# rishabhmisra/Scalable-Bayesian-Matrix-Factorization

Measured on AMD Instinct MI355X. Metric: ratings/sec per Gibbs sweep, ML-20M K=100, higher is better.
Workload: dtype f64

## Files before the change

### scalable-bayesian-matrix-factorization_amd/csrc/ctx.h

```cpp
#pragma once
#include <hip/hip_runtime.h>

#include <algorithm>
#include <array>
#include <chrono>
#include <cmath>
#include <cstdarg>
#include <cstdio>
#include <cstdlib>
#include <cstring>
#include <memory>
#include <numeric>
#include <string>
#include <thread>
#include <vector>

#include "../../include/sbmf.h"
#include "comm.h"
#include "common.h"
#include <rccl/rccl.h>
#include "kernels.h"
#include "rng.h"
#include "fmc.h"
#include "fmm.h"
#include "fmg.h"
#include "fmq.h"
#include "foldin.h"
#include "lists.h"
#include "recommend.h"
#include "samples.h"
#include "samples_foldin.h"
#include "vbo.h"

struct sbmf_ctx;

namespace sbmf {

static const int NBIN = GK_NUM + 1;

struct Side {
    uint32_t R = 0;
    std::vector<uint32_t> ptr;
    std::vector<uint32_t> part;
    std::vector<uint32_t> perm;
    std::vector<double> r;
    uint32_t r0 = 0, r1 = 0;
    std::vector<uint64_t> bounds;
    struct StreamSet {
        std::vector<SplitTask> stasks;
        std::vector<SplitRow> xrows;
        uint32_t nxchunk = 0;
        uint32_t sgrid = 0;
        uint32_t cmax = 0;
        uint32_t tune = 0;
    };
    struct Stage {
        uint32_t r0 = 0, r1 = 0;
        std::vector<uint32_t> bin_rows[NBIN];
        StreamSet ss[2];
        std::vector<std::array<uint32_t, 3>> gsub[GK_NUM];
        DBuf d_bins[NBIN], d_stasks[2], d_xrows[2];
        std::vector<size_t> soff, scnt, roff, rcnt;
        size_t rbeg = 0, rend = 0;
    };
    std::vector<std::unique_ptr<Stage>> stg;
    std::vector<std::vector<uint64_t>> sbounds;
    std::vector<ResidTask> rtasks;
    std::vector<uint32_t> rtptr;
    std::vector<uint32_t> perm2, unpack;
    size_t nsend = 0, nrecv = 0;
};

static const int KIND_STREAM = GK_NUM;

}

using namespace sbmf;

struct Hyper {
    double tau = 1.0, b0 = 0.0, mu_b0 = 0.0, sig_b0 = 0.0;
    std::vector<double> sig_u, mu_u, sig_v, mu_v;
};

struct ScoreList {
    const char* what;
    const char* reg;
    uint32_t n = 0, J = 0, Jp = 0;
    uint32_t count = 0;
    int clamp = 0;
    bool latest = false;
    DBuf d_ids, d_S1, d_S2;
    Span sel;
    void alloc(uint32_t n_, uint32_t J_, int clamp_, hipStream_t st);
    void drop();
    template <typename T>
    void accumulate(sbmf_ctx* c, const T* rows, const double* bu, const double* bv, double b0, hipStream_t se);
    void scores(sbmf_ctx* c, const char* fn, uint32_t row, double* mean, double* stdev);
    void recommend(sbmf_ctx* c, const uint32_t* csr_ptr, const uint32_t* csr_items, uint32_t topn, uint32_t flags,
                   double risk, uint32_t* items, double* mean, double* stdev);
};

struct SampleStore {
    uint32_t cap = 0, every = 1, head = 0, count = 0, seen = 0;
    size_t bytes = 0;
    DBuf d_U, d_V, d_bu, d_bv;
    std::vector<double> b0;
    std::vector<uint32_t> sweep;
    std::vector<double> hyper;
    bool has_hyper = false;
    Span cev, scv, sel;
    Span gdr, gsc, gse;
    uint64_t budget = 0;
    bool unfused = false, fused_draw = false;
    uint32_t slot(uint32_t s) const { return (head + s) % cap; }
    void alloc(sbmf_ctx* c, uint32_t cap_, uint32_t every_);
    void drop();
    template <typename T>
    void keep(sbmf_ctx* c, const Hyper& hy, hipStream_t se);
};

struct sbmf_ctx {
    sbmf_ctx() { sbmf::audit().contexts++; }
    sbmf_config cfg{};
    std::string err;
    bool spent = false, dead = false;
    std::vector<uint32_t> tu, ti, su, si;
    std::vector<double> tr, sr;
    uint32_t I = 0, J = 0, I_req = 0, J_req = 0;
    bool prepared = false;
    double init_sd = 1.0, lo = 1.0, hi = 5.0;
    int sd_is_var = 1;
    uint32_t K = 0, Kp = 0;
    Side users, items;
    uint64_t t0 = 0, t1 = 0;
    std::vector<uint64_t> tbounds, tbblocks;
    std::vector<uint64_t> tperm;
    Hyper hyp[2];
    int reported = 0;
    Hyper& hyper_of(uint32_t sw) { return hyp[sw & 1]; }
    bool bias = false;
    std::vector<uint32_t> empty_u, empty_v;
    std::vector<std::array<double, 3>> shadow_u, shadow_v;
    uint32_t sweep = 0, collected = 0;
    GlibcRand grand{1};
    int nranks = 1, rank = 0;
    Comm own_comm;
    Comm* comm = &own_comm;
    hipStream_t st = nullptr;
    hipEvent_t ev[10] = {};
    std::vector<hipEvent_t> kevs;
    hipEvent_t& kev(uint32_t stage, int side, int kind, int e) {
        return kevs[(((size_t)stage * 2 + side) * SBMF_NKIND + kind) * 2 + e];
    }
    std::vector<int8_t> kprev;
    int8_t& kpv(uint32_t stage, int side, int kind) { return kprev[((size_t)stage * 2 + side) * SBMF_NKIND + kind]; }
    std::vector<hipEvent_t> kbegin;
    hipEvent_t& kbg(uint32_t stage, int side, int kind) { return kbegin[((size_t)stage * 2 + side) * SBMF_NKIND + kind]; }
    uint32_t nstages = 1;
    hipStream_t stc = nullptr;
    std::vector<hipEvent_t> sev;
    bool virt = false;
    std::vector<hipEvent_t> tsev;
    hipEvent_t cev[2] = {};
    hipStream_t sto = nullptr;
    hipStream_t sto2 = nullptr;
    hipEvent_t oev[4] = {};
    DBuf d_uptr, d_upart, d_uperm, d_ur, d_vptr, d_vpart, d_vperm, d_vr;
    DBuf d_U, d_V, d_Eu, d_Ev, d_zU, d_zV, d_hyper;
    DBuf d_rowsq_u, d_rowtr_u, d_rowsq_v, d_rowtr_v;
    DBuf d_colpart, d_res, d_scratch;
    size_t scratch_half = 0;

    bool kprof = false;
    int kprof_set = 0;
    DBuf d_kprof;
    DBuf d_rtasks, d_rtptr, d_rtsq;
    DBuf d_xslabs, d_xcnt, d_xchunk_sq, d_xchunk_tr, d_xnewown;
    static constexpr size_t kColdSlot = 256;
    DBuf d_gcold;
    std::vector<unsigned char> h_gcold;
    bool time_kinds = true;
    size_t xset_nx = 1;
    DBuf d_tu, d_ti, d_tr, d_tsum, d_tpart;
    DBuf d_uperm2, d_vperm2, d_uunpack, d_vunpack, d_xrecv;
    DBuf d_bu, d_bv, d_mbu, d_mbv, d_sbu, d_sbv;
    DBuf d_var3u, d_var3v, d_epart;
    std::vector<double> h_res;
    double* h_pre = nullptr;
    void* h_io = nullptr;
    double* h_out() { return static_cast<double*>(h_io); }
    void* h_hyper() { return static_cast<char*>(h_io) + 128; }
    hipEvent_t hev = nullptr;
    struct PreDraw {
        bool valid = false;
        bool staged = false;
        uint32_t sweep = 0;
        double d0 = 0;
        Hyper h;
    } pre;
    bool hyper_ahead = false;
    double* h_pinned = nullptr;
    size_t h_pinned_bytes = 0, h_pre_bytes = 0, h_io_bytes = 0;
    sbmf_timing timing{};
    uint32_t launches = 0;
    ScoreList watch{"watch list", "sbmf_watch_users"};
    hipEvent_t wev[2] = {};
    ScoreList guests{"fold-in list", "sbmf_foldin_users"};
    uint32_t fdrawn = 0;
    GuestCSR fcsr;
    DBuf d_fG, d_fhyp;
    double* h_fhyp = nullptr;
    size_t h_fhyp_bytes = 0;
    hipEvent_t fev[3] = {};
    ScoreList fmq{"query list", "sbmf_fm_query_cases"};
    FMQueryList fmqd;
    SampleStore samples;
    VBLearner* vb = nullptr;
    FMChain* fm = nullptr;
    FMGroups fmgroups;
    std::vector<FMRelation> fmrels;
    struct HostCases {
        std::vector<uint64_t> ptr;
        std::vector<uint32_t> attr;
        std::vector<float> x, y;
        uint32_t num_attr = 0;
        bool set = false;
        sbmf_cases view() {
            sbmf_cases c{};
            c.n = y.size();
            c.nnz = attr.size();
            c.num_attr = num_attr;
            c.ptr = ptr.data();
            c.attr = attr.data();
            c.x = x.data();
            c.target = y.data();
            return c;
        }
    } ctr, cte;
    ~sbmf_ctx();
};

#define API_BEGIN try {
#define API_END(ctx) } catch (...) { return sbmf::api_error(ctx); } return SBMF_OK;

namespace sbmf {

int api_error(sbmf_ctx* ctx);
void samples_ready(sbmf_ctx* c, const char* fn);
size_t slot_bytes(const sbmf_ctx* c);
void partition_bounds(const uint32_t* ptr, uint32_t R, int nranks, uint64_t* bounds);
template <typename T>
void prepare_T(sbmf_ctx* c);
template <typename T>
void run_half(sbmf_ctx* c, const Hyper& hy, bool users, uint32_t stage, hipEvent_t start = nullptr);
template <typename T>
void run_sweeps_T(sbmf_ctx* c, uint32_t nsweeps, sbmf_sweep_cb cb, void* user);

enum { RES_ESQ = 0, RES_TRSQ = 1, RES_TEST_AVG = 2, RES_TEST_THIS = 3, RES_ES = 4, RES_ESQ2 = 5, RES_TIMEOUT = 7, RES_COL = 8 };

static size_t tsize(const sbmf_ctx* c) { return c->cfg.precision == SBMF_F32 ? 4 : 8; }

static bool avg_collected(const sbmf_config& cf) {
    return cf.average == 1 || (cf.average == 0 && cf.quirks == SBMF_QUIRKS_NONE);
}

template <typename T>
static std::vector<T> to_T(const std::vector<double>& v) {
    return std::vector<T>(v.begin(), v.end());
}

template <typename T>
static void upload_table(sbmf_ctx* c, DBuf& d, const double* src, uint32_t R) {
    std::vector<T> h((size_t)R * c->Kp, T(0));
    for (uint32_t r = 0; r < R; ++r)
        for (uint32_t k = 0; k < c->K; ++k) h[(size_t)r * c->Kp + k] = (T)src[(size_t)r * c->K + k];
    HIPCHK(hipMemcpy(d.p, h.data(), h.size() * sizeof(T), hipMemcpyHostToDevice));
}
template <typename T>
static void download_table(sbmf_ctx* c, const DBuf& d, double* dst, uint32_t R) {
    std::vector<T> h((size_t)R * c->Kp);
    HIPCHK(hipMemcpy(h.data(), d.p, h.size() * sizeof(T), hipMemcpyDeviceToHost));
    for (uint32_t r = 0; r < R; ++r)
        for (uint32_t k = 0; k < c->K; ++k) dst[(size_t)r * c->K + k] = (double)h[(size_t)r * c->Kp + k];
}
static void upload_table(sbmf_ctx* c, DBuf& d, const double* src, uint32_t R) {
    c->cfg.precision == SBMF_F32 ? upload_table<float>(c, d, src, R) : upload_table<double>(c, d, src, R);
}
static void download_table(sbmf_ctx* c, const DBuf& d, double* dst, uint32_t R) {
    c->cfg.precision == SBMF_F32 ? download_table<float>(c, d, dst, R) : download_table<double>(c, d, dst, R);
}

static void ensure_pinned(sbmf_ctx* c, size_t bytes) {
    if (c->h_pinned_bytes >= bytes) return;
    pinned_free(c->h_pinned, c->h_pinned_bytes);
    c->h_pinned_bytes = 0;
    pinned_alloc((void**)&c->h_pinned, bytes);
    c->h_pinned_bytes = bytes;
}

}
```

### scalable-bayesian-matrix-factorization_amd/csrc/kernels.h

```cpp
#pragma once
#include <hip/hip_runtime.h>

#include <cstdint>

namespace sbmf {

template <typename T>
struct HalfArgs {
    const uint32_t* ptr;
    const uint32_t* part;
    const uint32_t* perm;
    const T* E_this;
    T* E_other;
    const T* r_this;
    T* own;
    const T* partner;
    const T* sig;
    const T* mu;
    uint32_t zrow;
    const T* zbuf;
    T tau;
    uint32_t K, Kp;
    int sd_is_var;
    uint64_t seed;
    uint32_t sweep, tag;
    double* row_sq;
    double* row_tr;
    T lo, hi;
    int e_from_dot;
    uint32_t tune;
    unsigned long long* prof;
    uint64_t lim_partner;
    uint64_t lim_other;
    uint64_t lim_this;
    uint32_t lim_rows;
};

enum GblockKind { GK_W4 = 0, GK_W16 = 1, GK_B2 = 2, GK_B4 = 3, GK_B8 = 4, GK_NUM = 5 };
inline uint32_t gk_maxdeg(int kind, bool f64, bool wide = false) {
    static const uint32_t waves4[GK_NUM] = {1, 4, 8, 16, 32};
    const uint32_t per_wave = f64 ? 32 : 64;
    if (wide && f64 && (kind == GK_W16 || kind == GK_B2)) return 64;
    return kind == GK_W4 ? per_wave / 4 : per_wave * waves4[kind] / 4;
}

template <typename T>
hipError_t launch_gblock_nw(int nw, const uint32_t* rows, uint32_t nrows, const HalfArgs<T>& a, hipStream_t st);
template <typename T>
hipError_t launch_gblock(int kind, const uint32_t* rows, uint32_t nrows, const HalfArgs<T>& a, hipStream_t st);

template <typename T>
struct GresCold;
template <typename T>
hipError_t launch_grow(int nw, const uint32_t* rows, uint32_t nrows, const HalfArgs<T>& a, const GresCold<T>* d_cold,
                       hipStream_t st);
uint32_t grow_maxdeg(int nw, bool f64);

struct SplitTask {
    uint32_t row;
    uint32_t beg;
    uint32_t len;
    uint32_t nch;
    uint32_t chunk;
    uint32_t slab0;
    uint32_t xrow;
    uint32_t xown;
    uint32_t xstr;
    uint32_t pad[3];
};
constexpr uint32_t SLAB_DOUBLES = 16 * 16 + 16;
struct SplitRow {
    uint32_t row, slab0, nch, pad;
};
struct SplitSync {
    double* slabs;
    uint32_t* qhead;
    uint32_t nblk;
    double* chunk_sq;
    double* chunk_tr;
    void* newown;
    uint32_t* timeout;
    uint32_t cmax;
    unsigned long long* prof;
    uint64_t lim_slab;
    uint32_t lim_chunk;
};
template <typename T>
struct GresCold {
    const uint32_t* ptr;
    const uint32_t* part;
    const uint32_t* perm;
    const T* E_this;
    T* E_other;
    const T* r_this;
    T* own;
    const T* zbuf;
    const T* sig;
    double* row_sq;
    double* row_tr;
    double* chunk_sq;
    double* chunk_tr;
    T* newown;
    uint32_t* timeout;
    T lo, hi;
    uint32_t zrow;
    int e_from_dot;
    unsigned long long* prof;
    uint64_t lim_partner, lim_other, lim_this, lim_slab;
    uint32_t lim_rows, lim_chunk;
};
template <typename T>
GresCold<T> gres_cold(const HalfArgs<T>& a, const SplitSync* sy);

template <typename T>
uint32_t gstream_cmax(uint32_t tune);
int gstream_wg_target(uint32_t tune);
template <typename T>
int gstream_blocks_per_cu(uint32_t cmax, uint32_t tune);
template <typename T>
hipError_t launch_gstream(const SplitTask* tasks, uint32_t ntask, uint32_t grid, const SplitRow* srows, uint32_t nsrow,
                          const HalfArgs<T>& a, const SplitSync& sy, const GresCold<T>* d_cold, hipStream_t st);

constexpr uint32_t RESID_CHUNK = 1024;
struct ResidTask {
    uint32_t row, beg, len, pad;
};
template <typename T>
hipError_t launch_resid(const ResidTask* tasks, uint32_t ntask, const uint32_t* tptr, uint32_t r0, uint32_t r1,
                        const uint32_t* part, const uint32_t* perm, const T* r, const T* own, const T* partner,
                        uint32_t K, uint32_t Kp, T* E_other, double* task_sq, double* row_sq, const double* b_own,
                        const double* b_part, double b0, hipStream_t st);

template <typename T>
hipError_t launch_colstats(const T* tabA, uint32_t rA, const T* muA, double* outA, const T* tabB, uint32_t rB,
                           const T* muB, double* outB, uint32_t K, uint32_t Kp, hipStream_t st);

template <typename T>
hipError_t launch_test(const uint32_t* tu, const uint32_t* ti, const double* tr, uint64_t t0, uint64_t t1,
                       const T* U, const T* V, uint32_t K, uint32_t Kp, T lo, T hi, int collect, double div,
                       double* sum, double* part, const double* bu, const double* bv, double b0, hipStream_t st);

struct BiasArgs {
    double alpha;
    double d0;
    double ag, bg, sg, mg;
    uint64_t seed;
    uint32_t sweep, tag;
    int sd_is_var;
};
template <typename T>
hipError_t launch_bias_rows(const uint32_t* ptr, uint32_t r0, uint32_t r1, T* E, double* b, double* mu_b,
                            double* sig_b, const double* var3, const BiasArgs& p, hipStream_t st);
template <typename T>
hipError_t launch_esum2(const T* E, uint64_t n, double* part, double* out2, hipStream_t st);

template <typename T>
hipError_t launch_rowsum2(const uint32_t* ptr, uint32_t r0, uint32_t r1, const T* E, double* out, hipStream_t st);

template <typename T>
hipError_t launch_unpack(const T* recv, const uint32_t* idx, uint64_t n, T* E, hipStream_t st);

hipError_t launch_sum(const double* in, uint64_t n, double* out, double* scratch, hipStream_t st);
hipError_t launch_sum_cols(const double* in, uint32_t nchunk, uint32_t width, double* out, hipStream_t st);
hipError_t launch_sum_cols2(const double* in, uint32_t nchunk, double* out, const double* in2, uint32_t nchunk2,
                            double* out2, uint32_t width, hipStream_t st);

template <typename T>
hipError_t launch_philox_fill(T* z, uint32_t K, uint32_t r0, uint32_t r1, uint64_t seed, uint32_t sweep, uint32_t tag,
                              hipStream_t st);
template <typename T>
hipError_t launch_philox_fill2(T* zu, uint32_t u0, uint32_t u1, uint32_t tagu, T* zv, uint32_t v0, uint32_t v1,
                               uint32_t tagv, uint32_t K, uint64_t seed, uint32_t sweep, hipStream_t st);
template <typename T>
hipError_t launch_init_philox(T* tab, uint32_t K, uint32_t Kp, uint32_t r0, uint32_t r1, double sd, uint64_t seed,
                              uint32_t tag, hipStream_t st);

}
```

### scalable-bayesian-matrix-factorization_amd/csrc/kernels.hip

```cpp
#include <hip/hip_runtime.h>

#include <cstdlib>

#include "kernels.h"
#include "rng.h"

#ifndef SBMF_KERNELS_INSTR_H_
#define CHK(i, lim) (i)
#define SBMF_GBLOCK_PHASES(on) auto stamp = [](int) {}
#define SBMF_GRES_PHASES(nch, prof_) \
    auto stamp = [](int) {};         \
    auto stamp_first = [](int) {}
#define SBMF_XSENT_CHECK(bad) ((void)0)
#endif

namespace sbmf {
namespace {

template <int CTRL, int ROWM>
__device__ __forceinline__ int dpp_i(int v) {
    if constexpr (ROWM == 0xf && (CTRL <= 0xff || (CTRL >= 0x121 && CTRL <= 0x12f) || CTRL == 0x140 || CTRL == 0x141))
        return __builtin_amdgcn_mov_dpp(v, CTRL, ROWM, 0xf, false);
    else
        return __builtin_amdgcn_update_dpp(0, v, CTRL, ROWM, 0xf, false);
// ... 225 lines not shown
    __shared__ uint32_t pmS[NWAVE][V * 4];
    __shared__ T eS[NWAVE][V * 4];
    {
        const uint32_t k0 = NW > 1 ? threadIdx.x : lane, kst = NW > 1 ? 64 * NW : 64;
        for (uint32_t k = k0; k < Kp; k += kst) zS[ws][k] = k < K ? a.zbuf[(size_t)CHK(row, a.lim_rows) * K + k] : T(0);
    }
    T e[V];
    T* const eR = &eS[wv][rr];
    const uint32_t* const pjR = &pjS[wv][rr];
    constexpr int SG = V < 8 ? V : V >= 16 ? 4 : 8;
#pragma unroll
    for (int g0 = 0; g0 < V; g0 += SG) {
        uint32_t pjv[SG], pmv[SG];
        T ev[SG];
#pragma unroll
        for (int u = 0; u < SG; ++u) {
            const uint32_t q = (uint32_t)((wr * V + g0 + u) * 4 + rr);
            const uint32_t qi = (uint32_t)CHK(q < n ? beg + q : 0u, a.lim_this);
            pjv[u] = a.part[qi];
            pmv[u] = a.perm[qi];
            ev[u] = a.e_from_dot ? T(0) : a.E_this[qi];
        }
#pragma unroll
        for (int u = 0; u < SG; ++u) {
            const int v = g0 + u;
            const uint32_t q = (uint32_t)((wr * V + v) * 4 + rr);
            const uint32_t pj = q < n ? pjv[u] : a.zrow;
            if (ci == 0) {
                pjS[wv][4 * v + rr] = pj * Kp;
                pmS[wv][4 * v + rr] = q < n ? pmv[u] : 0u;
                eR[4 * v] = q < n ? ev[u] : T(0);
            }
        }
    }
    asm volatile("" ::: "memory");
    const T* __restrict__ pbase = a.partner + ci;
#define PROW(v) (pbase + pjR[4 * (v)])
    auto gat = [&](int v, uint32_t k0) -> T { return pbase[CHK(pjR[4 * v] + k0 + ci, a.lim_partner) - ci]; };
    if (a.e_from_dot) {
        T dot[V];
#pragma unroll
        for (int v = 0; v < V; ++v) dot[v] = T(0);
        for (uint32_t k0 = 0; k0 < K; k0 += GB) {
            const T o = a.own[(size_t)row * Kp + k0 + ci];
#pragma unroll
            for (int v = 0; v < V; ++v) dot[v] += PROW(v)[k0] * o;
        }
#pragma unroll
        for (int v = 0; v < V; ++v) {
            const T d = row16_sum(dot[v]);
            const uint32_t q = (uint32_t)((wr * V + v) * 4 + rr);
            const T e0 = q < n ? a.r_this[beg + q] - d : T(0);
            if (ci == 0) eR[4 * v] = e0;
        }
    }
    asm volatile("" ::: "memory");
    const T tau = a.tau;
    const T* __restrict__ orow = a.own + (size_t)CHK(row, a.lim_rows) * Kp + ci;
    stamp(0);
    __shared__ T Rs[NWAVE * V * 4];
    const bool want_r = a.row_tr != nullptr;
    if (want_r) {
#pragma unroll
        for (int g0 = 0; g0 < V; g0 += SG) {
            T rv[SG];
#pragma unroll
            for (int u = 0; u < SG; ++u) {
                const uint32_t q = (uint32_t)((wr * V + g0 + u) * 4 + rr);
                rv[u] = a.r_this[q < n ? beg + q : 0u];
            }
            if (ci == 0) {
#pragma unroll
                for (int u = 0; u < SG; ++u) {
                    const uint32_t q = (uint32_t)((wr * V + g0 + u) * 4 + rr);
                    Rs[(wv * V + g0 + u) * 4 + rr] = q < n ? rv[u] : T(0);
                }
            }
        }
    }
    T s[V], sn[V];
#pragma unroll
    for (int v = 0; v < V; ++v) s[v] = gat(v, 0);
    T oldc = orow[0], sgc = a.sig[ci], muc = a.mu[ci];
    for (uint32_t b0 = 0; b0 < K; b0 += GB) {
        const uint32_t kk = b0 + ci;
        const bool kin = kk < K;
        const uint32_t kn = b0 + GB;
        const T oldn = orow[kn];
        const T sgn = a.sig[kn + ci];
        const T mun = a.mu[kn + ci];
#pragma unroll
        for (int v = 0; v < V; ++v) sn[v] = gat(v, kn);
        acc_t g = {T(0), T(0), T(0), T(0)};
        T cc = T(0);
#pragma unroll
        for (int v = 0; v < V; ++v) {
            g = MfmaT<T>::mfma(s[v], g);
            cc += s[v] * eR[4 * v];
        }
        cc += shfl_xor_t(cc, 16);
        cc += shfl_xor_t(cc, 32);
        stamp(1);
        if constexpr (NW > 1) lds_barrier();
        stamp(2);
#pragma unroll
        for (int j = 0; j < 4; ++j) {
            const int r = MfmaT<T>::row(lane, j);
            Ls[NW > 1 ? wr : ws][r][ci] = ci < r ? g[j] : T(0);
            if (r == ci) Ps[NW > 1 ? wr : ws][ci] = g[j];
        }
        if (lane < GB) Cs[NW > 1 ? wr : ws][lane] = cc;
        if constexpr (NW > 1) {
            lds_barrier();
            for (int x = threadIdx.x; x < GB * GB; x += 64 * NW) {
                const int r0 = x >> 4, c0 = x & 15;
                if (c0 < r0) {
                    T sum = Ls[0][r0][c0];
#pragma unroll
                    for (int w = 1; w < NW; ++w) sum += Ls[w][r0][c0];
                    Ls[0][r0][c0] = sum;
                }
                if (x < GB) {
                    T cs = Cs[0][x], ps = Ps[0][x];
#pragma unroll
                    for (int w = 1; w < NW; ++w) {
                        cs += Cs[w][x];
                        ps += Ps[w][x];
                    }
                    Cs[0][x] = cs;
                    Ps[0][x] = ps;
                }
            }
            lds_barrier();
            stamp(3);
        } else {
            __builtin_amdgcn_s_waitcnt(0xc07f);
            __builtin_amdgcn_wave_barrier();
        }
        T dlt = T(0);
        if (NW == 1 || wr == 0) {
            const T P = Ps[ws][ci];
            const T old = oldc, sg = sgc, mu = muc;
            const T z = zS[ws][kk];
            const T var = kin ? T(1) / (sg + tau * P) : T(0);
            const T sd = tsqrt_if(var, !a.sd_is_var);
            const T A = var * sg * mu + sd * z;
            const T Bq = var * tau;
            dlt = gblock_solve_lds(&Ls[ws][ci][0], Bq, A - old + Bq * (Cs[ws][ci] + P * old));
            const T nwv = old + dlt;
            if constexpr (NW > 1) {
                if (wr == 0 && lane < GB && kin) newS[kk] = nwv;
                if (lane < GB) Dsh[lane] = dlt;
            } else {
                if (lane < GB && kin) a.own[(size_t)row * Kp + kk] = nwv;
            }
        }
        if constexpr (NW > 1) {
            lds_barrier();
            dlt = Dsh[ci];
        }
        stamp(4);
        {
#pragma unroll
            for (int v = 0; v < V; ++v) s[v] = s[v] * dlt;
            const int vb = row16_scatter(s, ci);
            constexpr int RV = V >= 16 ? V / 16 : 1;
#pragma unroll
            for (int j = 0; j < RV; ++j) eR[4 * (vb + j)] = eR[4 * (vb + j)] - s[j];
            asm volatile("" ::: "memory");
        }
        stamp(5);
#pragma unroll
        for (int v = 0; v < V; ++v) s[v] = sn[v];
        oldc = oldn;
        sgc = sgn;
        muc = mun;
    }

    if constexpr (NW > 1) {
        lds_barrier();
        for (uint32_t k = threadIdx.x; k < K; k += 64 * NW) a.own[(size_t)row * Kp + k] = newS[k];
    }
    T sq = T(0), trs = T(0);
#pragma unroll
    for (int v = 0; v < V; ++v) e[v] = eR[4 * v];
#pragma unroll
    for (int v = 0; v < V; ++v) {
        const uint32_t q = (uint32_t)((wr * V + v) * 4 + rr);
        if (q < n && ci == 0) {
            a.E_other[CHK(pmS[wv][4 * v + rr], a.lim_other)] = e[v];
            sq += e[v] * e[v];
            if (want_r) {
                const T r = Rs[(wv * V + v) * 4 + rr];
                T pr = r - e[v];
                pr = (pr < a.hi) ? pr : a.hi;
                pr = (a.lo < pr) ? pr : a.lo;
                trs += (pr - r) * (pr - r);
            }
        }
    }
    if (a.row_sq || a.row_tr) {
        double dsq = wave_sum((double)sq);
        double dtr = wave_sum((double)trs);
        if constexpr (NW > 1) {
            __shared__ double red2[NW][2];
            if (lane == 0) {
                red2[wr][0] = dsq;
                red2[wr][1] = dtr;
            }
            lds_barrier();
            dsq = 0.0;
            dtr = 0.0;
            for (int w = 0; w < NW; ++w) {
                dsq += red2[w][0];
                dtr += red2[w][1];
            }
        }
        if (wr == 0 && lane == 0) {
            if (a.row_sq) a.row_sq[row] = dsq;
            if (a.row_tr) a.row_tr[row] = dtr;
        }
    }
    stamp(6);
#undef PROW
}


__device__ __forceinline__ void st_sc1(double* p, double v) {
    __hip_atomic_store(p, v, __ATOMIC_RELAXED, __HIP_MEMORY_SCOPE_AGENT);
}
__device__ __forceinline__ void st_sc1(uint64_t* p, uint64_t v) {
    __hip_atomic_store(p, v, __ATOMIC_RELAXED, __HIP_MEMORY_SCOPE_AGENT);
}
__device__ __forceinline__ uint64_t ld_sc1(const uint64_t* p) {
    return __hip_atomic_load(p, __ATOMIC_RELAXED, __HIP_MEMORY_SCOPE_AGENT);
}
constexpr uint64_t XSENT = ~0ull;
__device__ __forceinline__ uint64_t xsent_here() {
    uint32_t w = ~0u;
    asm volatile("" : "+v"(w));
    return ((uint64_t)w << 32) | w;
}
__device__ __forceinline__ uint64_t xword(double v) { return (uint64_t)__double_as_longlong(v); }
__device__ __forceinline__ double xdbl(uint64_t w) { return __longlong_as_double((long long)w); }
#ifndef SBMF_XDELAY
#define SBMF_XDELAY 0
#endif
#ifndef SBMF_XBACKOFF
#define SBMF_XBACKOFF 1
#endif
struct GresSums {
    double sq, tr;
};
template <int VC>
struct GresOrder {
    static constexpr int VP = VC <= 8 ? 8 : VC <= 16 ? 16 : VC <= 32 ? 32 : VC <= 64 ? 64 : 128;
    static constexpr int RV = VP >= 16 ? VP / 16 : 1;
    struct Arr {
        int a[VC];
    };
    static constexpr Arr make() {
        Arr o{};
        int n = 0;
        const int lo[4] = {VP / 2, VP / 4, VP / 8, VP / 16};
        const int hi[4] = {VC, VP / 2, VP / 4, VP / 8};
        for (int l = 0; l < 4; ++l) {
            if (l == 3 && VP < 16) break;
            for (int j = lo[l]; j < hi[l] && j < VC; ++j) o.a[n++] = j;
        }
        for (int j = 0; j < RV && j < VC; ++j) o.a[n++] = j;
        return o;
    }
    static constexpr Arr arr = make();
    static constexpr const int* v = arr.a;
};
template <typename T>
struct GresW {
    static constexpr int VW = sizeof(T) == 8 ? 32 : 64;
};
template <typename T>
struct GresHot {
    const T* partner;
    const GresCold<T>* cold;
    T* own;
    const T* sig;
    double* slabs;
    uint32_t* qhead;
    T tau;
    uint32_t K, Kp;
    int sd_is_var;
};
template <typename T>
using ColdP = const __attribute__((address_space(4))) GresCold<T>*;
template <typename T>
__device__ __forceinline__ ColdP<T> cold_here(const GresCold<T>* p) {
    ColdP<T> q = (ColdP<T>)(uintptr_t)p;
    asm volatile("" : "+s"(q));
    return q;
}
template <typename U>
__device__ __forceinline__ __attribute__((address_space(1))) U* glob(U* p) {
    return (__attribute__((address_space(1))) U*)(uintptr_t)p;
}
template <typename T, int NW, int SIDE, bool LIST, int KL = 256>
__device__ __forceinline__ void gres_run(const SplitTask* __restrict__ tasks, const uint32_t* __restrict__ lrows,
                                         uint32_t ntask, const GresHot<T>& a) {
    typedef typename MfmaT<T>::acc_t acc_t;
    constexpr bool ONE = NW == 1;
    constexpr bool DIRECT = LIST;
    constexpr bool SMG = LIST && KL > 128;
    constexpr int VW = GresW<T>::VW;
    constexpr uint32_t CAP = 4 * NW * VW;
    constexpr int SL = GB * GB + GB;
    static_assert(SL == (int)SLAB_DOUBLES, "the host's exchange offsets (SplitTask::xrow, xstr) use SLAB_DOUBLES");
    const int lane = threadIdx.x & 63;
    const int wr = threadIdx.x >> 6;
    const int ci = lane & 15;
    const int rr = lane >> 4;
    const uint32_t K = a.K, Kp = a.Kp;
    const uint32_t nblk = (K + GB - 1) / GB;
    const T tau = a.tau;
#ifdef SBMF_KPROF_BUILD
    unsigned long long* const kprof_ = cold_here(a.cold)->prof;
#endif
    __shared__ uint32_t pjL[CAP];
    __shared__ uint32_t pmL[CAP];
    __shared__ T eL[CAP];
    constexpr int PW = GB * GLD + GB;
    __shared__ T Pw[NW][ONE ? 1 : PW];
    __shared__ T Rr[PW + GB + (ONE ? 64 : 0)];
    __shared__ T newS[DIRECT ? 1 : 256];
    __shared__ double red2[NW][2];
    constexpr int SLP = GB * (GB + 1) / 2 + GB;
    constexpr bool XCH = NW >= 3;
// ... 218 lines not shown
                    if (SBMF_XDELAY > 0) __builtin_amdgcn_s_sleep(SBMF_XDELAY);
                    lds_barrier();
                    if (xpart < XP) {
                        const uint32_t c0 = xpart * nch / XP, c1 = (xpart + 1) * nch / XP;
                        const uint32_t p0 = xrow + tb + xb;
                        auto slab = [&](uint32_t c_, uint32_t u_) {
                            uint32_t pc = p0 + c_ * xstr;
                            asm volatile("" : "+v"(pc));
                            return reinterpret_cast<const uint64_t*>(sb + (size_t)(u_ * xstr) + pc);
                        };
                        uint32_t spins = 0;
                        auto miss = [&](uint32_t m) -> bool {
                            if (!__builtin_amdgcn_ballot_w64(m == 0xffffffffu)) return false;
                            if (++spins > (1u << 22)) {
                                uint32_t one = 1u;
                                asm volatile("" : "+v"(one));
                                __hip_atomic_store(glob(cold_here(a.cold)->timeout), one, __ATOMIC_RELAXED, __HIP_MEMORY_SCOPE_AGENT);
                                spins = 1u << 22;
                                return false;
                            }
                            __builtin_amdgcn_s_sleep(SBMF_XBACKOFF);
                            return true;
                        };
                        double sum = 0.0;
                        uint32_t c = c0;
                        while (c + 8 <= c1) {
                            uint64_t v[8];
                            uint32_t m = 0u;
#pragma unroll
                            for (int u = 0; u < 8; ++u) v[u] = ld_sc1(slab(c, u));
#pragma unroll
                            for (int u = 0; u < 8; ++u) m = max(m, (uint32_t)v[u] & (uint32_t)(v[u] >> 32));
                            if (miss(m)) continue;
                            stamp_first(8);
#pragma unroll
                            for (int u = 0; u < 8; ++u) sum += xdbl(v[u]);
                            c += 8;
                        }
                        while (c < c1) {
                            const uint64_t v = ld_sc1(slab(c, 0));
                            if (miss((uint32_t)v & (uint32_t)(v >> 32))) continue;
                            stamp_first(8);
                            sum += xdbl(v);
                            ++c;
                        }
                        xsum[xpart][xe] = sum;
                    }
                    lds_barrier();
                    if (xin && t > 0)
                        st_sc1(reinterpret_cast<uint64_t*>(sb + (xown + tb + xb) - (uint32_t)(SL * sizeof(double))), xsent_here());
                    if (xin) {
                        double sum = xsum[0][xe];
#pragma unroll
                        for (int q = 1; q < XP; ++q) sum += xsum[q][xe];
                        val = (T)sum;
                    }
                }
                if (xin) Rr[xd] = val;
                lds_barrier();
                }
                stamp(4);
                T dlt;
                {
                    const uint32_t kk = t * GB + ci;
                    const bool kin = kk < K;
                    T sg, mu;
                    if constexpr (SMG) {
                        const T* sgp = a.sig + t * GB;
                        asm volatile("" : "+s"(sgp));
                        sg = sgp[ci];
                        mu = sgp[Kp + ci];
                    } else {
                        sg = sgL[kk];
                        mu = muL[kk];
                    }
                    const T old = oL[kk], z = zL[kk];
                    const T P = Rr[PW + ci];
                    const T Cc = Rr[GB * GLD + ci];
                    const T var = kin ? T(1) / (sg + tau * P) : T(0);
                    const T sd = tsqrt_if(var, !a.sd_is_var);
                    const T A = var * sg * mu + sd * z;
                    const T Bq = var * tau;
                    dlt = gblock_solve_lds(&Rr[ci * GLD], Bq, A - old + Bq * (Cc + P * old));
                    if (lane < GB && wr == 0) {
                        if constexpr (DIRECT) {
                            T* orow = a.own + ((size_t)CHK(row_d, cold_here(a.cold)->lim_rows) * Kp + t * GB);
                            asm volatile("" : "+s"(orow));
                            if (kin) orow[ci] = old + dlt;
                        } else {
                            if (kin) newS[kk] = old + dlt;
                        }
                    }
                }
                Dl = dlt;
                stamp(5);
                return Dl;
            };
            {
                T s[VC];
#pragma unroll
                for (int j = 0; j < VC; ++j) s[j] = gat(j, 0);
                for (uint32_t t = 0; t < nblk; ++t) {
                    asm volatile("" ::: "memory");
                    if (t > 0) {
                        apply(s, Dl, [&](int j) { s[j] = gat(j, t); });
                    }
                    stamp(1);
                    acc_t g = {T(0), T(0), T(0), T(0)};
                    T cc = T(0);
                    accumulate(s, g, cc);
                    stamp(2);
                    Dl = finish_block(g, cc, t, [] {}, std::integral_constant<int, 0>{});
                }
                apply(s, Dl, [](int) {});
            }
            __syncthreads();
            double sq = 0.0, trs = 0.0;
            {
                const ColdP<T> ce = cold_here(a.cold);
                const auto Eo = glob(ce->E_other);
                const bool tr = ce->row_tr != nullptr;
                const auto rt = glob(ce->r_this);
                const T lo = ce->lo, hi = ce->hi;
                const uint32_t beg = tr ? task_here().beg : 0u;
                for (uint32_t x = threadIdx.x; x < n; x += 64 * NW) {
                    const T e = eL[x];
                    Eo[CHK(pmL[x], ce->lim_other)] = e;
                    sq += (double)(e * e);
                    if (tr) {
                        const T r = rt[beg + x];
                        T pr = r - e;
                        pr = (pr < hi) ? pr : hi;
                        pr = (lo < pr) ? pr : lo;
                        trs += (double)((pr - r) * (pr - r));
                    }
                }
            }
            return GresSums{sq, trs};
        };
        GresSums sums;
        if (vpw <= (uint32_t)VW / 4)
            sums = body(std::integral_constant<int, VW / 4>{});
        else if (vpw <= (uint32_t)VW / 2)
            sums = body(std::integral_constant<int, VW / 2>{});
        else if (vpw <= (uint32_t)(3 * VW / 4))
            sums = body(std::integral_constant<int, 3 * VW / 4>{});
        else
            sums = body(std::integral_constant<int, VW>{});
        const ColdP<T> cz = cold_here(a.cold);
        const SplitTask tk = task_here();
        const uint32_t row = tk.row;
        if (!DIRECT && tk.chunk == 0) {
            const auto dst = nch > 1 ? glob(cz->newown) + (size_t)CHK(tk.slab0, cz->lim_chunk) * Kp
                                     : glob(cz->own) + (size_t)CHK(row, cz->lim_rows) * Kp;
            for (uint32_t k = threadIdx.x; k < K; k += 64 * NW) dst[k] = newS[k];
        }
        double dsq = wave_sum(sums.sq);
        double dtr = wave_sum(sums.tr);
        if (lane == 0) {
            red2[wr][0] = dsq;
            red2[wr][1] = dtr;
        }
        __syncthreads();
        if (threadIdx.x == 0) {
            dsq = 0.0;
            dtr = 0.0;
            for (int w = 0; w < NW; ++w) {
                dsq += red2[w][0];
                dtr += red2[w][1];
            }
            if (nch > 1) {
                cz->chunk_sq[CHK(tk.slab0 + tk.chunk, cz->lim_chunk)] = dsq;
                cz->chunk_tr[CHK(tk.slab0 + tk.chunk, cz->lim_chunk)] = dtr;
            } else {
                if (cz->row_sq) cz->row_sq[row] = dsq;
                if (cz->row_tr) cz->row_tr[row] = dtr;
            }
        }
        __syncthreads();
        stamp(6);
    }
}
template <typename T, int NW, int SIDE>
__global__ __launch_bounds__(64 * NW, 4) void k_gres(
    const SplitTask* __restrict__ tasks, uint32_t ntask, GresHot<T> a) {
    gres_run<T, NW, SIDE, false>(tasks, nullptr, ntask, a);
}
template <typename T, int NW, int SIDE, int KL>
__global__ __launch_bounds__(64 * NW, 4) void k_grow(
    const uint32_t* __restrict__ rows, uint32_t nrows, GresHot<T> a) {
    gres_run<T, NW, SIDE, true, KL>(nullptr, rows, nrows, a);
}

template <typename T>
__global__ __launch_bounds__(64) void k_split_finish(const SplitRow* __restrict__ srows, uint32_t nrows, HalfArgs<T> a,
                                                     SplitSync sy) {
    if (blockIdx.x == 0 && threadIdx.x == 0) *sy.qhead = 0u;
    if (blockIdx.x >= nrows) return;
    const SplitRow sr = srows[blockIdx.x];
    const uint32_t K = a.K, Kp = a.Kp;
    {
        constexpr uint32_t SLP = GB * (GB + 1) / 2 + GB;
        uint64_t* const last = reinterpret_cast<uint64_t*>(sy.slabs) + ((size_t)sr.slab0 * sy.nblk + (sy.nblk - 1)) * SLAB_DOUBLES;
        for (uint32_t i = threadIdx.x; i < sr.nch * SLP; i += 64)
            last[CHK((size_t)(i / SLP) * sy.nblk * SLAB_DOUBLES + i % SLP,
                     sy.lim_slab - ((size_t)sr.slab0 * sy.nblk + (sy.nblk - 1)) * SLAB_DOUBLES)] = XSENT;
    }
    for (uint32_t k = threadIdx.x; k < K; k += 64) a.own[(size_t)sr.row * Kp + k] = static_cast<const T*>(sy.newown)[(size_t)sr.slab0 * Kp + k];
    if (threadIdx.x == 0) {
        double s = 0.0, t = 0.0;
        for (uint32_t c = 0; c < sr.nch; ++c) {
            s += sy.chunk_sq[sr.slab0 + c];
            t += sy.chunk_tr[sr.slab0 + c];
        }
        if (a.row_sq) a.row_sq[sr.row] = s;
        if (a.row_tr) a.row_tr[sr.row] = t;
    }
}


template <typename T>
__global__ __launch_bounds__(256) void k_resid(const ResidTask* __restrict__ tasks, uint32_t ntask,
                                                const uint32_t* __restrict__ part, const uint32_t* __restrict__ perm,
                                                const T* __restrict__ r, const T* __restrict__ own,
                                                const T* __restrict__ partner, uint32_t K, uint32_t Kp,
                                                T* __restrict__ E_other, double* __restrict__ task_sq,
                                                const double* __restrict__ b_own, const double* __restrict__ b_part,
                                                double b0) {
    const uint32_t ti = blockIdx.x * 4 + (threadIdx.x >> 6);
    const int lane = threadIdx.x & 63;
    if (ti >= ntask) return;
    const ResidTask tk = tasks[ti];
    const int ci = lane & 15, rr = lane >> 4;
    const T* o = own + (size_t)tk.row * Kp;
    T ov[16];
#pragma unroll
    for (int b = 0; b < 16; ++b) ov[b] = 16 * b < (int)Kp ? o[16 * b + ci] : T(0);
    double sq = 0.0;
    const uint32_t end = tk.beg + tk.len;
    for (uint32_t i0 = tk.beg; i0 < end; i0 += 4) {
        const uint32_t idx = i0 + rr;
        const bool ok = idx < end;
        const T* src = partner + (size_t)part[ok ? idx : tk.beg] * Kp;
        T d = T(0);
#pragma unroll
        for (int b = 0; b < 16; ++b)
            if (16 * b < (int)Kp) d += ov[b] * src[16 * b + ci];
        d = row16_sum(d);
        if (ok && ci == 0) {
            const T e = b_own ? r[idx] - ((T)((b0 + b_part[part[idx]]) + b_own[tk.row]) + d) : r[idx] - d;
            E_other[perm[idx]] = e;
            sq += (double)(e * e);
        }
    }
    sq = wave_sum(sq);
    if (lane == 0) task_sq[ti] = sq;
}

__global__ __launch_bounds__(256) void k_resid_rows(const uint32_t* __restrict__ tptr, uint32_t r0, uint32_t r1,
                                                     const double* __restrict__ task_sq, double* __restrict__ row_sq) {
    const uint32_t row = r0 + blockIdx.x * 256 + threadIdx.x;
    if (row >= r1) return;
    double s = 0.0;
    for (uint32_t t = tptr[row - r0]; t < tptr[row - r0 + 1]; ++t) s += task_sq[t];
    row_sq[row] = s;
}

template <typename T, int CPL>
__global__ __launch_bounds__(256) void k_colstats(const T* __restrict__ tabA, uint32_t rA, const T* __restrict__ muA,
                                                   double* __restrict__ outA, uint32_t nA, const T* __restrict__ tabB,
                                                   uint32_t rB, const T* __restrict__ muB, double* __restrict__ outB,
                                                   uint32_t K, uint32_t Kp) {
    constexpr int RW = 64;
    constexpr int RB = CPL <= 2 ? 16 : 8;
    const bool first = blockIdx.x < nA;
    const T* __restrict__ tab = first ? tabA : tabB;
    const T* __restrict__ mu = first ? muA : muB;
    double* __restrict__ out = first ? outA : outB;
    const uint32_t R = first ? rA : rB;
    const uint32_t c = first ? blockIdx.x : blockIdx.x - nA;
    const int lane = threadIdx.x & 63, w = threadIdx.x >> 6;
    double m[CPL], s1[CPL], s2[CPL];
#pragma unroll
    for (int j = 0; j < CPL; ++j) {
        const uint32_t k = lane + 64 * j;
        m[j] = k < K ? (double)mu[k] : 0.0;
        s1[j] = 0.0;
        s2[j] = 0.0;
    }
    const uint32_t rb = c * 256 + w * RW;
    for (int b0 = 0; b0 < RW; b0 += RB) {
        double x[RB][CPL];
#pragma unroll
        for (int i = 0; i < RB; ++i) {
            const uint32_t r = rb + b0 + i;
            const T* row = tab + (size_t)(r < R ? r : 0) * Kp + lane;
#pragma unroll
            for (int j = 0; j < CPL; ++j) x[i][j] = lane + 64 * j < Kp ? (double)row[64 * j] : 0.0;
        }
#pragma unroll
        for (int i = 0; i < RB; ++i) {
            if (rb + b0 + i < R) {
#pragma unroll
                for (int j = 0; j < CPL; ++j) {
                    s2[j] += (x[i][j] - m[j]) * (x[i][j] - m[j]);
                    s1[j] += x[i][j];
                }
            }
        }
    }
    __shared__ double red[4][2][64 * CPL];
#pragma unroll
    for (int j = 0; j < CPL; ++j) {
        red[w][0][lane + 64 * j] = s2[j];
        red[w][1][lane + 64 * j] = s1[j];
    }
    __syncthreads();
    for (uint32_t k = threadIdx.x; k < K; k += 256) {
        out[(size_t)c * 2 * K + k] = ((red[0][0][k] + red[1][0][k]) + red[2][0][k]) + red[3][0][k];
        out[(size_t)c * 2 * K + K + k] = ((red[0][1][k] + red[1][1][k]) + red[2][1][k]) + red[3][1][k];
    }
}

template <typename T, int PR, int CB, bool REUSE>
__global__ __launch_bounds__(256) void k_test(const uint32_t* __restrict__ tu, const uint32_t* __restrict__ ti,
                                               const double* __restrict__ tr, uint64_t t0, uint64_t t1,
                                               const T* __restrict__ U, const T* __restrict__ V, uint32_t K,
                                               uint32_t Kp, T lo, T hi, int collect, double div,
                                               double* __restrict__ sum, double* __restrict__ part,
                                               const double* __restrict__ bu, const double* __restrict__ bv,
                                               double b0) {
    const int lane = threadIdx.x & 63, w = threadIdx.x >> 6;
    const int ci = lane & 15, rr = lane >> 4;
    const uint64_t gbase = t0 + (uint64_t)blockIdx.x * 256 + (uint64_t)w * 64 + (uint64_t)rr * 16;
    const uint32_t nb = Kp / 16;
    const uint64_t mt = gbase + ci;
    const bool mok = mt < t1;
    const uint64_t mtc = mok ? mt : t0;
    const uint32_t myu = tu[mtc], myi = ti[mtc];
    const double myr = tr[mtc], mys = sum[mtc];
    double myb = 0.0;
    if (bu) myb = (b0 + bu[myu]) + bv[myi];
    double a2 = 0.0, t2 = 0.0;
    T uc[REUSE ? CB : 1];
    uint32_t ucur = 0xffffffffu;
    for (int it = 0; it < 16; it += PR) {
        uint32_t uu[PR], ii[PR];
#pragma unroll
        for (int j = 0; j < PR; ++j) {
            const int src = (lane & 48) + it + j;
            uu[j] = (uint32_t)__shfl((int)myu, src);
            ii[j] = (uint32_t)__shfl((int)myi, src);
        }
        T p[PR];
#pragma unroll
        for (int j = 0; j < PR; ++j) p[j] = T(0);
        if constexpr (REUSE) {
            T ub[PR][CB], vb[PR][CB];
#pragma unroll
            for (int j = 0; j < PR; ++j) {
#pragma unroll
// ... 195 lines not shown
    for (; q < end; q += 64) E[q] = (E[q] + d0) + db;
    if (lane == 0) {
        b[row] = bn;
        mu_b[row] = mu;
        sig_b[row] = sig;
    }
}

template <typename T>
__global__ __launch_bounds__(256) void k_esum2(const T* __restrict__ E, uint64_t n, double* __restrict__ part) {
    const uint64_t b0 = (uint64_t)blockIdx.x * 1024;
    double s = 0.0, s2 = 0.0;
#pragma unroll
    for (int q = 0; q < 4; ++q) {
        const uint64_t i = b0 + threadIdx.x * 4 + q;
        if (i < n) {
            const double e = (double)E[i];
            s += e;
            s2 += e * e;
        }
    }
    s = wave_sum(s);
    s2 = wave_sum(s2);
    __shared__ double red[4][2];
    if ((threadIdx.x & 63) == 0) {
        red[threadIdx.x >> 6][0] = s;
        red[threadIdx.x >> 6][1] = s2;
    }
    __syncthreads();
    if (threadIdx.x == 0) {
        part[2 * blockIdx.x] = ((red[0][0] + red[1][0]) + red[2][0]) + red[3][0];
        part[2 * blockIdx.x + 1] = ((red[0][1] + red[1][1]) + red[2][1]) + red[3][1];
    }
}

template <typename T>
__global__ __launch_bounds__(256) void k_rowsum2(const uint32_t* __restrict__ ptr, uint32_t r0, uint32_t r1,
                                                 const T* __restrict__ E, double* __restrict__ out) {
    const uint32_t r = r0 + blockIdx.x * 4 + (threadIdx.x >> 6);
    if (r >= r1) return;
    const int lane = threadIdx.x & 63;
    double s = 0.0, s2 = 0.0;
    const uint32_t end = ptr[r + 1];
    uint32_t q = ptr[r] + lane;
    for (; q + 7 * 64 < end; q += 8 * 64) {
        T ev[8];
#pragma unroll
        for (int u = 0; u < 8; ++u) ev[u] = E[q + u * 64];
#pragma unroll
        for (int u = 0; u < 8; ++u) {
            const double e = (double)ev[u];
            s += e;
            s2 += e * e;
        }
    }
    for (; q < end; q += 64) {
        const double e = (double)E[q];
        s += e;
        s2 += e * e;
    }
    s = wave_sum(s);
    s2 = wave_sum(s2);
    if (lane == 0) {
        out[2 * (size_t)r] = s;
        out[2 * (size_t)r + 1] = s2;
    }
}

template <typename T>
__global__ __launch_bounds__(256) void k_unpack(const T* __restrict__ recv, const uint32_t* __restrict__ idx,
                                                 uint64_t n, T* __restrict__ E) {
    const uint64_t j = (uint64_t)blockIdx.x * 256 + threadIdx.x;
    if (j < n) E[idx[j]] = recv[j];
}

}

template <typename T>
hipError_t launch_gblock(int kind, const uint32_t* rows, uint32_t nrows, const HalfArgs<T>& a, hipStream_t st) {
    if (nrows == 0) return hipSuccess;
    if (a.K > 256) return hipErrorInvalidValue;
    constexpr int V = sizeof(T) == 8 ? 8 : 16;
    switch (kind) {
        case GK_W4:
            k_gblock<T, V / 4, 1, 4><<<(nrows + 3) / 4, 256, 0, st>>>(rows, nrows, a);
            break;
        case GK_W16:
            if (sizeof(T) == 8 && !(a.tune & 8u))
                k_gblock<T, 16, 1, 2><<<(nrows + 1) / 2, 128, 0, st>>>(rows, nrows, a);
            else
                k_gblock<T, V, 1, 4><<<(nrows + 3) / 4, 256, 0, st>>>(rows, nrows, a);
            break;
        case GK_B2:
            k_gblock<T, V, 2, 1><<<nrows, 128, 0, st>>>(rows, nrows, a);
            break;
        case GK_B4:
            k_gblock<T, V, 4, 1><<<nrows, 256, 0, st>>>(rows, nrows, a);
            break;
        case GK_B8:
            k_gblock<T, V, 8, 1><<<nrows, 512, 0, st>>>(rows, nrows, a);
            break;
        default:
            return hipErrorInvalidValue;
    }
    return hipGetLastError();
}

static int gres_nw(uint32_t tune) { return (tune & 128u) ? 4 : (tune & 0x20000u) ? 16 : 8; }
int gstream_wg_target(uint32_t tune) { return 16 / gres_nw(tune); }

template <typename T>
hipError_t launch_gblock_nw(int nw, const uint32_t* rows, uint32_t nrows, const HalfArgs<T>& a, hipStream_t st) {
    if (nrows == 0) return hipSuccess;
    constexpr int V = sizeof(T) == 8 ? 8 : 16;
    const bool wide = sizeof(T) == 8 && nw >= 5;
#define SBMF_GB_NW(V_, NW_)                                                                      \
    case NW_:                                                                                    \
        k_gblock<T, V_, NW_, 1><<<nrows, 64 * NW_, 0, st>>>(rows, nrows, a);                     \
        break;
    if (wide) {
        switch ((nw + 1) / 2) {
            SBMF_GB_NW(16, 3)
            SBMF_GB_NW(16, 4)
            default:
                return hipErrorInvalidValue;
        }
        return hipGetLastError();
    }
    switch (nw) {
        SBMF_GB_NW(V, 2)
        SBMF_GB_NW(V, 3)
        SBMF_GB_NW(V, 4)
        SBMF_GB_NW(V, 5)
        SBMF_GB_NW(V, 6)
        SBMF_GB_NW(V, 7)
        SBMF_GB_NW(V, 8)
        default:
            return hipErrorInvalidValue;
    }
#undef SBMF_GB_NW
    return hipGetLastError();
}

template <typename T>
GresCold<T> gres_cold(const HalfArgs<T>& a, const SplitSync* sy) {
    GresCold<T> c{};
    c.ptr = a.ptr;
    c.part = a.part;
    c.perm = a.perm;
    c.E_this = a.E_this;
    c.E_other = a.E_other;
    c.r_this = a.r_this;
    c.own = a.own;
    c.zbuf = a.zbuf;
    c.sig = a.sig;
    c.row_sq = a.row_sq;
    c.row_tr = a.row_tr;
    c.lo = a.lo;
    c.hi = a.hi;
    c.zrow = a.zrow;
    c.e_from_dot = a.e_from_dot;
    c.lim_partner = a.lim_partner;
    c.lim_other = a.lim_other;
    c.lim_this = a.lim_this;
    c.lim_rows = a.lim_rows;
    if (sy) {
        c.chunk_sq = sy->chunk_sq;
        c.chunk_tr = sy->chunk_tr;
        c.newown = static_cast<T*>(sy->newown);
        c.timeout = sy->timeout;
        c.prof = sy->prof;
        c.lim_slab = sy->lim_slab;
        c.lim_chunk = sy->lim_chunk;
    }
    return c;
}
template <typename T>
static GresHot<T> gres_hot(const HalfArgs<T>& a, const SplitSync* sy, const GresCold<T>* d_cold) {
    GresHot<T> h{};
    h.partner = a.partner;
    h.cold = d_cold;
    if (!sy) {
        h.own = a.own;
        h.sig = a.sig;
    }
    h.tau = a.tau;
    h.K = a.K;
    h.Kp = a.Kp;
    h.sd_is_var = a.sd_is_var;
    if (sy) {
        h.slabs = sy->slabs;
        h.qhead = sy->qhead;
    }
    return h;
}

template <typename T>
hipError_t launch_grow(int nw, const uint32_t* rows, uint32_t nrows, const HalfArgs<T>& ha, const GresCold<T>* d_cold,
                       hipStream_t st) {
    if (nrows == 0) return hipSuccess;
    if (ha.K > 256 || !d_cold || ha.mu != ha.sig + ha.Kp) return hipErrorInvalidValue;
    const bool side = ha.tag == TAG_ITEMS;
    const GresHot<T> a = gres_hot<T>(ha, nullptr, d_cold);
    auto go = [&](auto kl) {
        constexpr int KL = decltype(kl)::value;
        if (nw == 1) {
            if (side)
                k_grow<T, 1, 1, KL><<<nrows, 64, 0, st>>>(rows, nrows, a);
            else
                k_grow<T, 1, 0, KL><<<nrows, 64, 0, st>>>(rows, nrows, a);
        } else if (nw == 2) {
            if (side)
                k_grow<T, 2, 1, KL><<<nrows, 128, 0, st>>>(rows, nrows, a);
            else
                k_grow<T, 2, 0, KL><<<nrows, 128, 0, st>>>(rows, nrows, a);
        } else {
            return hipErrorInvalidValue;
        }
        return hipGetLastError();
    };
    return ha.Kp <= 128 && !(ha.tune & 0x1000u) ? go(std::integral_constant<int, 128>{})
                                               : go(std::integral_constant<int, 256>{});
}
uint32_t grow_maxdeg(int nw, bool f64) { return 4u * (uint32_t)nw * (f64 ? GresW<double>::VW : GresW<float>::VW); }

template <typename T>
static const void* gstream_fn(uint32_t tune, uint32_t side = 0) {
    if (gres_nw(tune) == 4) return side ? (const void*)k_gres<T, 4, 1> : (const void*)k_gres<T, 4, 0>;
    if (gres_nw(tune) == 16) return side ? (const void*)k_gres<T, 16, 1> : (const void*)k_gres<T, 16, 0>;
    return side ? (const void*)k_gres<T, 8, 1> : (const void*)k_gres<T, 8, 0>;
}

template <typename T>
uint32_t gstream_cmax(uint32_t tune) {
    return 4 * gres_nw(tune) * GresW<T>::VW;
}

template <typename T>
int gstream_blocks_per_cu(uint32_t cmax, uint32_t tune) {
    (void)cmax;
    int n = 0;
    if (hipOccupancyMaxActiveBlocksPerMultiprocessor(&n, gstream_fn<T>(tune), 64 * gres_nw(tune), 0) != hipSuccess)
        return 1;
    return n;
}

template <typename T>
hipError_t launch_gstream(const SplitTask* tasks, uint32_t ntask, uint32_t grid, const SplitRow* srows, uint32_t nsrow,
                          const HalfArgs<T>& a, const SplitSync& sy, const GresCold<T>* d_cold, hipStream_t st) {
    if (ntask == 0) return hipSuccess;
    if (a.K > 256 || sy.cmax == 0 || grid == 0 || !d_cold || a.mu != a.sig + a.Kp) return hipErrorInvalidValue;
    hipError_t err;
    const SplitTask* tp = tasks;
    GresHot<T> hp = gres_hot<T>(a, &sy, d_cold);
    void* args[] = {(void*)&tp, (void*)&ntask, (void*)&hp};
    const void* fn = gstream_fn<T>(a.tune, a.tag == TAG_ITEMS ? 1u : 0u);
    const dim3 g(std::min(grid, ntask)), b(64 * gres_nw(a.tune));
    if (a.tune & 0x1000000u)
        err = hipLaunchCooperativeKernel(fn, g, b, args, 0, st);
    else
        err = hipLaunchKernel(fn, g, b, args, 0, st);
    if (err != hipSuccess) return err;
    {
        k_split_finish<T><<<std::max(nsrow, 1u), 64, 0, st>>>(srows, nsrow, a, sy);
        return hipGetLastError();
    }
    return hipSuccess;
}

template <typename T>
hipError_t launch_resid(const ResidTask* tasks, uint32_t ntask, const uint32_t* tptr, uint32_t r0, uint32_t r1,
                        const uint32_t* part, const uint32_t* perm, const T* r, const T* own, const T* partner,
                        uint32_t K, uint32_t Kp, T* E_other, double* task_sq, double* row_sq, const double* b_own,
                        const double* b_part, double b0, hipStream_t st) {
    if (r1 <= r0) return hipSuccess;
    if (Kp > 256) return hipErrorInvalidValue;
    if (ntask) k_resid<T><<<(ntask + 3) / 4, 256, 0, st>>>(tasks, ntask, part, perm, r, own, partner, K, Kp, E_other,
                                                          task_sq, b_own, b_part, b0);
    k_resid_rows<<<(r1 - r0 + 255) / 256, 256, 0, st>>>(tptr, r0, r1, task_sq, row_sq);
    return hipGetLastError();
}

template <typename T>
hipError_t launch_colstats(const T* tabA, uint32_t rA, const T* muA, double* outA, const T* tabB, uint32_t rB,
                           const T* muB, double* outB, uint32_t K, uint32_t Kp, hipStream_t st) {
    const uint32_t nA = (rA + 255) / 256, nB = (rB + 255) / 256;
    if (nA + nB == 0) return hipSuccess;
    if (K > 256 || Kp > 256) return hipErrorInvalidValue;
    if (Kp <= 64)
        k_colstats<T, 1><<<nA + nB, 256, 0, st>>>(tabA, rA, muA, outA, nA, tabB, rB, muB, outB, K, Kp);
    else if (Kp <= 128)
        k_colstats<T, 2><<<nA + nB, 256, 0, st>>>(tabA, rA, muA, outA, nA, tabB, rB, muB, outB, K, Kp);
    else
        k_colstats<T, 4><<<nA + nB, 256, 0, st>>>(tabA, rA, muA, outA, nA, tabB, rB, muB, outB, K, Kp);
    return hipGetLastError();
}

template <typename T>
hipError_t launch_test(const uint32_t* tu, const uint32_t* ti, const double* tr, uint64_t t0, uint64_t t1, const T* U,
                       const T* V, uint32_t K, uint32_t Kp, T lo, T hi, int collect, double div, double* sum,
                       double* part, const double* bu, const double* bv, double b0, hipStream_t st) {
    if (t1 <= t0) return hipSuccess;
    const uint64_t nb = (t1 - t0 + 255) / 256;
    if (Kp <= 128)
        k_test<T, 2, 8, true><<<(uint32_t)nb, 256, 0, st>>>(tu, ti, tr, t0, t1, U, V, K, Kp, lo, hi, collect, div, sum,
                                                            part, bu, bv, b0);
    else
        k_test<T, 2, 8, false><<<(uint32_t)nb, 256, 0, st>>>(tu, ti, tr, t0, t1, U, V, K, Kp, lo, hi, collect, div, sum,
                                                             part, bu, bv, b0);
    return hipGetLastError();
}

hipError_t launch_sum(const double* in, uint64_t n, double* out, double* scratch, hipStream_t st) {
    if (n == 0) return hipMemsetAsync(out, 0, sizeof(double), st);
    const double* cur = in;
    double* buf[2] = {scratch, scratch + (n + 1023) / 1024 + 1};
    int which = 0;
    while (n > 1) {
        const uint64_t nb = (n + 1023) / 1024;
        double* dst = (nb == 1) ? out : buf[which];
        k_sum_blocks<<<(uint32_t)nb, 256, 0, st>>>(cur, n, dst);
        hipError_t err = hipGetLastError();
        if (err != hipSuccess) return err;
        cur = dst;
        n = nb;
        which ^= 1;
        if (nb == 1) return hipSuccess;
    }
    return hipMemcpyAsync(out, cur, sizeof(double), hipMemcpyDeviceToDevice, st);
}

hipError_t launch_sum_cols(const double* in, uint32_t nchunk, uint32_t width, double* out, hipStream_t st) {
    k_sum_cols<<<width, 256, 0, st>>>(in, nchunk, width, out, nullptr, 0, nullptr);
    return hipGetLastError();
}
hipError_t launch_sum_cols2(const double* in, uint32_t nchunk, double* out, const double* in2, uint32_t nchunk2,
// ... 101 lines not shown
```

### scalable-bayesian-matrix-factorization_amd/csrc/lists.cpp

```cpp
#include "ctx.h"

namespace sbmf {

static void one_real_rank(const sbmf_ctx* c, const char* what, const char* fn) {
    if (c->virt) fail(SBMF_E_STATE, "%s: a virtual rank's numbers are not a chain; no %s there", fn, what);
    if (c->nranks > 1 || c->comm->active() || c->comm != &c->own_comm)
        fail(SBMF_E_STATE, "%s: the %s runs on one rank; this context joined a communicator", fn, what);
}
static void is_prepared(const sbmf_ctx* c, const char* fn) {
    if (!c->prepared) fail(SBMF_E_STATE, "%s: not prepared (sbmf_prepare)", fn);
}
void list_scope(const sbmf_ctx* c, const char* what, const char* fn, bool unbiased_only) {
    if (c->cfg.method != SBMF_METHOD_MCMC)
        fail(SBMF_E_STATE, "%s: the %s is offered by the SBPMF sampler (SBMF_METHOD_MCMC) only; this "
                           "context runs the %s learner", fn, what,
             c->cfg.method == SBMF_METHOD_VB ? "online VB" : c->cfg.method == SBMF_METHOD_ALS ? "ALS" : "libFM MCMC");
    if (unbiased_only && c->bias)
        fail(SBMF_E_STATE, "%s: the %s covers the unbiased quirk sets (final, sbpmf2, none); a guest of "
                           "the biased sampler (bias2 / bias22) would need a bias draw of its own", fn, what);
    one_real_rank(c, what, fn);
    is_prepared(c, fn);
}
void list_sync(sbmf_ctx* c) {
    HIPCHK(hipSetDevice(c->cfg.device));
    HIPCHK(hipStreamSynchronize(c->sto));
    HIPCHK(hipStreamSynchronize(c->st));
}

void TopnScratch::alloc(uint32_t rows, uint32_t topn, uint32_t J, bool exclude) {
    const size_t slots = (size_t)rows * topn;
    d_it.alloc(slots * sizeof(uint32_t));
    d_ms.alloc(2 * slots * sizeof(double));
    if (exclude) d_mask.alloc((size_t)rows * watch_jw(J) * sizeof(uint32_t));
}
void select_topn(TopnScratch& t, const uint32_t* d_ids, uint32_t m, const double* S1, const double* S2, uint32_t J,
                 uint32_t count, const uint32_t* csr_ptr, const uint32_t* csr_items, uint32_t topn, double risk, Span& span,
                 hipStream_t st, uint32_t* items, double* mean, double* stdev) {
    const uint32_t Jw = watch_jw(J);
    const size_t slots = (size_t)m * topn;
    uint32_t* mask = csr_ptr ? t.d_mask.as<uint32_t>() : nullptr;
    double* ms = t.d_ms.as<double>();
    span.begin(st);
    if (mask) {
        HIPCHK(hipMemsetAsync(mask, 0, (size_t)m * Jw * sizeof(uint32_t), st));
        HIPCHK(launch_watch_mask(d_ids, m, csr_ptr, csr_items, mask, Jw, st));
    }
    HIPCHK(launch_watch_select(m, S1, S2, J, (double)count, risk, mask, topn, t.d_it.as<uint32_t>(), ms, ms + slots, st));
    span.end(st);
    HIPCHK(hipStreamSynchronize(st));
    HIPCHK(hipMemcpy(items, t.d_it.p, slots * sizeof(uint32_t), hipMemcpyDeviceToHost));
    HIPCHK(hipMemcpy(mean, ms, slots * sizeof(double), hipMemcpyDeviceToHost));
    if (stdev) HIPCHK(hipMemcpy(stdev, ms + slots, slots * sizeof(double), hipMemcpyDeviceToHost));
}
void row_moments(const double* S1, const double* S2, uint32_t J, uint32_t count, hipStream_t st, double* mean, double* stdev) {
    DBuf tmp;
    tmp.alloc((size_t)2 * J * sizeof(double));
    double* d = tmp.as<double>();
    HIPCHK(launch_watch_moments(S1, S2, J, (double)count, d, d + J, st));
    HIPCHK(hipStreamSynchronize(st));
    HIPCHK(hipMemcpy(mean, d, (size_t)J * sizeof(double), hipMemcpyDeviceToHost));
    if (stdev) HIPCHK(hipMemcpy(stdev, d + J, (size_t)J * sizeof(double), hipMemcpyDeviceToHost));
}

void GuestCSR::check(const char* fn, uint32_t n, const uint32_t* ptr, const uint32_t* items, const double* ratings, uint32_t J) {
    if (n && !ptr) fail(SBMF_E_ARG, "%s: null ptr with n > 0", fn);
    if (n >= 0xfffffffeu) fail(SBMF_E_ARG, "%s: %u guests are too many", fn, n);
    for (uint32_t g = 0; g < n; ++g)
        if (ptr[g + 1] < ptr[g]) fail(SBMF_E_ARG, "%s: ptr decreases at guest %u (%u then %u)", fn, g, ptr[g], ptr[g + 1]);
    const uint32_t p0 = n ? ptr[0] : 0, nnz = n ? ptr[n] - p0 : 0;
    if (nnz && (!items || !ratings)) fail(SBMF_E_ARG, "%s: null items / ratings with ratings listed", fn);
    for (uint32_t q = 0; q < nnz; ++q)
        if (items[p0 + q] >= J)
            fail(SBMF_E_ARG, "%s: items[%u] = %u is not below the %u items", fn, p0 + q, items[p0 + q], J);
}
void GuestCSR::upload(uint32_t n_, const uint32_t* ptr, const uint32_t* items, const double* ratings, uint32_t rows_per_slice,
                      hipStream_t st, uint32_t* ids) {
    n = n_;
    const uint32_t p0 = ptr[0];
    nnz = ptr[n] - p0;
    std::vector<uint32_t> hp(n + 1), ident(n);
    for (uint32_t g = 0; g <= n; ++g) hp[g] = ptr[g] - p0;
    std::iota(ident.begin(), ident.end(), 0u);
    std::vector<uint32_t> order(ident);
    for (uint32_t off = 0; off < n; off += rows_per_slice)
        std::stable_sort(order.begin() + off, order.begin() + std::min(n, off + rows_per_slice),
                         [&](uint32_t x, uint32_t y) { return hp[x + 1] - hp[x] > hp[y + 1] - hp[y]; });
    d_E.alloc((size_t)nnz * sizeof(double));
    d_items.alloc((size_t)nnz * sizeof(uint32_t));
    d_ratings.alloc((size_t)nnz * sizeof(double));
    sbmf::upload(d_ptr, hp, st);
    sbmf::upload(d_order, order, st);
    if (ids) HIPCHK(hipMemcpyAsync(ids, ident.data(), ident.size() * sizeof(uint32_t), hipMemcpyHostToDevice, st));
    else sbmf::upload(d_ids, ident, st);
    if (nnz) {
        HIPCHK(hipMemcpyAsync(d_items.p, items + p0, (size_t)nnz * sizeof(uint32_t), hipMemcpyHostToDevice, st));
        HIPCHK(hipMemcpyAsync(d_ratings.p, ratings + p0, (size_t)nnz * sizeof(double), hipMemcpyHostToDevice, st));
    }
    HIPCHK(hipStreamSynchronize(st));
}
void GuestCSR::drop() {
    for (DBuf* d : {&d_ptr, &d_items, &d_ratings, &d_order, &d_E, &d_ids}) d->release();
    n = nnz = 0;
}

}

void ScoreList::alloc(uint32_t n_, uint32_t J_, int clamp_, hipStream_t st) {
    n = n_;
    J = J_;
    Jp = sbmf::watch_jp(J);
    clamp = clamp_;
    const size_t bytes = (size_t)n * Jp * sizeof(double);
    d_S1.alloc(bytes);
    d_S2.alloc(bytes);
    d_ids.alloc((size_t)n * sizeof(uint32_t));
    sel.create();
    HIPCHK(hipMemsetAsync(d_S1.p, 0, bytes, st));
    HIPCHK(hipMemsetAsync(d_S2.p, 0, bytes, st));
}
void ScoreList::drop() {
    for (sbmf::DBuf* d : {&d_ids, &d_S1, &d_S2}) d->release();
    sel.destroy();
    n = J = Jp = count = 0;
    clamp = 0;
    latest = false;
}
template <typename T>
void ScoreList::accumulate(sbmf_ctx* c, const T* rows, const double* bu, const double* bv, double b0, hipStream_t se) {
    HIPCHK(sbmf::launch_watch_accum<T>(d_ids.as<uint32_t>(), n, rows, c->d_V.as<T>(), c->J, c->Kp, bu, bv, b0, clamp,
                                       c->lo, c->hi, d_S1.as<double>(), d_S2.as<double>(), se));
    count++;
    c->launches++;
}
template void ScoreList::accumulate<float>(sbmf_ctx*, const float*, const double*, const double*, double, hipStream_t);
template void ScoreList::accumulate<double>(sbmf_ctx*, const double*, const double*, const double*, double, hipStream_t);
void ScoreList::scores(sbmf_ctx* c, const char* fn, uint32_t row, double* mean, double* stdev) {
    if (row >= n) sbmf::fail(SBMF_E_ARG, "%s: row %u of a %s of %u", fn, row, what, n);
    sbmf::row_moments(d_S1.as<double>() + (size_t)row * Jp, d_S2.as<double>() + (size_t)row * Jp, J, count, c->st, mean, stdev);
    if (stdev && latest) std::fill(stdev, stdev + J, 0.0);
}
void ScoreList::recommend(sbmf_ctx* c, const uint32_t* csr_ptr, const uint32_t* csr_items, uint32_t topn,
                          uint32_t flags, double risk, uint32_t* items, double* mean, double* stdev) {
    const bool exclude = !(flags & 1u);
    sbmf::TopnScratch t;
    t.alloc(n, topn, J, exclude);
    sbmf::select_topn(t, d_ids.as<uint32_t>(), n, d_S1.as<double>(), d_S2.as<double>(), J, count, exclude ? csr_ptr : nullptr,
                      csr_items, topn, risk, sel, c->st, items, mean, stdev);
    if (stdev && latest)
        for (size_t q = 0, slots = (size_t)n * topn; q < slots; ++q)
            if (items[q] != 0xffffffffu) stdev[q] = 0.0;
}

extern "C" {

static void list_registered(const ScoreList& l, const char* fn) {
    if (!l.n) sbmf::fail(SBMF_E_STATE, "%s: no %s registered (%s)", fn, l.what, l.reg);
}
static void list_ready(sbmf_ctx* c, const ScoreList& l, const char* fn, bool sums = true, const char* note = "") {
    list_registered(l, fn);
    if (sums && !l.count)
        sbmf::fail(SBMF_E_STATE, "%s: no sweep accumulated since the %s was registered%s", fn, l.what, note);
    list_sync(c);
}
static void recommend_args(const char* fn, uint32_t topn, uint32_t flags, double risk) {
    if (topn < 1 || topn > 1024) sbmf::fail(SBMF_E_ARG, "%s: topn %u is not in 1..1024", fn, topn);
    if (flags & ~1u) sbmf::fail(SBMF_E_ARG, "%s: unknown flags 0x%x (bit 0 = keep rated items)", fn, flags & ~1u);
    if (!(risk == risk)) sbmf::fail(SBMF_E_ARG, "%s: risk is NaN", fn);
}

static void watch_drop(sbmf_ctx* c) {
    c->watch.drop();
    for (hipEvent_t& e : c->wev) sbmf::event_destroy(e);
}

int sbmf_watch_users(sbmf_ctx* ctx, uint32_t n, const uint32_t* users, uint32_t flags) {
    API_BEGIN
    if (!ctx) sbmf::fail(SBMF_E_ARG, "null context");
    list_scope(ctx, ctx->watch.what, "sbmf_watch_users", false);
    if (n && !users) sbmf::fail(SBMF_E_ARG, "null user list with n > 0");
// ... 352 lines not shown
```

### scalable-bayesian-matrix-factorization_amd/csrc/prepare.cpp

```cpp
#include "ctx.h"

namespace sbmf {

static void build_exchange(Side& s, const Side& other, int nranks, int rank) {
    const uint64_t N = s.perm.size();
    const size_t P = s.stg.size();
    std::vector<uint64_t> obase(nranks + 1);
    for (int k = 0; k <= nranks; ++k) obase[k] = other.ptr[other.bounds[k]];
    auto owner = [&](uint32_t pos) {
        return (int)(std::upper_bound(obase.begin(), obase.end(), (uint64_t)pos) - obase.begin()) - 1;
    };
    size_t off = 0;
    for (size_t p = 0; p < P; ++p) {
        Side::Stage& g = *s.stg[p];
        g.scnt.assign(nranks, 0);
        for (uint64_t idx = s.ptr[g.r0]; idx < s.ptr[g.r1]; ++idx) {
            const int q = owner(s.perm[idx]);
            if (q != rank) g.scnt[q]++;
        }
        g.soff.assign(nranks, 0);
        for (int k = 0; k < nranks; ++k) {
            g.soff[k] = off;
            off += g.scnt[k];
        }
// ... 96 lines not shown
        const uint32_t d = deg(r);
        if (d > stream_thr) {
            g.bin_rows[KIND_STREAM].push_back(r);
            continue;
        }
        int kind = GK_W4;
        while (d > gk_maxdeg(kind, f64, wide)) ++kind;
        g.bin_rows[kind].push_back(r);
    }
}

static void fill_kernel_bytes(sbmf_ctx* c);
static void build_stream_tasks(const Side& s, Side::StreamSet& S, const std::vector<uint32_t>& rows, uint32_t gres,
                               uint32_t nblk);

template <typename T>
void prepare_T(sbmf_ctx* c) {
    const sbmf_config& cf = c->cfg;
    const uint64_t N = c->tu.size();
    if (N >= 0xffffffffull) fail(SBMF_E_ARG, "more than 2^32-1 ratings are not supported");
    c->K = cf.num_factor;
    c->Kp = (c->K + 15) / 16 * 16;
    if ((uint64_t)(std::max(c->I, c->J) + 2) * c->Kp >= 0xffffffffull)
        fail(SBMF_E_ARG, "factor tables of %u x %u rows at K=%u exceed 2^32 elements", c->I, c->J, c->K);

    std::vector<uint32_t> pos_u, pos_v;
    build_side(N, c->tu.data(), c->ti.data(), c->tr.data(), c->I, c->users, pos_u);
    build_side(N, c->ti.data(), c->tu.data(), c->tr.data(), c->J, c->items, pos_v);
    c->users.perm.resize(N);
    c->items.perm.resize(N);
    for (uint64_t x = 0; x < N; ++x) {
        c->users.perm[pos_u[x]] = pos_v[x];
        c->items.perm[pos_v[x]] = pos_u[x];
    }
    c->nstages = c->nranks > 1 ? 2u : 1u;
    if (const char* e = std::getenv("SBMF_STAGES")) c->nstages = std::max(1, std::min(16, std::atoi(e)));
    partition(c->users, c->nranks, c->rank, c->nstages);
    partition(c->items, c->nranks, c->rank, c->nstages);
    if (c->nranks > 1) {
        build_exchange(c->users, c->items, c->nranks, c->rank);
        build_exchange(c->items, c->users, c->nranks, c->rank);
    }
    const bool f64 = sizeof(T) == 8;
    const bool wide = !(cf.tune & 8u);
    const uint32_t gkmax = gk_maxdeg(GK_NUM - 1, f64, wide);
    const uint32_t sthr = std::min<uint32_t>(cf.stream_threshold ? cf.stream_threshold : gkmax, gkmax);
    for (Side* sd : {&c->users, &c->items})
        for (auto& g : sd->stg) build_bins(*sd, *g, sthr, f64, wide);
    for (Side* sd : {&c->users, &c->items})
        for (auto& gp : sd->stg)
        for (int k = GK_B2; k < GK_NUM; ++k) {
            Side::Stage& g = *gp;
            g.gsub[k].clear();
            const std::vector<uint32_t>& rows = g.bin_rows[k];
            const uint32_t per_wave = f64 ? 32 : 64;
            for (uint32_t i = 0; i < rows.size();) {
                const uint32_t d = sd->ptr[rows[i] + 1] - sd->ptr[rows[i]];
                const uint32_t nw = std::max(2u, (d + per_wave - 1) / per_wave);
                uint32_t j = i;
                while (j < rows.size() &&
                       std::max(2u, (sd->ptr[rows[j] + 1] - sd->ptr[rows[j]] + per_wave - 1) / per_wave) == nw)
                    ++j;
                auto shape = [&](uint32_t w) { return f64 && w >= 5 ? 100 + (w + 1) / 2 : w; };
                if (!g.gsub[k].empty() && shape(g.gsub[k].back()[0]) == shape(nw)) {
                    auto& last = g.gsub[k].back();
                    last[2] += j - i;
                } else {
                    g.gsub[k].push_back({nw, i, j - i});
                }
                i = j;
            }
        }
    const uint32_t nblk = (c->K + 15) / 16;
    {
        int dev_cus = 0;
        HIPCHK(hipDeviceGetAttribute(&dev_cus, hipDeviceAttributeMultiprocessorCount, cf.device));
        for (Side* sd : {&c->users, &c->items}) {
            const bool item16 = sd == &c->items && sizeof(T) == 8 && !(cf.tune & (128u | 0x20000u | 0x8000000u));
            const bool user4 = sd == &c->users && sizeof(T) == 8 && !(cf.tune & (128u | 0x20000u | 0x800000u));
            const bool user2 = user4 && (!(cf.tune & 0x2000u) || (cf.tune & 0x4000u));
            const uint32_t stunes[2] = {user4 ? cf.tune | 128u : cf.tune,
                                        user2 && !(cf.tune & 0x4000u) ? cf.tune : cf.tune | 0x20000u};
            for (auto& gp : sd->stg) {
            std::vector<uint32_t> rows[2];
            for (uint32_t r : gp->bin_rows[KIND_STREAM]) {
                const uint32_t d = sd->ptr[r + 1] - sd->ptr[r];
                rows[(item16 && d > 1024u) || (user2 && d > 512u) ? 1 : 0].push_back(r);
            }
            for (int k = 0; k < 2; ++k) {
                Side::StreamSet& S = gp->ss[k];
                S.tune = stunes[k];
                S.cmax = gstream_cmax<T>(S.tune);
                if (cf.split_chunk) S.cmax = std::min(S.cmax, std::max(cf.split_chunk, 1u));
                const int per_cu =
                    std::max(1, std::min(gstream_wg_target(S.tune), gstream_blocks_per_cu<T>(S.cmax, S.tune)));
                build_stream_tasks(*sd, S, rows[k], (uint32_t)(dev_cus * per_cu), nblk);
            }
            }
        }
    }
    {
        const uint64_t T_ = c->su.size(), nb = (T_ + 255) / 256;
        c->tbounds.assign(c->nranks + 1, 0);
        c->tbblocks.assign(c->nranks + 1, 0);
        for (int k = 0; k <= c->nranks; ++k) {
            c->tbblocks[k] = nb * k / c->nranks;
            c->tbounds[k] = std::min<uint64_t>(T_, c->tbblocks[k] * 256);
        }
        c->t0 = c->tbounds[c->rank];
        c->t1 = c->tbounds[c->rank + 1];
    }

    hipStream_t st = c->st;
    upload(c->d_uptr, c->users.ptr, st);
    upload(c->d_upart, c->users.part, st);
    upload(c->d_uperm, c->users.perm, st);
    upload(c->d_ur, to_T<T>(c->users.r), st);
    upload(c->d_vptr, c->items.ptr, st);
    upload(c->d_vpart, c->items.part, st);
    upload(c->d_vperm, c->items.perm, st);
    upload(c->d_vr, to_T<T>(c->items.r), st);
    for (Side* sd : {&c->users, &c->items})
        for (auto& g : sd->stg)
            for (int k = 0; k < NBIN; ++k) upload(g->d_bins[k], g->bin_rows[k], st);
    {
        Side& s = c->items;
        s.rtasks.clear();
        s.rtptr.assign(1, 0);
        for (uint32_t r = s.r0; r < s.r1; ++r) {
            for (uint32_t b = s.ptr[r]; b < s.ptr[r + 1]; b += RESID_CHUNK)
                s.rtasks.push_back(ResidTask{r, b, std::min<uint32_t>(RESID_CHUNK, s.ptr[r + 1] - b), 0});
            s.rtptr.push_back((uint32_t)s.rtasks.size());
        }
        upload(c->d_rtasks, s.rtasks, st);
        upload(c->d_rtptr, s.rtptr, st);
        c->d_rtsq.alloc(std::max<size_t>(s.rtasks.size(), 1) * sizeof(double));
    }
    size_t nxk[2] = {0, 0};
    for (Side* sd : {&c->users, &c->items})
        for (auto& g : sd->stg)
            for (int k = 0; k < 2; ++k) {
                const Side::StreamSet& S = g->ss[k];
                upload(g->d_stasks[k], S.stasks, st);
                upload(g->d_xrows[k], S.xrows, st);
                nxk[k] = std::max<size_t>(nxk[k], S.nxchunk);
            }
    c->xset_nx = std::max<size_t>(nxk[0], 1);
    {
        const size_t nx = c->xset_nx + std::max<size_t>(nxk[1], 1);
        if ((uint64_t)nx * nblk * SLAB_DOUBLES * sizeof(double) >= 0xffffffffull)
            fail(SBMF_E_ARG, "split-row exchange area of %zu chunks at K=%u exceeds 2^32 bytes", nx, c->K);
        c->d_xslabs.alloc(nx * nblk * SLAB_DOUBLES * sizeof(double));
        HIPCHK(hipMemsetAsync(c->d_xslabs.p, 0xff, c->d_xslabs.bytes, st));
        c->d_gcold.alloc((size_t)c->nstages * 6 * sbmf_ctx::kColdSlot);
        c->h_gcold.assign((size_t)c->nstages * 6 * sbmf_ctx::kColdSlot, 0xff);
        c->d_xcnt.alloc(64 * sizeof(uint32_t));
        HIPCHK(hipMemsetAsync(c->d_xcnt.p, 0, c->d_xcnt.bytes, st));
        c->d_xchunk_sq.alloc(nx * sizeof(double));
        c->d_xchunk_tr.alloc(nx * sizeof(double));
        HIPCHK(hipMemsetAsync(c->d_xchunk_tr.p, 0, c->d_xchunk_tr.bytes, st));
        c->d_xnewown.alloc(nx * c->Kp * sizeof(T));
    }
    c->d_U.alloc((size_t)(c->I + 2) * c->Kp * sizeof(T));
    c->d_V.alloc((size_t)(c->J + 2) * c->Kp * sizeof(T));
    HIPCHK(hipMemsetAsync(c->d_U.p, 0, c->d_U.bytes, st));
    HIPCHK(hipMemsetAsync(c->d_V.p, 0, c->d_V.bytes, st));
    c->d_Eu.alloc(std::max<uint64_t>(N + c->items.nsend, 1) * sizeof(T));
    c->d_Ev.alloc(std::max<uint64_t>(N + c->users.nsend, 1) * sizeof(T));
    if (c->nranks > 1) {
        upload(c->d_uperm2, c->users.perm2, st);
        upload(c->d_vperm2, c->items.perm2, st);
        upload(c->d_uunpack, c->users.unpack, st);
        upload(c->d_vunpack, c->items.unpack, st);
        c->d_xrecv.alloc(std::max<size_t>(std::max(c->users.nrecv, c->items.nrecv), 1) * sizeof(T));
        HIPCHK(hipMemsetAsync(c->d_xrecv.p, 0, c->d_xrecv.bytes, st));
    }
    HIPCHK(hipMemsetAsync(c->d_Eu.p, 0, c->d_Eu.bytes, st));
    HIPCHK(hipMemsetAsync(c->d_Ev.p, 0, c->d_Ev.bytes, st));
    c->d_rowsq_u.alloc((size_t)c->I * sizeof(double));
    c->d_rowtr_u.alloc((size_t)c->I * sizeof(double));
    c->d_rowsq_v.alloc((size_t)c->J * sizeof(double));
    c->d_rowtr_v.alloc((size_t)c->J * sizeof(double));
    HIPCHK(hipMemsetAsync(c->d_rowsq_v.p, 0, c->d_rowsq_v.bytes, st));
    HIPCHK(hipMemsetAsync(c->d_rowtr_v.p, 0, c->d_rowtr_v.bytes, st));
    c->d_hyper.alloc((4 * (size_t)c->Kp + 16) * sizeof(T));
    HIPCHK(hipMemsetAsync(c->d_hyper.p, 0, c->d_hyper.bytes, st));
    const uint32_t nchunk = (c->I + 255) / 256 + (c->J + 255) / 256;
    c->d_colpart.alloc((size_t)nchunk * 2 * c->K * sizeof(double));
    c->h_res.assign(RES_COL + 4 * (size_t)c->K, 0.0);
    c->d_res.alloc(c->h_res.size() * sizeof(double));
    HIPCHK(hipMemsetAsync(c->d_res.p, 0, c->d_res.bytes, st));
    pinned_free(c->h_pre, c->h_pre_bytes);
    c->h_pre_bytes = c->h_res.size() * sizeof(double);
    pinned_alloc((void**)&c->h_pre, c->h_pre_bytes);
    pinned_free(c->h_io, c->h_io_bytes);
    c->h_io_bytes = 128 + 4 * (size_t)c->Kp * sizeof(T);
    pinned_alloc(&c->h_io, c->h_io_bytes);
    c->pre.valid = false;
    c->hyper_ahead = false;
    const uint64_t big = std::max<uint64_t>({(uint64_t)c->I, (uint64_t)c->J, c->su.size() / 128 + 2});
    c->d_scratch.alloc((big / 1024 + 16) * 4 * sizeof(double));
    c->scratch_half = (big / 1024 + 16) * 2;
    const uint64_t T_ = c->su.size();
    {
        std::vector<uint64_t> start((size_t)c->I + 1, 0);
        for (uint64_t x = 0; x < T_; ++x) ++start[c->su[x] + 1];
        for (uint32_t u = 0; u < c->I; ++u) start[u + 1] += start[u];
        c->tperm.resize(T_);
        std::vector<uint32_t> su2(T_), si2(T_);
        std::vector<double> sr2(T_);
        for (uint64_t x = 0; x < T_; ++x) {
            const uint64_t j = start[c->su[x]]++;
            c->tperm[j] = x;
            su2[j] = c->su[x];
            si2[j] = c->si[x];
            sr2[j] = c->sr[x];
        }
        upload(c->d_tu, su2, st);
        upload(c->d_ti, si2, st);
        upload(c->d_tr, sr2, st);
        HIPCHK(hipStreamSynchronize(st));
    }
    c->d_tsum.alloc(std::max<uint64_t>(T_, 1) * sizeof(double));
    HIPCHK(hipMemsetAsync(c->d_tsum.p, 0, c->d_tsum.bytes, st));
    c->d_tpart.alloc(((T_ + 255) / 256 + 1) * 2 * sizeof(double));
    HIPCHK(hipMemsetAsync(c->d_tpart.p, 0, c->d_tpart.bytes, st));
    {
        c->d_zU.alloc((size_t)c->I * c->K * sizeof(T));
        c->d_zV.alloc((size_t)c->J * c->K * sizeof(T));
    }
    {
        const size_t nb = c->bias ? 1 : 0;
        for (DBuf* d : {&c->d_bu, &c->d_mbu, &c->d_sbu}) {
            d->alloc(nb * c->I * sizeof(double));
            HIPCHK(hipMemsetAsync(d->p, 0, d->bytes, st));
        }
        for (DBuf* d : {&c->d_bv, &c->d_mbv, &c->d_sbv}) {
            d->alloc(nb * c->J * sizeof(double));
            HIPCHK(hipMemsetAsync(d->p, 0, d->bytes, st));
        }
        const bool refm = cf.rng_mode == SBMF_RNG_REFERENCE;
        c->d_var3u.alloc((refm ? nb : 0) * 3 * c->I * sizeof(double));
        c->d_var3v.alloc((refm ? nb : 0) * 3 * c->J * sizeof(double));
        c->d_epart.alloc(nb * 2 * ((size_t)c->I + 1) * sizeof(double));
        c->empty_u.clear();
        c->empty_v.clear();
        for (uint32_t i = 0; c->bias && i < c->I; ++i)
            if (c->users.ptr[i + 1] == c->users.ptr[i]) c->empty_u.push_back(i);
        for (uint32_t j = 0; c->bias && j < c->J; ++j)
            if (c->items.ptr[j + 1] == c->items.ptr[j]) c->empty_v.push_back(j);
        c->shadow_u.assign(c->empty_u.size(), {0.0, 0.0, 0.0});
        c->shadow_v.assign(c->empty_v.size(), {0.0, 0.0, 0.0});
    }
    const std::vector<double> z(c->K, 0.0);
    c->hyp[0] = c->hyp[1] = Hyper{1.0, 0.0, 0.0, 0.0, z, z, z, z};
    c->reported = 0;

    if (cf.rng_mode == SBMF_RNG_REFERENCE) {
        c->grand.seed_((unsigned)cf.seed);
        std::vector<double> U((size_t)c->I * c->K), V((size_t)c->J * c->K);
        for (uint32_t i = 0; i < c->I; ++i)
            for (uint32_t k = 0; k < c->K; ++k) U[(size_t)i * c->K + k] = 0.0 + c->init_sd * leva_normal(c->grand);
        for (uint32_t k = 0; k < c->K; ++k)
            for (uint32_t j = 0; j < c->J; ++j) V[(size_t)j * c->K + k] = 0.0 + c->init_sd * leva_normal(c->grand);
        HIPCHK(hipStreamSynchronize(st));
        upload_table<T>(c, c->d_U, U.data(), c->I);
        upload_table<T>(c, c->d_V, V.data(), c->J);
    } else {
        HIPCHK(launch_init_philox<T>(c->d_U.as<T>(), c->K, c->Kp, 0, c->I, c->init_sd, cf.seed, TAG_INIT_U, st));
        HIPCHK(launch_init_philox<T>(c->d_V.as<T>(), c->K, c->Kp, 0, c->J, c->init_sd, cf.seed, TAG_INIT_V, st));
    }
    HIPCHK(hipStreamSynchronize(st));
    c->kprof = std::getenv("SBMF_KPROF") && std::atoi(std::getenv("SBMF_KPROF")) > 0;
    if (c->kprof) {
        if (const char* e = std::getenv("SBMF_KPROF_SET")) c->kprof_set = std::atoi(e) ? 1 : 0;
        c->d_kprof.alloc(128 * sizeof(unsigned long long));
        HIPCHK(hipMemset(c->d_kprof.p, 0, 128 * sizeof(unsigned long long)));
    }
    for (hipEvent_t& e : c->kevs) event_destroy(e);
    for (hipEvent_t& e : c->sev) event_destroy(e);
    c->kevs.assign((size_t)c->nstages * 2 * SBMF_NKIND * 2, nullptr);
    c->kprev.assign((size_t)c->nstages * 2 * SBMF_NKIND, (int8_t)-1);
    c->kbegin.assign((size_t)c->nstages * 2 * SBMF_NKIND, nullptr);
    c->sev.assign((size_t)2 * c->nstages, nullptr);
    for (hipEvent_t& e : c->kevs) event_create(&e);
    for (hipEvent_t& e : c->sev) event_create(&e, hipEventDisableTiming);
    for (hipEvent_t& e : c->tsev) event_destroy(e);
    c->tsev.assign(c->virt ? (size_t)2 * (c->nstages + 1) : 0, nullptr);
    for (hipEvent_t& e : c->tsev) event_create(&e);
    c->sweep = 0;
    c->collected = 0;
    fill_kernel_bytes(c);
    c->prepared = true;
}
template void prepare_T<float>(sbmf_ctx*);
template void prepare_T<double>(sbmf_ctx*);

static void build_stream_tasks(const Side& s, Side::StreamSet& S, const std::vector<uint32_t>& rows, uint32_t gres,
                               uint32_t nblk) {
    const uint32_t cmax = S.cmax;
    S.stasks.clear();
    S.xrows.clear();
    S.nxchunk = 0;
    S.sgrid = 0;
    for (uint32_t r : rows) {
        const uint32_t n = s.ptr[r + 1] - s.ptr[r];
        const uint32_t nch = (n + cmax - 1) / cmax;
        if (nch > gres)
            fail(SBMF_E_ARG, "row %u has %u ratings: more than %u co-resident chunks of %u", r, n, gres, cmax);
        if (nch == 1) {
            S.stasks.push_back(SplitTask{r, s.ptr[r], n, 1, 0, 0, 0, 0, 0, {0, 0, 0}});
        } else {
            const uint32_t slab0 = S.nxchunk;
            const uint32_t per = (n + nch - 1) / nch;
            const uint64_t xstr = (uint64_t)nblk * SLAB_DOUBLES * sizeof(double), xrow = (uint64_t)slab0 * xstr;
            if (xrow + (uint64_t)nch * xstr >= 0xffffffffull)
                fail(SBMF_E_ARG, "split-row exchange area exceeds 2^32 bytes at row %u", r);
            for (uint32_t c = 0; c < nch; ++c) {
                const uint32_t b = c * per, e = std::min(n, b + per);
                S.stasks.push_back(SplitTask{r, s.ptr[r] + b, e - b, nch, c, slab0, (uint32_t)xrow,
                                             (uint32_t)(xrow + c * xstr), (uint32_t)xstr, {0, 0, 0}});
            }
            S.xrows.push_back(SplitRow{r, slab0, nch, 0});
            S.nxchunk += nch;
        }
    }
    S.sgrid = std::min<uint32_t>(gres, (uint32_t)S.stasks.size());
}

static uint64_t alg_bytes(const Side& s, const std::vector<uint32_t>& rows, uint32_t K, uint64_t tsz) {
    uint64_t b = 0;
    for (uint32_t r : rows) b += (uint64_t)(s.ptr[r + 1] - s.ptr[r]) * (tsz * K + 4 + tsz) + 2 * tsz * K;
    return b;
}
static void fill_kernel_bytes(sbmf_ctx* c) {
    const uint64_t tsz = tsize(c);
    for (int sd = 0; sd < 2; ++sd) {
        const Side& s = sd == 0 ? c->users : c->items;
        for (int k = 0; k < SBMF_NKIND; ++k) {
            c->timing.kern_bytes[sd][k] = 0;
            c->timing.kern_rows[sd][k] = 0;
        }
        for (const auto& g : s.stg) {
            for (int k = 0; k < NBIN; ++k) {
                c->timing.kern_bytes[sd][k] += alg_bytes(s, g->bin_rows[k], c->K, tsz);
                c->timing.kern_rows[sd][k] += (uint32_t)g->bin_rows[k].size();
            }
        }
    }
}

}
```

### scalable-bayesian-matrix-factorization_amd/csrc/samples.cpp

```cpp
#include "ctx.h"

namespace sbmf {

void samples_ready(sbmf_ctx* c, const char* fn) {
    list_scope(c, "sample store", fn, false);
    if (!c->samples.cap || !c->samples.count)
        fail(SBMF_E_STATE, "%s: no sample kept yet (sbmf_keep_samples, then a collected sweep; or sbmf_load_samples)", fn);
    list_sync(c);
}
size_t slot_bytes(const sbmf_ctx* c) {
    return ((size_t)c->I + c->J) * c->Kp * tsize(c) + (c->bias ? ((size_t)c->I + c->J) * sizeof(double) : 0);
}

}

namespace {

sbmf::SampleView view_of(sbmf_ctx* c, sbmf::DBuf& d_b0, hipStream_t st) {
    const SampleStore& ss = c->samples;
    sbmf::SampleView v;
    v.U = ss.d_U.p;
    v.V = ss.d_V.p;
    v.su = (size_t)c->I * c->Kp;
    v.sv = (size_t)c->J * c->Kp;
// ... 45 lines not shown

constexpr uint64_t kBudget = 1ull << 30;

void guests_ready(sbmf_ctx* c, const char* fn, uint32_t n, const uint32_t* ptr, const uint32_t* items, const double* ratings,
                  uint32_t scans) {
    list_scope(c, "sample store", fn, false);
    if (c->bias)
        sbmf::fail(SBMF_E_STATE, "%s: guests are folded into a store of the unbiased quirk sets (final, sbpmf2, none); a "
                                 "guest bias would need a draw of its own", fn);
    if (scans < 1 || scans > sbmf::SAMPLES_FOLDIN_SCANS_MAX)
        sbmf::fail(SBMF_E_ARG, "%s: scans %u is not in 1..%u", fn, scans, sbmf::SAMPLES_FOLDIN_SCANS_MAX);
    sbmf::GuestCSR::check(fn, n, ptr, items, ratings, c->J);
    samples_ready(c, fn);
    if (!c->samples.has_hyper)
        sbmf::fail(SBMF_E_STATE, "%s: the stored samples have no hyperparameters (a sample file holds none: "
                                 "sbmf_load_samples_hyper loads its companion file)", fn);
}

struct GuestCall {
    sbmf_ctx* c;
    const char* fn;
    uint32_t n, nnz, scans, rows = 0;
    size_t gs = 0;
    sbmf::GuestCSR csr;
    sbmf::DBuf d_hyp, d_tau, d_sw, d_GS, d_S1, d_S2, d_b0;
    sbmf::SamplesFoldinArgs a;

    GuestCall(sbmf_ctx* c_, const char* fn_, uint32_t n_, const uint32_t* ptr, const uint32_t* items, const double* ratings,
              uint32_t scans_, bool sums)
        : c(c_), fn(fn_), n(n_), nnz(n_ ? ptr[n_] - ptr[0] : 0), scans(scans_) {
        const SampleStore& ss = c->samples;
        const uint32_t K = c->K, Kp = c->Kp, Jp = sbmf::watch_jp(c->J), count = ss.count;
        const size_t ts = sbmf::tsize(c);
        const uint64_t budget = ss.budget ? ss.budget : kBudget;
        const uint64_t per = (sums ? (uint64_t)2 * Jp * sizeof(double) : 0) + (uint64_t)count * Kp * ts;
        rows = (uint32_t)std::min<uint64_t>(n, std::max<uint64_t>(budget / per / 64 * 64, 64));
        gs = ((size_t)rows + 2) * Kp;
        const size_t b_GS = (size_t)count * gs * ts, b_sum = sums ? (size_t)rows * Jp * sizeof(double) : 0;
        const size_t b_tot = b_GS + 2 * b_sum + ((size_t)n + 1 + 3 * (size_t)n + nnz + count) * sizeof(uint32_t) +
                             ((size_t)2 * nnz + (size_t)count * (2 * Kp + 1)) * sizeof(double) +
                             (ss.fused_draw ? 0 : (size_t)rows * Kp * sizeof(double));
        try {
            hipStream_t st = c->st;
            std::vector<double> hyp((size_t)count * 2 * Kp, 0.0), tau(count);
            std::vector<uint32_t> sw(count);
            for (uint32_t s = 0; s < count; ++s) {
                const uint32_t p = ss.slot(s);
                const double* h = ss.hyper.data() + (size_t)p * (4 * K + 1);
                std::copy(h, h + K, hyp.begin() + (size_t)s * 2 * Kp);
                std::copy(h + K, h + 2 * K, hyp.begin() + (size_t)s * 2 * Kp + Kp);
                tau[s] = h[4 * K];
                sw[s] = ss.sweep[p];
            }
            d_GS.alloc(b_GS + (ss.fused_draw ? 0 : (size_t)rows * Kp * sizeof(double)));
            if (sums) {
                d_S1.alloc(b_sum);
                d_S2.alloc(b_sum);
            }
            sbmf::upload(d_hyp, hyp, st);
            sbmf::upload(d_tau, tau, st);
            sbmf::upload(d_sw, sw, st);
            a.sv = view_of(c, d_b0, st);
            csr.upload(n, ptr, items, ratings, rows, st);
        } catch (const sbmf::Error& e) {
            if (e.code == SBMF_E_NOMEM)
                sbmf::fail(SBMF_E_NOMEM, "%s: %u guests with %u ratings at %u samples need %zu bytes of device memory: %s", fn,
                           n, nnz, count, b_tot, e.msg.c_str());
            throw;
        }
        a.GS = d_GS.p;
        a.gs = gs;
        a.ptr = csr.d_ptr.as<uint32_t>();
        a.items = csr.d_items.as<uint32_t>();
        a.ratings = csr.d_ratings.as<double>();
        a.K = K;
        a.Kp = Kp;
        a.hyper = d_hyp.as<double>();
        a.tau = d_tau.as<double>();
        a.sweeps = d_sw.as<uint32_t>();
        a.scans = scans;
        a.sd_is_var = c->sd_is_var;
        a.seed = c->cfg.seed;
        a.E = csr.d_E.as<double>();
    }

    template <typename T>
    void draw_T(uint32_t off, uint32_t m) {
        SampleStore& ss = c->samples;
        hipStream_t st = c->st;
        a.n = m;
        a.g0 = off;
        a.order = csr.d_order.as<uint32_t>() + off;
        HIPCHK(hipMemsetAsync(d_GS.p, 0, d_GS.bytes, st));
        ss.gdr.begin(st);
        if (ss.fused_draw) {
            HIPCHK(sbmf::launch_samples_foldin<T>(a, st));
        } else {
            double* carry = reinterpret_cast<double*>(static_cast<char*>(d_GS.p) + (size_t)ss.count * gs * sizeof(T));
            for (uint32_t s = 0; s < ss.count; ++s)
                for (uint32_t r = 0; r < scans; ++r) HIPCHK(sbmf::launch_samples_foldin_step<T>(a, s, r, carry, st));
        }
        ss.gdr.end(st);
    }
    void draw(uint32_t off, uint32_t m) {
        c->cfg.precision == SBMF_F32 ? draw_T<float>(off, m) : draw_T<double>(off, m);
    }
    void score(uint32_t m, int clamp) {
        SampleStore& ss = c->samples;
        sbmf::SampleView v = a.sv;
        v.U = d_GS.p;
        v.su = gs;
        ss.gsc.begin(c->st);
        score_rows(c, v, csr.d_ids.as<uint32_t>(), m, clamp, d_S1.as<double>(), d_S2.as<double>(), c->st);
        ss.gsc.end(c->st);
    }
};

}

void SampleStore::alloc(sbmf_ctx* c, uint32_t cap_, uint32_t every_) {
    const size_t ts = sbmf::tsize(c), I = c->I, J = c->J, Kp = c->Kp;
    d_U.alloc((size_t)cap_ * I * Kp * ts);
    d_V.alloc((size_t)cap_ * J * Kp * ts);
    if (c->bias) {
        d_bu.alloc((size_t)cap_ * I * sizeof(double));
        d_bv.alloc((size_t)cap_ * J * sizeof(double));
    }
    for (sbmf::Span* s : {&cev, &scv, &sel, &gdr, &gsc, &gse}) s->create();
    b0.assign(cap_, 0.0);
    sweep.assign(cap_, 0);
    hyper.assign((size_t)cap_ * (4 * c->K + 1), 0.0);
    has_hyper = true;
    cap = cap_;
    every = every_;
    bytes = (size_t)cap_ * slot_bytes(c);
}
void SampleStore::drop() {
    for (sbmf::DBuf* d : {&d_U, &d_V, &d_bu, &d_bv}) d->release();
    for (sbmf::Span* s : {&cev, &scv, &sel, &gdr, &gsc, &gse}) s->destroy();
    b0.clear();
    sweep.clear();
    hyper.clear();
    has_hyper = false;
    cap = head = count = seen = 0;
    every = 1;
    bytes = 0;
}
template <typename T>
void SampleStore::keep(sbmf_ctx* c, const Hyper& hy, hipStream_t se) {
    if (seen++ % every) return;
    const uint32_t p = count < cap ? slot(count) : head;
    const size_t I = c->I, J = c->J, Kp = c->Kp;
    cev.begin(se);
    HIPCHK(hipMemcpyAsync(d_U.as<T>() + p * I * Kp, c->d_U.p, I * Kp * sizeof(T), hipMemcpyDeviceToDevice, se));
    HIPCHK(hipMemcpyAsync(d_V.as<T>() + p * J * Kp, c->d_V.p, J * Kp * sizeof(T), hipMemcpyDeviceToDevice, se));
    if (c->bias) {
        HIPCHK(hipMemcpyAsync(d_bu.as<double>() + p * I, c->d_bu.p, I * sizeof(double), hipMemcpyDeviceToDevice, se));
        HIPCHK(hipMemcpyAsync(d_bv.as<double>() + p * J, c->d_bv.p, J * sizeof(double), hipMemcpyDeviceToDevice, se));
    }
    cev.end(se);
    b0[p] = hy.b0;
    sweep[p] = c->sweep;
    const size_t K = c->K;
    double* h = hyper.data() + (size_t)p * (4 * K + 1);
    std::copy(hy.sig_u.begin(), hy.sig_u.begin() + K, h);
    std::copy(hy.mu_u.begin(), hy.mu_u.begin() + K, h + K);
    std::copy(hy.sig_v.begin(), hy.sig_v.begin() + K, h + 2 * K);
    std::copy(hy.mu_v.begin(), hy.mu_v.begin() + K, h + 3 * K);
    h[4 * K] = hy.tau;
    if (count < cap) count++;
    else head = (head + 1) % cap;
    c->launches += c->bias ? 4 : 2;
}
template void SampleStore::keep<float>(sbmf_ctx*, const Hyper&, hipStream_t);
template void SampleStore::keep<double>(sbmf_ctx*, const Hyper&, hipStream_t);

extern "C" {

int sbmf_keep_samples(sbmf_ctx* ctx, uint32_t every, uint32_t cap) {
    API_BEGIN
    if (!ctx) sbmf::fail(SBMF_E_ARG, "null context");
    list_scope(ctx, "sample store", "sbmf_keep_samples", false);
    if (every == 0) sbmf::fail(SBMF_E_ARG, "sbmf_keep_samples: every = 0 (1 keeps every collected sweep)");
    if (cap > 65535) sbmf::fail(SBMF_E_ARG, "sbmf_keep_samples: cap %u is above 65535", cap);
    list_sync(ctx);
    ctx->samples.drop();
    if (cap == 0) return SBMF_OK;
    try {
        ctx->samples.alloc(ctx, cap, every);
    } catch (const sbmf::Error& e) {
        ctx->samples.drop();
        if (e.code == SBMF_E_NOMEM)
            sbmf::fail(SBMF_E_NOMEM, "sbmf_keep_samples: %u samples of %zu bytes need %zu bytes of device memory: %s", cap,
                       slot_bytes(ctx), (size_t)cap * slot_bytes(ctx), e.msg.c_str());
        throw;
    } catch (...) {
        ctx->samples.drop();
        throw;
    }
    API_END(ctx)
}

int sbmf_samples_info(sbmf_ctx* ctx, uint32_t* count, uint32_t* cap, uint32_t* every, uint64_t* bytes) {
    API_BEGIN
    if (!ctx) sbmf::fail(SBMF_E_ARG, "null context");
    list_scope(ctx, "sample store", "sbmf_samples_info", false);
    const SampleStore& ss = ctx->samples;
    if (count) *count = ss.count;
    if (cap) *cap = ss.cap;
    if (every) *every = ss.every;
    if (bytes) *bytes = ss.bytes;
    API_END(ctx)
}

int sbmf_get_sample(sbmf_ctx* ctx, uint32_t s, uint32_t* sweep, double* U, double* V, double* bu, double* bv, double* b0) {
    API_BEGIN
    if (!ctx) sbmf::fail(SBMF_E_ARG, "null context");
    samples_ready(ctx, "sbmf_get_sample");
    const SampleStore& ss = ctx->samples;
    if (s >= ss.count) sbmf::fail(SBMF_E_ARG, "sbmf_get_sample: sample %u of %u kept", s, ss.count);
    const uint32_t p = ss.slot(s);
    const size_t I = ctx->I, J = ctx->J;
    if (sweep) *sweep = ss.sweep[p];
    if (b0) *b0 = ctx->bias ? ss.b0[p] : 0.0;
    const size_t K = ctx->K, Kp = ctx->Kp;
    auto table = [&](auto type, const sbmf::DBuf& d, size_t R, double* out) {
        using T = decltype(type);
        std::vector<T> h(R * Kp);
        HIPCHK(hipMemcpy(h.data(), d.as<T>() + (size_t)p * R * Kp, R * Kp * sizeof(T), hipMemcpyDeviceToHost));
        for (size_t r = 0; r < R; ++r)
            for (size_t k = 0; k < K; ++k) out[r * K + k] = (double)h[r * Kp + k];
    };
    const bool f32 = ctx->cfg.precision == SBMF_F32;
    if (U) f32 ? table(float{}, ss.d_U, I, U) : table(double{}, ss.d_U, I, U);
    if (V) f32 ? table(float{}, ss.d_V, J, V) : table(double{}, ss.d_V, J, V);
    auto biases = [&](const sbmf::DBuf& d, size_t R, double* out) {
        if (ctx->bias)
            HIPCHK(hipMemcpy(out, d.as<double>() + (size_t)p * R, R * sizeof(double), hipMemcpyDeviceToHost));
        else
            std::fill(out, out + R, 0.0);
    };
    if (bu) biases(ss.d_bu, I, bu);
    if (bv) biases(ss.d_bv, J, bv);
    API_END(ctx)
}

int sbmf_samples_recommend(sbmf_ctx* ctx, uint32_t n, const uint32_t* users, uint32_t topn, uint32_t flags, double risk,
                           uint32_t* items, double* mean, double* stdev) {
    API_BEGIN
    const char* fn = "sbmf_samples_recommend";
    if (!ctx) sbmf::fail(SBMF_E_ARG, "null context");
    list_scope(ctx, "sample store", fn, false);
    if (n && (!users || !items || !mean)) sbmf::fail(SBMF_E_ARG, "%s: null argument", fn);
    if (topn < 1 || topn > 1024) sbmf::fail(SBMF_E_ARG, "%s: topn %u is not in 1..1024", fn, topn);
    if (flags & ~3u)
        sbmf::fail(SBMF_E_ARG, "%s: unknown flags 0x%x (bit 0 = keep rated items, bit 1 = clamp)", fn, flags & ~3u);
    if (!(risk == risk)) sbmf::fail(SBMF_E_ARG, "%s: risk is NaN", fn);
    check_users(ctx, fn, n, users);
    samples_ready(ctx, fn);
    if (n == 0) return SBMF_OK;
    SampleStore& ss = ctx->samples;
    hipStream_t st = ctx->st;
    const uint32_t J = ctx->J, Jp = sbmf::watch_jp(J);
    const bool exclude = !(flags & 1u);
    const int clamp = (flags & 2u) ? 1 : 0;
    const uint64_t budget = ss.budget ? ss.budget : kBudget;
    const uint64_t fit = budget / ((uint64_t)2 * Jp * sizeof(double)) / 64 * 64;
    const uint32_t rows = (uint32_t)std::min<uint64_t>(n, std::max<uint64_t>(fit, 64));
    sbmf::DBuf d_b0, d_ids, d_S1, d_S2;
    sbmf::TopnScratch t;
    const sbmf::SampleView v = view_of(ctx, d_b0, st);
    d_ids.alloc((size_t)rows * sizeof(uint32_t));
    d_S1.alloc((size_t)rows * Jp * sizeof(double));
    d_S2.alloc((size_t)rows * Jp * sizeof(double));
    t.alloc(rows, topn, J, exclude);
    for (uint32_t off = 0; off < n; off += rows) {
        const uint32_t m = std::min(rows, n - off);
        const size_t o = (size_t)off * topn;
        HIPCHK(hipMemcpyAsync(d_ids.p, users + off, (size_t)m * sizeof(uint32_t), hipMemcpyHostToDevice, st));
        ss.scv.begin(st);
        score_rows(ctx, v, d_ids.as<uint32_t>(), m, clamp, d_S1.as<double>(), d_S2.as<double>(), st);
        ss.scv.end(st);
        sbmf::select_topn(t, d_ids.as<uint32_t>(), m, d_S1.as<double>(), d_S2.as<double>(), J, ss.count,
                          exclude ? ctx->d_uptr.as<uint32_t>() : nullptr, ctx->d_upart.as<uint32_t>(), topn, risk, ss.sel, st,
                          items + o, mean + o, stdev ? stdev + o : nullptr);
    }
    API_END(ctx)
}

int sbmf_samples_scores(sbmf_ctx* ctx, uint32_t user, uint32_t flags, double* mean, double* stdev) {
    API_BEGIN
    const char* fn = "sbmf_samples_scores";
    if (!ctx || !mean) sbmf::fail(SBMF_E_ARG, "null argument");
    list_scope(ctx, "sample store", fn, false);
    if (flags & ~2u) sbmf::fail(SBMF_E_ARG, "%s: unknown flags 0x%x (bit 1 = clamp)", fn, flags & ~2u);
    check_users(ctx, fn, 1, &user);
    samples_ready(ctx, fn);
    SampleStore& ss = ctx->samples;
    hipStream_t st = ctx->st;
    const uint32_t J = ctx->J, Jp = sbmf::watch_jp(J);
    sbmf::DBuf d_b0, d_id, d_S;
    const sbmf::SampleView v = view_of(ctx, d_b0, st);
    d_id.alloc(sizeof(uint32_t));
    d_S.alloc((size_t)2 * Jp * sizeof(double));
    double* S = d_S.as<double>();
    HIPCHK(hipMemcpyAsync(d_id.p, &user, sizeof(uint32_t), hipMemcpyHostToDevice, st));
    ss.scv.begin(st);
// ... 200 lines not shown
```

### scalable-bayesian-matrix-factorization_amd/csrc/sbmf.cpp

```cpp
#include "ctx.h"

namespace {
thread_local std::string g_err;
}

namespace sbmf {

[[noreturn]] void comm_fail(const char* what, ncclResult_t r) {
    fail(SBMF_E_COMM, "%s failed: %s", what, rccl_error_string((int)r));
}

Audit& audit() {
    static Audit a;
    return a;
}

}

sbmf_ctx::~sbmf_ctx() {
    vbo_destroy(vb);
    delete fm;
    using namespace sbmf;
    pinned_free(h_pinned, h_pinned_bytes);
    pinned_free(h_pre, h_pre_bytes);
    pinned_free(h_io, h_io_bytes);
    for (hipEvent_t& e : ev) event_destroy(e);
    for (hipEvent_t& e : kevs) event_destroy(e);
    for (hipEvent_t& e : sev) event_destroy(e);
    for (hipEvent_t& e : tsev) event_destroy(e);
    for (hipEvent_t& e : cev) event_destroy(e);
    for (hipEvent_t& e : oev) event_destroy(e);
    for (hipEvent_t& e : wev) event_destroy(e);
    for (hipEvent_t& e : fev) event_destroy(e);
    for (ScoreList* l : {&watch, &guests, &fmq}) l->drop();
    fmqd.drop();
    samples.drop();
    pinned_free(h_fhyp, h_fhyp_bytes);
    event_destroy(hev);
    stream_destroy(sto);
    stream_destroy(sto2);
    stream_destroy(stc);
    stream_destroy(st);
    audit().contexts--;
}

namespace sbmf {
template <typename T>
void rccl_selftest(sbmf_ctx* c, uint64_t nbytes, uint32_t reps, double deadline_s, sbmf_rccl_selftest* out) {
    *out = sbmf_rccl_selftest{};
    Comm loop;
    loop.init_loopback();
    const size_t n = (size_t)nbytes, nag = n / 4;
    std::vector<uint8_t> pa(n), pb(n), pc(nag);
    for (size_t x = 0; x < n; ++x) {
        pa[x] = (uint8_t)(x * 2654435761u >> 13);
        pb[x] = (uint8_t)(x * 40503u + 17u);
    }
    for (size_t x = 0; x < nag; ++x) pc[x] = (uint8_t)(x * 97u + 5u);
    DBuf blk, snd, rcv, ags, agr;
    blk.alloc(n);
    snd.alloc(n);
    rcv.alloc(n);
    ags.alloc(nag);
    agr.alloc(nag);
    HIPCHK(hipMemcpy(blk.p, pa.data(), n, hipMemcpyHostToDevice));
    HIPCHK(hipMemcpy(snd.p, pb.data(), n, hipMemcpyHostToDevice));
    HIPCHK(hipMemcpy(ags.p, pc.data(), nag, hipMemcpyHostToDevice));
    HIPCHK(hipDeviceSynchronize());
    struct Events {
        hipEvent_t e[4] = {};
        bool keep = false;
        ~Events() {
            if (!keep)
                for (hipEvent_t& x : e) event_destroy(x);
        }
    } evs;
    hipEvent_t* e = evs.e;
    for (int x = 0; x < 4; ++x) event_create(&e[x]);
    const std::vector<uint64_t> b0{0}, b1{n / 3}, b2{2 * (n / 3)}, b3{n};
    const std::vector<size_t> soff{0}, scnt{n / 2}, roff{n / 2}, rcnt{n / 2};
    const std::vector<size_t> soff2{n / 2}, scnt2{n / 2}, roff2{0}, rcnt2{n / 2};
    HIPCHK(hipEventRecord(e[0], c->st));
    for (uint32_t r = 0; r < reps; ++r) {
        run_half<T>(c, c->hyp[c->reported], false, 0);
        if (r == 0) HIPCHK(hipEventRecord(e[2], c->stc));
        loop.group_begin();
        loop.bcast_blocks(blk.p, 1, b0, b1, c->stc);
        loop.bcast_blocks(blk.p, 1, b1, b2, c->stc);
        loop.bcast_blocks(blk.p, 1, b2, b3, c->stc);
        loop.group_end();
        loop.alltoallv(snd.p, r & 1 ? soff2 : soff, r & 1 ? scnt2 : scnt, rcv.p, r & 1 ? roff2 : roff,
                       r & 1 ? rcnt2 : rcnt, c->stc);
        loop.allgather(ags.p, nag, agr.p, c->stc);
        out->n_calls += 3 + 2 + 1;
    }
    HIPCHK(hipEventRecord(e[1], c->st));
    HIPCHK(hipEventRecord(e[3], c->stc));
    const auto t0 = std::chrono::steady_clock::now();
    for (;;) {
        const hipError_t q = hipEventQuery(e[3]);
        if (q == hipSuccess) break;
        if (q != hipErrorNotReady) fail(SBMF_E_COMM, "RCCL self-test: %s", hipGetErrorString(q));
        if (std::chrono::duration<double>(std::chrono::steady_clock::now() - t0).count() > deadline_s) {
            loop.abort();
            evs.keep = true;
            for (DBuf* b : {&blk, &snd, &rcv, &ags, &agr}) b->leak();
            c->dead = true;
            fail(SBMF_E_COMM, "RCCL self-test: the comm stream did not finish within %.1f s (communicator aborted, "
                              "context unusable)", deadline_s);
        }
        std::this_thread::sleep_for(std::chrono::microseconds(200));
    }
    HIPCHK(hipEventSynchronize(e[1]));
    float f = 0.f;
    HIPCHK(hipEventElapsedTime(&f, e[0], e[1]));
    out->ms_half = f;
    HIPCHK(hipEventElapsedTime(&f, e[2], e[3]));
    out->ms_rccl = f;
    HIPCHK(hipEventElapsedTime(&f, e[0], e[3]));
    out->ms_rccl_end = f;
    std::vector<uint8_t> h(n);
    HIPCHK(hipMemcpy(h.data(), blk.p, n, hipMemcpyDeviceToHost));
    for (size_t x = 0; x < n; ++x) out->bad_bcast += h[x] != pa[x];
    HIPCHK(hipMemcpy(h.data(), rcv.p, n, hipMemcpyDeviceToHost));
    for (size_t x = 0; x < n; ++x) {
        if (x < n / 2 && reps == 1) continue;
        out->bad_p2p += h[x] != pb[x < n / 2 ? x + n / 2 : x - n / 2];
    }
    h.resize(nag);
    HIPCHK(hipMemcpy(h.data(), agr.p, nag, hipMemcpyDeviceToHost));
    for (size_t x = 0; x < nag; ++x) out->bad_allgather += h[x] != pc[x];
    out->overlapped = out->ms_rccl_end < out->ms_half ? 1u : 0u;
}
}

int sbmf::api_error(sbmf_ctx* ctx) {
    int code = SBMF_E_ARG;
    try {
        throw;
    } catch (const sbmf::Error& e) {
        g_err = e.msg;
        code = e.code;
    } catch (const std::bad_alloc&) {
        g_err = "host allocation failed";
        code = SBMF_E_NOMEM;
    } catch (const std::exception& e) {
        g_err = e.what();
    }
    if (ctx) ctx->err = g_err;
    return code;
}

extern "C" {

int sbmf_abi_version(void) { return SBMF_ABI_VERSION; }

namespace {
int g_exit_rc = 1;
bool g_exit_guarded = false;
void exit_guard_handler() {
    std::fflush(nullptr);
    std::_Exit(g_exit_rc);
}
}
int sbmf_exit_guard(int rc) {
    g_exit_rc = rc;
    if (g_exit_guarded) return SBMF_OK;
    if (std::atexit(exit_guard_handler) != 0) {
        g_err = "sbmf_exit_guard: atexit failed";
        return SBMF_E_STATE;
    }
    g_exit_guarded = true;
    return SBMF_OK;
}

int sbmf_config_default(sbmf_config* c) {
    if (!c) return SBMF_E_ARG;
    std::memset(c, 0, sizeof *c);
    c->num_factor = 20;
    c->num_iter = 100;
    c->burnin = 0;
    c->seed = 1;
    c->rng_mode = SBMF_RNG_REFERENCE;
    c->quirks = SBMF_QUIRKS_FINAL;
    c->precision = SBMF_F64;
    c->device = 0;
    c->init_stdev = -1.0;
    c->clamp_lo = -1.0;
    c->clamp_hi = 5.0;
    c->a0 = 1;
    c->b0 = 1;
    c->alpha0 = 1;
    c->beta0 = 1;
    c->nu0 = 1;
    c->mu0 = 0.0;
    c->recompute_every = 1;
    c->eval_train = 0;
    c->eval_test = 1;
    c->libfm_dim = 3;
    return SBMF_OK;
}

const char* sbmf_last_error(const sbmf_ctx* ctx) { return ctx ? ctx->err.c_str() : g_err.c_str(); }
const char* sbmf_last_global_error(void) { return g_err.c_str(); }

int sbmf_create(const sbmf_config* cfg, sbmf_ctx** out) {
    sbmf_ctx* ctx = nullptr;
    API_BEGIN
    if (!cfg || !out) sbmf::fail(SBMF_E_ARG, "null argument");
    *out = nullptr;
    if (cfg->num_factor == 0 || cfg->num_factor > 256) sbmf::fail(SBMF_E_ARG, "num_factor must be in [1,256]");
    if (cfg->rng_mode != SBMF_RNG_REFERENCE && cfg->rng_mode != SBMF_RNG_PHILOX) sbmf::fail(SBMF_E_ARG, "bad rng_mode");
    if (cfg->quirks < 0 || cfg->quirks > 4) sbmf::fail(SBMF_E_ARG, "bad quirks");
    if (cfg->average > 2) sbmf::fail(SBMF_E_ARG, "bad average (0 default, 1 collected sweeps, 2 sweep + 1)");
    if (cfg->precision != SBMF_F64 && cfg->precision != SBMF_F32) sbmf::fail(SBMF_E_ARG, "bad precision");
    if (cfg->method > SBMF_METHOD_ALS) sbmf::fail(SBMF_E_ARG, "bad method");
    if (cfg->method == SBMF_METHOD_VB && cfg->precision != SBMF_F64)
        sbmf::fail(SBMF_E_ARG, "the online VB learner computes in f64 (the reference's double) only");
    if ((cfg->method == SBMF_METHOD_LIBFM_MCMC || cfg->method == SBMF_METHOD_ALS) && cfg->precision != SBMF_F64)
        sbmf::fail(SBMF_E_ARG, "the libFM MCMC / ALS learner computes in f64 (the reference's double) only");
    if (cfg->libfm_dim > 3) sbmf::fail(SBMF_E_ARG, "bad libfm_dim (bit 0 = w0, bit 1 = w)");
    if (cfg->task > SBMF_TASK_CLASSIFICATION) sbmf::fail(SBMF_E_ARG, "bad task (0 regression, 1 classification)");
    if (cfg->task == SBMF_TASK_CLASSIFICATION && cfg->method != SBMF_METHOD_LIBFM_MCMC && cfg->method != SBMF_METHOD_ALS) {
        static const char* const names[] = {"mcmc (the SBPMF sampler)", "vb (online VB)"};
        sbmf::fail(SBMF_E_ARG, "classification (task = SBMF_TASK_CLASSIFICATION) is libFM's MCMC / ALS learner's "
                               "(SBMF_METHOD_LIBFM_MCMC, SBMF_METHOD_ALS); method %s fits real-valued targets only",
                   names[cfg->method]);
    }
    {
        constexpr uint32_t known = (1u << 1) | (1u << 2) | (1u << 3) | (1u << 7) | (1u << 8) | (1u << 9) | (1u << 10) |
                                   (1u << 11) | (1u << 12) | (1u << 13) | (1u << 14) | (1u << 17) |
                                   (1u << 23) | (1u << 24) | (1u << 25) | (1u << 26) | (1u << 27) | (1u << 28) |
                                   (1u << 29) | (1u << 30);
        if (cfg->tune & ~known)
            sbmf::fail(SBMF_E_ARG, "tune bits 0x%x have no meaning in this build (variants removed earlier; see "
                                   "include/sbmf.h and INTEGRATION.md)", cfg->tune & ~known);
    }
    if (cfg->gram_threshold || cfg->row_kernel)
        sbmf::fail(SBMF_E_ARG, "gram_threshold / row_kernel are reserved (must be 0): the per-coordinate and "
                               "full-Gram row kernels were removed (measured slower than the Gram-block kernels)");
    int ndev = 0;
    const hipError_t derr = hipGetDeviceCount(&ndev);
    if (derr != hipSuccess || ndev <= 0)
        sbmf::fail(SBMF_E_DEVICE, "no HIP device available (%s; this library has no CPU fallback)",
                   derr != hipSuccess ? hipGetErrorString(derr) : "0 devices");
    if (cfg->device < 0 || cfg->device >= ndev) sbmf::fail(SBMF_E_DEVICE, "device %d out of range (%d)", cfg->device, ndev);
    hipDeviceProp_t prop;
    HIPCHK(hipGetDeviceProperties(&prop, cfg->device));
    if (std::strncmp(prop.gcnArchName, "gfx950", 6) != 0)
        sbmf::fail(SBMF_E_DEVICE, "device %d is %s; this build targets gfx950 (MI355X)", cfg->device, prop.gcnArchName);
    HIPCHK(hipSetDevice(cfg->device));
    std::unique_ptr<sbmf_ctx> c(new sbmf_ctx());
    c->cfg = *cfg;
    const bool q2 = cfg->quirks == SBMF_QUIRKS_SBPMF2 || cfg->quirks == SBMF_QUIRKS_BIAS2;
    c->bias = cfg->quirks == SBMF_QUIRKS_BIAS2 || cfg->quirks == SBMF_QUIRKS_BIAS22;
    if (c->bias && (cfg->tune & 2u))
        sbmf::fail(SBMF_E_ARG, "tune bit 1 (residuals from r - own.partner) does not carry biases");
    c->init_sd = cfg->init_stdev >= 0 ? cfg->init_stdev : (q2 ? 0.1 : 1.0);
    c->lo = cfg->clamp_lo >= 0 ? cfg->clamp_lo : (q2 ? 0.5 : 1.0);
    c->hi = cfg->clamp_hi;
    c->sd_is_var = cfg->quirks == SBMF_QUIRKS_NONE ? 0 : 1;
    sbmf::stream_create(&c->st);
    sbmf::stream_create(&c->stc);
    for (auto& e : c->ev) sbmf::event_create(&e);
    for (auto& e : c->cev) sbmf::event_create(&e, hipEventDisableTiming);
    sbmf::stream_create(&c->sto);
    sbmf::stream_create(&c->sto2);
    for (auto& e : c->oev) sbmf::event_create(&e, hipEventDisableTiming);
    sbmf::event_create(&c->hev, hipEventDisableTiming);
    *out = c.release();
    API_END(ctx)
}

void sbmf_destroy(sbmf_ctx* ctx) {
    if (!ctx || ctx->dead) return;
    (void)hipSetDevice(ctx->cfg.device);
    (void)hipStreamSynchronize(ctx->st);
    delete ctx;
}

static bool libfm_method(const sbmf_ctx* c) {
    return c->cfg.method == SBMF_METHOD_LIBFM_MCMC || c->cfg.method == SBMF_METHOD_ALS;
}

static void prepare_cases(sbmf_ctx* c, bool triples) {
    if (c->nranks > 1 || c->virt || c->comm != &c->own_comm || c->own_comm.active())
        sbmf::fail(SBMF_E_STATE, "the general libFM learner (cases with any number of features) runs on one rank: "
                                 "this context joined a communicator or is a virtual rank");
    c->K = c->cfg.num_factor;
    c->fm = fmg_create(c->cfg, c->ctr.view(), c->cte.view(), c->st, &c->fmgroups, &c->fmrels);
    if (triples) {
        c->fm->I = c->I;
        c->fm->J = c->J;
    }
    c->prepared = true;
}

static void triples_to_cases(const std::vector<uint32_t>& u, const std::vector<uint32_t>& i, const std::vector<double>& r,
                             uint32_t I, sbmf_ctx::HostCases& out) {
    const size_t n = u.size();
    out.ptr.resize(n + 1);
    out.attr.resize(2 * n);
    out.x.assign(2 * n, 1.0f);
    out.y.resize(n);
    uint32_t mx = 0;
    for (size_t q = 0; q < n; ++q) {
        if ((uint64_t)I + i[q] > 0xfffffffdull) sbmf::fail(SBMF_E_ARG, "attribute id too large");
        out.ptr[q] = 2 * q;
        out.attr[2 * q] = u[q];
        out.attr[2 * q + 1] = I + i[q];
        mx = std::max(mx, I + i[q]);
        out.y[q] = (float)r[q];
    }
    out.ptr[n] = 2 * n;
    out.num_attr = n ? mx + 1 : 0;
    out.set = true;
}

static void prepare_ctx(sbmf_ctx* c) {
    if (c->ctr.set) {
        prepare_cases(c, false);
        return;
    }
    if (c->cte.set) sbmf::fail(SBMF_E_STATE, "sbmf_set_test_cases without sbmf_set_train_cases");
    if (c->tu.empty()) sbmf::fail(SBMF_E_STATE, "no training data (sbmf_set_train)");
    uint32_t umax = 0, imax = 0;
    for (size_t x = 0; x < c->tu.size(); ++x) {
        umax = std::max(umax, c->tu[x]);
        imax = std::max(imax, c->ti[x]);
    }
    for (size_t x = 0; x < c->su.size(); ++x) {
        umax = std::max(umax, c->su[x]);
        imax = std::max(imax, c->si[x]);
    }
    c->I = std::max(c->I_req, umax + 1);
    c->J = std::max(c->J_req, imax + 1);
    c->K = c->cfg.num_factor;
    if (c->cfg.method == SBMF_METHOD_MCMC) {
        c->cfg.precision == SBMF_F32 ? prepare_T<float>(c) : prepare_T<double>(c);
        return;
    }
    sbmf::Comm* comm = c->nranks > 1 ? c->comm : nullptr;
    const char* gen = std::getenv("SBMF_FMM_GENERAL");
    const bool grouped = !c->fmgroups.group.empty() || !c->fmgroups.regw.empty() || !c->fmrels.empty();
    if (libfm_method(c) && ((gen && std::atoi(gen) != 0) || grouped)) {
        triples_to_cases(c->tu, c->ti, c->tr, c->I, c->ctr);
        triples_to_cases(c->su, c->si, c->sr, c->I, c->cte);
        prepare_cases(c, true);
        return;
    }
    if (c->cfg.method == SBMF_METHOD_VB)
        c->vb = vbo_create(c->cfg, c->tu.size(), c->tu.data(), c->ti.data(), c->tr.data(), c->su.size(), c->su.data(),
                           c->si.data(), c->sr.data(), c->I, c->J, c->st, comm);
    else
        c->fm = fmm_create(c->cfg, c->tu.size(), c->tu.data(), c->ti.data(), c->tr.data(), c->su.size(), c->su.data(),
                           c->si.data(), c->sr.data(), c->I, c->J, c->st, comm);
    c->prepared = true;
}

static void set_triples(uint64_t n, const uint32_t* u, const uint32_t* i, const double* r, std::vector<uint32_t>& U,
                        std::vector<uint32_t>& I, std::vector<double>& R) {
    if (n && (!u || !i || !r)) sbmf::fail(SBMF_E_ARG, "null array with n > 0");
    U.assign(u, u + n);
    I.assign(i, i + n);
    R.assign(r, r + n);
}

int sbmf_set_train(sbmf_ctx* ctx, uint64_t n, const uint32_t* user, const uint32_t* item, const double* rating) {
    API_BEGIN
    if (!ctx) sbmf::fail(SBMF_E_ARG, "null context");
    if (ctx->prepared) sbmf::fail(SBMF_E_STATE, "data already prepared");
    if (ctx->ctr.set || ctx->cte.set) sbmf::fail(SBMF_E_STATE, "the context already holds cases (sbmf_set_train_cases)");
    set_triples(n, user, item, rating, ctx->tu, ctx->ti, ctx->tr);
    API_END(ctx)
}

int sbmf_set_test(sbmf_ctx* ctx, uint64_t n, const uint32_t* user, const uint32_t* item, const double* rating) {
    API_BEGIN
    if (!ctx) sbmf::fail(SBMF_E_ARG, "null context");
    if (ctx->prepared) sbmf::fail(SBMF_E_STATE, "data already prepared");
    if (ctx->ctr.set || ctx->cte.set) sbmf::fail(SBMF_E_STATE, "the context already holds cases (sbmf_set_test_cases)");
    set_triples(n, user, item, rating, ctx->su, ctx->si, ctx->sr);
    API_END(ctx)
}

static void set_cases(const sbmf_cases* in, sbmf_ctx::HostCases& out, const char* fn) {
    if (!in) sbmf::fail(SBMF_E_ARG, "%s: null cases", fn);
    if ((in->n && (!in->ptr || !in->target)) || (in->nnz && (!in->attr || !in->x)))
        sbmf::fail(SBMF_E_ARG, "%s: null array", fn);
    if (in->n && (in->ptr[0] != 0 || in->ptr[in->n] != in->nnz))
        sbmf::fail(SBMF_E_ARG, "%s: ptr must run from 0 to nnz", fn);
    sbmf_ctx::HostCases h;
    h.ptr.assign(in->n + 1, 0);
    if (in->n) h.ptr.assign(in->ptr, in->ptr + in->n + 1);
    h.attr.assign(in->attr, in->attr + in->nnz);
    h.x.assign(in->x, in->x + in->nnz);
    h.y.assign(in->target, in->target + in->n);
    h.num_attr = in->num_attr;
    std::vector<std::pair<uint32_t, float>> tmp;
    for (uint64_t c = 0; c < in->n; ++c) {
        const uint64_t b = h.ptr[c], e = h.ptr[c + 1];
        if (e < b || e > in->nnz) sbmf::fail(SBMF_E_ARG, "%s: ptr decreases at case %llu", fn, (unsigned long long)c);
        bool sorted = true;
        for (uint64_t k = b; k < e; ++k) {
            if (h.attr[k] >= in->num_attr)
                sbmf::fail(SBMF_E_ARG, "%s: case %llu holds attribute %u >= num_attr %u", fn, (unsigned long long)c,
                           h.attr[k], in->num_attr);
            if (k > b && h.attr[k - 1] >= h.attr[k]) sorted = false;
        }
        if (sorted) continue;
        tmp.clear();
        for (uint64_t k = b; k < e; ++k) tmp.emplace_back(h.attr[k], h.x[k]);
        std::stable_sort(tmp.begin(), tmp.end(), [](const auto& a, const auto& b2) { return a.first < b2.first; });
        for (uint64_t k = b; k < e; ++k) {
            h.attr[k] = tmp[k - b].first;
            h.x[k] = tmp[k - b].second;
            if (k > b && h.attr[k - 1] == h.attr[k])
                sbmf::fail(SBMF_E_ARG, "%s: case %llu repeats attribute %u (the learner writes one record per case of "
                                       "a row)", fn, (unsigned long long)c, h.attr[k]);
        }
    }
    h.set = true;
// ... 221 lines not shown
    if (!ctx || !out) sbmf::fail(SBMF_E_ARG, "null argument");
    if (!ctx->prepared) sbmf::fail(SBMF_E_STATE, "not prepared");
    if (!ctx->fm || !ctx->fm->nranges)
        sbmf::fail(SBMF_E_STATE, "sbmf_test_fm_group_sums: this context does not run the general libFM learner");
    HIPCHK(hipSetDevice(ctx->cfg.device));
    ctx->fm->group_sums(out);
    API_END(ctx)
}

int sbmf_test_tgauss(int mode, int device, uint64_t seed, uint32_t it, uint64_t n, const double* mean, const int32_t* sign,
                     const uint32_t* index, double* out) {
    sbmf_ctx* ctx = nullptr;
    API_BEGIN
    if (n && (!mean || !sign || !out)) sbmf::fail(SBMF_E_ARG, "null argument");
    if (mode == 1) {
        sbmf::GlibcRand g((unsigned)seed);
        for (uint64_t i = 0; i < n; ++i)
            out[i] = sign[i] >= 0 ? sbmf::ran_left_tgaussian(g, 0.0, mean[i], 1.0)
                                  : sbmf::ran_right_tgaussian(g, 0.0, mean[i], 1.0);
    } else if (mode == 0) {
        if (n >= 0xffffffffull) sbmf::fail(SBMF_E_ARG, "more than 2^32-1 draws");
        int ndev = 0;
        const hipError_t derr = hipGetDeviceCount(&ndev);
        if (derr != hipSuccess || ndev <= 0)
            sbmf::fail(SBMF_E_DEVICE, "no HIP device available (%s; this library has no CPU fallback)",
                       derr != hipSuccess ? hipGetErrorString(derr) : "0 devices");
        if (device < 0 || device >= ndev) sbmf::fail(SBMF_E_DEVICE, "device %d out of range (%d)", device, ndev);
        HIPCHK(hipSetDevice(device));
        std::vector<float> y(n);
        for (uint64_t i = 0; i < n; ++i) y[i] = sign[i] >= 0 ? 1.0f : -1.0f;
        sbmf::DBuf d_mean, d_y, d_out, d_idx;
        if (index && n) {
            d_idx.alloc(n * sizeof(uint32_t));
            HIPCHK(hipMemcpy(d_idx.p, index, n * sizeof(uint32_t), hipMemcpyHostToDevice));
        }
        d_mean.alloc(std::max<uint64_t>(n, 1) * sizeof(double));
        d_y.alloc(std::max<uint64_t>(n, 1) * sizeof(float));
        d_out.alloc(std::max<uint64_t>(n, 1) * sizeof(double));
        if (n) {
            HIPCHK(hipMemcpy(d_mean.p, mean, n * sizeof(double), hipMemcpyHostToDevice));
            HIPCHK(hipMemcpy(d_y.p, y.data(), n * sizeof(float), hipMemcpyHostToDevice));
            HIPCHK(sbmf::fm_tgauss(seed, it, n, d_mean.as<double>(), d_y.as<float>(), d_idx.as<uint32_t>(), d_out.as<double>(),
                                   nullptr));
            HIPCHK(hipDeviceSynchronize());
            HIPCHK(hipMemcpy(out, d_out.p, n * sizeof(double), hipMemcpyDeviceToHost));
        }
    } else {
        sbmf::fail(SBMF_E_ARG, "sbmf_test_tgauss: mode %d (0 device, 1 host)", mode);
    }
    API_END(ctx)
}

int sbmf_fm_ranges(const sbmf_cases* train, uint32_t num_attr, uint32_t* bounds, uint32_t cap, uint32_t* nranges) {
    sbmf_ctx* ctx = nullptr;
    API_BEGIN
    if (!train || !nranges) sbmf::fail(SBMF_E_ARG, "null argument");
    if ((train->n && !train->ptr) || (train->nnz && !train->attr)) sbmf::fail(SBMF_E_ARG, "null array");
    if (train->n && train->ptr[train->n] != train->nnz) sbmf::fail(SBMF_E_ARG, "ptr[n] != nnz");
    for (uint64_t k = 0; k < train->nnz; ++k)
        if (train->attr[k] >= num_attr) sbmf::fail(SBMF_E_ARG, "attribute %u >= num_attr %u", train->attr[k], num_attr);
    std::vector<uint32_t> b;
    sbmf::fm_ranges(*train, num_attr, b);
    *nranges = (uint32_t)b.size() - 1;
    if (bounds) {
        if (cap < b.size()) sbmf::fail(SBMF_E_ARG, "bounds holds %u values, %zu needed", cap, b.size());
        std::copy(b.begin(), b.end(), bounds);
    }
    API_END(ctx)
}

int sbmf_set_dims(sbmf_ctx* ctx, uint32_t num_users, uint32_t num_items) {
    API_BEGIN
    if (!ctx) sbmf::fail(SBMF_E_ARG, "null context");
    if (ctx->prepared) sbmf::fail(SBMF_E_STATE, "data already prepared");
    ctx->I_req = num_users;
    ctx->J_req = num_items;
    API_END(ctx)
}

int sbmf_prepare(sbmf_ctx* ctx) {
    API_BEGIN
    if (!ctx) sbmf::fail(SBMF_E_ARG, "null context");
    HIPCHK(hipSetDevice(ctx->cfg.device));
    if (ctx->prepared) return SBMF_OK;
    for (size_t x = 0; x < ctx->tu.size(); ++x)
        if ((ctx->I_req && ctx->tu[x] >= ctx->I_req) || (ctx->J_req && ctx->ti[x] >= ctx->J_req))
            sbmf::fail(SBMF_E_ARG, "rating %zu has an id beyond sbmf_set_dims", x);
    prepare_ctx(ctx);
    API_END(ctx)
}

int sbmf_run(sbmf_ctx* ctx, uint32_t sweeps, sbmf_sweep_cb cb, void* user) {
    API_BEGIN
    if (!ctx) sbmf::fail(SBMF_E_ARG, "null context");
    if (ctx->spent || ctx->dead)
        sbmf::fail(SBMF_E_STATE, "sbmf_test_rccl_selftest ran extra item halves on this context: its chain is no "
                                 "longer the sampler's; create a new context");
    HIPCHK(hipSetDevice(ctx->cfg.device));
    if (!ctx->prepared) prepare_ctx(ctx);
    if (ctx->vb) {
        vbo_run(ctx->vb, sweeps, cb, user);
        ctx->timing = sbmf_timing{};
        ctx->timing.n_launch = vbo_launches(ctx->vb);
        ctx->timing.ms_vb_factor = vbo_factor_ms(ctx->vb);
        return SBMF_OK;
    }
    if (ctx->fm) {
        ctx->fm->run(sweeps, cb, user);
        ctx->timing = sbmf_timing{};
        ctx->timing.n_launch = ctx->fm->n_launch;
        return SBMF_OK;
    }
    ctx->cfg.precision == SBMF_F32 ? run_sweeps_T<float>(ctx, sweeps, cb, user) : run_sweeps_T<double>(ctx, sweeps, cb, user);
    API_END(ctx)
}

int sbmf_predict(sbmf_ctx* ctx, double* out) {
    API_BEGIN
    if (!ctx || !out) sbmf::fail(SBMF_E_ARG, "null argument");
    if (!ctx->prepared) sbmf::fail(SBMF_E_STATE, "not prepared");
    HIPCHK(hipSetDevice(ctx->cfg.device));
    if (ctx->vb) {
        vbo_predict_out(ctx->vb, out);
        return SBMF_OK;
    }
    if (ctx->fm) {
        ctx->fm->predict_out(out);
        return SBMF_OK;
    }
    const uint64_t T_ = ctx->su.size();
    if (ctx->nranks > 1) ctx->comm->bcast_ranges(ctx->d_tsum.p, sizeof(double), ctx->tbounds, ctx->st);
    HIPCHK(hipStreamSynchronize(ctx->st));
    std::vector<double> h(T_);
    HIPCHK(hipMemcpy(h.data(), ctx->d_tsum.p, T_ * sizeof(double), hipMemcpyDeviceToHost));
    const double div = sbmf::avg_collected(ctx->cfg) ? (double)std::max(1u, ctx->collected) : (double)std::max(1u, ctx->sweep);
    for (uint64_t j = 0; j < T_; ++j) out[ctx->tperm[j]] = h[j] / div;
    API_END(ctx)
}

int sbmf_get_factors(sbmf_ctx* ctx, double* U, double* V) {
    API_BEGIN
    if (!ctx) sbmf::fail(SBMF_E_ARG, "null context");
    if (!ctx->prepared) sbmf::fail(SBMF_E_STATE, "not prepared");
    HIPCHK(hipSetDevice(ctx->cfg.device));
    HIPCHK(hipStreamSynchronize(ctx->st));
    if (ctx->vb) {
        vbo_factors(ctx->vb, U, V);
        return SBMF_OK;
    }
    if (ctx->fm) {
        ctx->fm->factors(U, V);
        return SBMF_OK;
    }
    if (U) sbmf::download_table(ctx, ctx->d_U, U, ctx->I);
    if (V) sbmf::download_table(ctx, ctx->d_V, V, ctx->J);
    API_END(ctx)
}

int sbmf_set_factors(sbmf_ctx* ctx, const double* U, const double* V) {
    API_BEGIN
    if (!ctx) sbmf::fail(SBMF_E_ARG, "null context");
    if (!ctx->prepared) sbmf::fail(SBMF_E_STATE, "not prepared");
    if (ctx->vb || ctx->fm)
        sbmf::fail(SBMF_E_STATE, "sbmf_set_factors is not supported by the VB / libFM learners");
    HIPCHK(hipSetDevice(ctx->cfg.device));
    HIPCHK(hipStreamSynchronize(ctx->st));
    ctx->pre.valid = false;
    if (U) sbmf::upload_table(ctx, ctx->d_U, U, ctx->I);
    if (V) sbmf::upload_table(ctx, ctx->d_V, V, ctx->J);
    API_END(ctx)
}

int sbmf_get_hyper(sbmf_ctx* ctx, double* h, double* tau) {
    API_BEGIN
    if (!ctx) sbmf::fail(SBMF_E_ARG, "null context");
    if (!ctx->prepared) sbmf::fail(SBMF_E_STATE, "not prepared");
    if (ctx->vb) {
        HIPCHK(hipSetDevice(ctx->cfg.device));
        vbo_hyper_out(ctx->vb, h, tau);
        return SBMF_OK;
    }
    if (ctx->fm) {
        ctx->fm->hyper_out(h, tau);
        return SBMF_OK;
    }
    const uint32_t K = ctx->K;
    const Hyper& hy = ctx->hyp[ctx->reported];
    if (h) {
        std::copy(hy.sig_u.begin(), hy.sig_u.end(), h);
        std::copy(hy.mu_u.begin(), hy.mu_u.end(), h + K);
        std::copy(hy.sig_v.begin(), hy.sig_v.end(), h + 2 * K);
        std::copy(hy.mu_v.begin(), hy.mu_v.end(), h + 3 * K);
    }
    if (tau) *tau = hy.tau;
    API_END(ctx)
}

int sbmf_get_biases(sbmf_ctx* ctx, double* bu, double* bv, double* b0) {
    API_BEGIN
    if (!ctx) sbmf::fail(SBMF_E_ARG, "null context");
    if (!ctx->prepared) sbmf::fail(SBMF_E_STATE, "not prepared");
    HIPCHK(hipSetDevice(ctx->cfg.device));
    if (ctx->vb) {
        vbo_biases(ctx->vb, bu, bv, b0);
        return SBMF_OK;
    }
    if (ctx->fm) {
        ctx->fm->biases(bu, bv, b0);
        return SBMF_OK;
    }
    if (!ctx->bias) sbmf::fail(SBMF_E_STATE, "not a biased sampler (quirks bias2 / bias22) or the VB learner");
    HIPCHK(hipStreamSynchronize(ctx->st));
    if (bu) HIPCHK(hipMemcpy(bu, ctx->d_bu.p, (size_t)ctx->I * sizeof(double), hipMemcpyDeviceToHost));
    if (bv) HIPCHK(hipMemcpy(bv, ctx->d_bv.p, (size_t)ctx->J * sizeof(double), hipMemcpyDeviceToHost));
    if (b0) *b0 = ctx->hyp[ctx->reported].b0;
    API_END(ctx)
}

int sbmf_get_dims(sbmf_ctx* ctx, uint32_t* nu, uint32_t* ni, uint64_t* ntr, uint64_t* nte) {
    API_BEGIN
    if (!ctx) sbmf::fail(SBMF_E_ARG, "null context");
    if (nu) *nu = ctx->I;
    if (ni) *ni = ctx->J;
    const bool cases = ctx->ctr.set && ctx->tu.empty();
    if (ntr) *ntr = cases ? ctx->ctr.y.size() : ctx->tu.size();
    if (nte) *nte = cases ? ctx->cte.y.size() : ctx->su.size();
    API_END(ctx)
}

int sbmf_get_timing(sbmf_ctx* ctx, sbmf_timing* t) {
    API_BEGIN
    if (!ctx || !t) sbmf::fail(SBMF_E_ARG, "null argument");
    *t = ctx->timing;
    const uint64_t s = sbmf::tsize(ctx);
    const uint64_t N = ctx->tu.size();
    t->bytes_algorithmic = 2 * N * (s * ctx->K + 4 + s) + ((uint64_t)ctx->I + ctx->J) * 2 * s * ctx->K;
    API_END(ctx)
}

int sbmf_comm_unique_id(uint8_t id[128]) {
    sbmf_ctx* ctx = nullptr;
    API_BEGIN
    if (!id) sbmf::fail(SBMF_E_ARG, "null id");
    sbmf::Comm::unique_id(id);
    API_END(ctx)
}

int sbmf_comm_init(sbmf_ctx* ctx, int nranks, int rank, const uint8_t id[128]) {
    API_BEGIN
    if (!ctx || !id) sbmf::fail(SBMF_E_ARG, "null argument");
    if (ctx->prepared) sbmf::fail(SBMF_E_STATE, "sbmf_comm_init must precede sbmf_prepare");
    if (nranks < 1 || rank < 0 || rank >= nranks) sbmf::fail(SBMF_E_ARG, "bad rank %d / %d", rank, nranks);
    HIPCHK(hipSetDevice(ctx->cfg.device));
    ctx->nranks = nranks;
    ctx->rank = rank;
    if (ctx->comm != &ctx->own_comm) sbmf::fail(SBMF_E_STATE, "context already attached to a communicator");
    if (nranks > 1) ctx->comm->init(nranks, rank, id);
    API_END(ctx)
}

struct sbmf_comm {
    sbmf::Comm c;
    int device = 0, nranks = 1, rank = 0;
};

int sbmf_comm_create(int device, int nranks, int rank, const uint8_t id[128], sbmf_comm** out) {
    sbmf_ctx* ctx = nullptr;
    API_BEGIN
    if (!id || !out) sbmf::fail(SBMF_E_ARG, "null argument");
    *out = nullptr;
    if (nranks < 1 || rank < 0 || rank >= nranks) sbmf::fail(SBMF_E_ARG, "bad rank %d / %d", rank, nranks);
    if (device < 0) sbmf::fail(SBMF_E_ARG, "bad device %d", device);
    std::unique_ptr<sbmf_comm> cm(new sbmf_comm());
    cm->device = device;
    cm->nranks = nranks;
    cm->rank = rank;
    if (nranks > 1) {
        HIPCHK(hipSetDevice(device));
        cm->c.init(nranks, rank, id);
    }
    *out = cm.release();
    API_END(ctx)
}

int sbmf_comm_attach(sbmf_ctx* ctx, sbmf_comm* comm) {
    API_BEGIN
    if (!ctx || !comm) sbmf::fail(SBMF_E_ARG, "null argument");
    if (ctx->prepared) sbmf::fail(SBMF_E_STATE, "sbmf_comm_attach must precede sbmf_prepare");
    if (ctx->own_comm.active() || ctx->virt) sbmf::fail(SBMF_E_STATE, "context already joined a communicator");
    if (comm->nranks > 1 && comm->device != ctx->cfg.device)
        sbmf::fail(SBMF_E_ARG, "communicator on device %d, context on device %d", comm->device, ctx->cfg.device);
    ctx->nranks = comm->nranks;
    ctx->rank = comm->rank;
    ctx->comm = &comm->c;
    API_END(ctx)
}

void sbmf_comm_destroy(sbmf_comm* comm) { delete comm; }

int sbmf_test_virtual_rank(sbmf_ctx* ctx, int nranks, int rank) {
    API_BEGIN
    if (!ctx) sbmf::fail(SBMF_E_ARG, "null context");
    if (ctx->prepared) sbmf::fail(SBMF_E_STATE, "sbmf_test_virtual_rank must precede sbmf_prepare");
    if (nranks < 2 || rank < 0 || rank >= nranks) sbmf::fail(SBMF_E_ARG, "bad rank %d / %d", rank, nranks);
    if (ctx->cfg.method != SBMF_METHOD_MCMC) sbmf::fail(SBMF_E_ARG, "virtual ranks: the SBPMF sampler only");
    if (ctx->comm->active() || ctx->comm != &ctx->own_comm)
        sbmf::fail(SBMF_E_STATE, "context already joined a communicator");
    ctx->nranks = nranks;
    ctx->rank = rank;
    ctx->virt = true;
    API_END(ctx)
}

int sbmf_test_stage_ms(sbmf_ctx* ctx, double* ms, uint32_t cap, uint32_t* nstages) {
    API_BEGIN
    if (!ctx || !nstages) sbmf::fail(SBMF_E_ARG, "null argument");
    if (!ctx->virt || !ctx->prepared) sbmf::fail(SBMF_E_STATE, "stage times need a prepared virtual rank");
    *nstages = ctx->nstages;
    if (ms && cap < 2 * ctx->nstages) sbmf::fail(SBMF_E_ARG, "need %u slots", 2 * ctx->nstages);
    HIPCHK(hipStreamSynchronize(ctx->st));
    for (uint32_t sd = 0; ms && sd < 2; ++sd)
// ... 88 lines not shown
```

### scalable-bayesian-matrix-factorization_amd/csrc/sweep.cpp

```cpp
#include "ctx.h"

namespace sbmf {

struct HostStream {
    double g_tau;
    double g_sb0 = 0, z_mb0 = 0, z_b0 = 0;
    std::vector<double> g_su, z_mu, g_sv, z_mv;
};

template <class G>
static void draw_hyper_variates(G& g, sbmf_ctx* c, HostStream& hs) {
    const sbmf_config& cf = c->cfg;
    const uint64_t N = c->tu.size();
    if (c->bias) {
        hs.g_tau = mt_gamma(g, cf.a0 + (double)N);
        hs.g_sb0 = mt_gamma(g, cf.alpha0 + 1);
        hs.z_mb0 = leva_normal(g);
        hs.z_b0 = leva_normal(g);
    } else {
        hs.g_tau = mt_gamma(g, cf.a0 + 0.5 * (double)N);
    }
    hs.g_su.resize(c->K);
    hs.z_mu.resize(c->K);
    hs.g_sv.resize(c->K);
    hs.z_mv.resize(c->K);
    const double shu = c->bias ? cf.alpha0 + c->I : cf.alpha0 + 0.5 * (c->I + 1);
    const double shv = c->bias ? cf.alpha0 + c->J : cf.alpha0 + 0.5 * (c->J + 1);
    for (uint32_t k = 0; k < c->K; ++k) {
        hs.g_su[k] = mt_gamma(g, shu);
        hs.z_mu[k] = leva_normal(g);
        hs.g_sv[k] = mt_gamma(g, shv);
        hs.z_mv[k] = leva_normal(g);
    }
}

template <typename T>
static void fill_bias_variates(sbmf_ctx* c, const Hyper& hy) {
    const uint32_t K = c->K;
    const sbmf_config& cf = c->cfg;
    auto sdv = [&](double var) { return c->sd_is_var ? var : std::sqrt(var); };
    auto consumes = [](double sd) { return !(sd == 0.0 || std::isnan(sd)); };
    auto hyper_rows = [&](uint32_t R, const std::vector<uint32_t>& empty, std::vector<std::array<double, 3>>& sh,
                          std::vector<double>& v) {
        size_t e = 0;
        for (uint32_t r = 0; r < R; ++r) {
            const double g = mt_gamma(c->grand, cf.alpha0 + 1);
            v[3 * (size_t)r] = g;
            if (e < empty.size() && empty[e] == r) {
                std::array<double, 3>& x = sh[e++];
                x[2] = g / (cf.beta0 + (0.5 * (x[0] - x[1]) * (x[0] - x[1])));
                const double s4 = 1.0 / (cf.nu0 + x[2]);
                const double mean = s4 * ((cf.nu0 * cf.mu0) + x[0] * x[2]);
                const double z = consumes(sdv(s4)) ? leva_normal(c->grand) : 0.0;
                v[3 * (size_t)r + 1] = z;
                x[1] = consumes(sdv(s4)) ? mean + sdv(s4) * z : mean;
            } else {
                v[3 * (size_t)r + 1] = leva_normal(c->grand);
            }
        }
    };
    auto bias_draw = [&](const std::vector<uint32_t>& empty, std::vector<std::array<double, 3>>& sh, uint32_t r,
                         size_t& e) -> double {
        if (e < empty.size() && empty[e] == r) {
            std::array<double, 3>& x = sh[e++];
            const double sb = 1 / (x[2] + (hy.tau * 0.0));
            const double mb = sb * ((x[2] * x[1]) + hy.tau * 0.0);
            if (!consumes(sdv(sb))) {
                x[0] = mb;
                return 0.0;
            }
            const double z = leva_normal(c->grand);
            x[0] = mb + sdv(sb) * z;
            return z;
        }
        return leva_normal(c->grand);
    };
    std::vector<double> vu((size_t)3 * c->I), vv((size_t)3 * c->J);
    hyper_rows(c->I, c->empty_u, c->shadow_u, vu);
    hyper_rows(c->J, c->empty_v, c->shadow_v, vv);
    const size_t nz = ((size_t)c->I + c->J) * K;
    ensure_pinned(c, nz * sizeof(T));
    T* h = reinterpret_cast<T*>(c->h_pinned);
    size_t e = 0;
    for (uint32_t i = 0; i < c->I; ++i) {
        vu[3 * (size_t)i + 2] = bias_draw(c->empty_u, c->shadow_u, i, e);
        for (uint32_t k = 0; k < K; ++k) h[(size_t)i * K + k] = (T)leva_normal(c->grand);
    }
    T* hv = h + (size_t)c->I * K;
    e = 0;
    for (uint32_t j = 0; j < c->J; ++j) {
        vv[3 * (size_t)j + 2] = bias_draw(c->empty_v, c->shadow_v, j, e);
        for (uint32_t k = 0; k < K; ++k) hv[(size_t)j * K + k] = (T)leva_normal(c->grand);
    }
    HIPCHK(hipMemcpy(c->d_zU.p, h, (size_t)c->I * K * sizeof(T), hipMemcpyHostToDevice));
    HIPCHK(hipMemcpy(c->d_zV.p, hv, (size_t)c->J * K * sizeof(T), hipMemcpyHostToDevice));
    HIPCHK(hipMemcpy(c->d_var3u.p, vu.data(), vu.size() * sizeof(double), hipMemcpyHostToDevice));
    HIPCHK(hipMemcpy(c->d_var3v.p, vv.data(), vv.size() * sizeof(double), hipMemcpyHostToDevice));
}

static BiasArgs bias_args(const sbmf_ctx* c, const Hyper& hy, bool users, double d0) {
    BiasArgs p{};
    p.alpha = hy.tau;
    p.d0 = d0;
    p.ag = c->cfg.alpha0;
    p.bg = c->cfg.beta0;
    p.sg = c->cfg.nu0;
    p.mg = c->cfg.mu0;
    p.seed = c->cfg.seed;
    p.sweep = c->sweep;
    p.tag = users ? TAG_BIAS_U : TAG_BIAS_V;
    p.sd_is_var = c->sd_is_var;
    return p;
}

template <typename T>
static void fill_z(sbmf_ctx* c, uint32_t R, DBuf& d) {
    const size_t n = (size_t)R * c->K;
    ensure_pinned(c, n * sizeof(T));
    T* h = reinterpret_cast<T*>(c->h_pinned);
    for (size_t x = 0; x < n; ++x) h[x] = (T)leva_normal(c->grand);
    HIPCHK(hipMemcpy(d.p, h, n * sizeof(T), hipMemcpyHostToDevice));
}

template <typename T>
static HalfArgs<T> half_args(sbmf_ctx* c, const Hyper& hy, bool users) {
    HalfArgs<T> a{};
    const bool md = c->nranks > 1;
    if (users) {
        a.ptr = c->d_uptr.as<uint32_t>();
        a.part = c->d_upart.as<uint32_t>();
        a.perm = (md ? c->d_uperm2 : c->d_uperm).as<uint32_t>();
        a.E_this = c->d_Eu.as<T>();
        a.E_other = c->d_Ev.as<T>();
        a.r_this = c->d_ur.as<T>();
        a.own = c->d_U.as<T>();
        a.partner = c->d_V.as<T>();
        a.sig = c->d_hyper.as<T>();
        a.mu = c->d_hyper.as<T>() + c->Kp;
        a.zrow = c->J;
        a.zbuf = c->d_zU.as<T>();
        a.tag = TAG_USERS;
        a.row_sq = nullptr;
        a.row_tr = nullptr;
    } else {
        a.ptr = c->d_vptr.as<uint32_t>();
        a.part = c->d_vpart.as<uint32_t>();
        a.perm = (md ? c->d_vperm2 : c->d_vperm).as<uint32_t>();
        a.E_this = c->d_Ev.as<T>();
        a.E_other = c->d_Eu.as<T>();
        a.r_this = c->d_vr.as<T>();
        a.own = c->d_V.as<T>();
        a.partner = c->d_U.as<T>();
        a.sig = c->d_hyper.as<T>() + 2 * c->Kp;
        a.mu = c->d_hyper.as<T>() + 3 * c->Kp;
        a.zrow = c->I;
        a.zbuf = c->d_zV.as<T>();
        a.tag = TAG_ITEMS;
        a.row_sq = c->d_rowsq_v.as<double>();
        a.row_tr = c->cfg.eval_train ? c->d_rowtr_v.as<double>() : nullptr;
    }
    a.tune = c->cfg.tune;
    a.prof = c->kprof ? c->d_kprof.as<unsigned long long>() + 16 + 8 * (users ? 0 : 1) : nullptr;
    a.tau = (T)hy.tau;
    a.K = c->K;
    a.Kp = c->Kp;
    a.sd_is_var = c->sd_is_var;
    a.seed = c->cfg.seed;
    a.sweep = c->sweep;
    a.lo = (T)c->lo;
    a.hi = (T)c->hi;
    a.lim_partner = (uint64_t)((users ? c->J : c->I) + 2) * c->Kp;
    a.lim_other = (uint64_t)c->tu.size() + (users ? c->users.nsend : c->items.nsend);
    a.lim_this = c->tu.size();
    a.lim_rows = users ? c->I : c->J;
    a.e_from_dot = (c->cfg.tune & 2u) ? 1 : 0;
    return a;
}

template <typename T>
static const GresCold<T>* cold_block(sbmf_ctx* c, int slot, const GresCold<T>& cold) {
    static_assert(sizeof(GresCold<T>) <= sbmf_ctx::kColdSlot, "cold block slot");
    unsigned char* h = c->h_gcold.data() + (size_t)slot * sbmf_ctx::kColdSlot;
    unsigned char* d = c->d_gcold.as<unsigned char>() + (size_t)slot * sbmf_ctx::kColdSlot;
    if (std::memcmp(h, &cold, sizeof(cold)) != 0) {
        for (hipStream_t s : {c->st, c->sto, c->sto2}) HIPCHK(hipStreamSynchronize(s));
        HIPCHK(hipMemcpy(d, &cold, sizeof(cold), hipMemcpyHostToDevice));
        std::memcpy(h, &cold, sizeof(cold));
        static const bool log = std::getenv("SBMF_COLD_LOG") != nullptr;
        if (log) std::fprintf(stderr, "[sbmf] cold block upload: slot %d, sweep %u\n", slot, c->sweep);
    }
    return reinterpret_cast<const GresCold<T>*>(d);
}

template <typename T>
void run_half(sbmf_ctx* c, const Hyper& hy, bool users, uint32_t stage, hipEvent_t start) {
    Side& s = users ? c->users : c->items;
    Side::Stage& g = *s.stg[stage];
    HalfArgs<T> a = half_args<T>(c, hy, users);
    hipStream_t st = c->st;
    const int sd = users ? 0 : 1;
    int others = 0;
    for (int k = 0; k < NBIN; ++k) others += k != KIND_STREAM && !g.bin_rows[k].empty();
    const bool serial = (c->cfg.tune & 0x20000000u) != 0;
    const bool ovl = !serial && others && !g.bin_rows[KIND_STREAM].empty();
    static const uint64_t kSetsSideMin = [] {
        const char* e = std::getenv("SBMF_SETS_SIDE_MIN");
        return e ? (uint64_t)std::strtoull(e, nullptr, 10) : (uint64_t)4000000;
    }();
    const bool big = (uint64_t)(s.ptr[g.r1] - s.ptr[g.r0]) >= kSetsSideMin;
    const bool sov = ovl && big && !(c->cfg.tune & 0x40000000u) && !g.ss[0].stasks.empty() && !g.ss[1].stasks.empty();
    const bool two = !serial && (others >= 2 || sov) && !(c->cfg.tune & 0x2000000u);
    const bool side = ovl || two;
    bool st_busy = false;
    auto fork = [&] {
        hipEvent_t f = start && !st_busy ? start : c->oev[0];
        if (f == c->oev[0]) HIPCHK(hipEventRecord(c->oev[0], c->st));
        HIPCHK(hipStreamWaitEvent(c->sto, f, 0));
        if (two) HIPCHK(hipStreamWaitEvent(c->sto2, f, 0));
    };
    if (side) fork();
    int last[3] = {-1, -1, -1};
    int nside = 0;
    for (int k = NBIN - 1; k >= 0; --k) {
        if (g.bin_rows[k].empty()) continue;
        st = side && k != KIND_STREAM ? (two && (sov || (nside++ & 1)) ? c->sto2 : c->sto) : c->st;
        const bool timed = c->time_kinds || k == KIND_STREAM;
        int& lk = last[st == c->st ? 0 : st == c->sto ? 1 : 2];
        if (timed) {
            c->kpv(stage, sd, k) = (int8_t)lk;
            if (lk < 0) {
                if (st == c->st && start && !st_busy) {
                    c->kbg(stage, sd, k) = start;
                } else {
                    HIPCHK(hipEventRecord(c->kev(stage, sd, k, 0), st));
                    c->kbg(stage, sd, k) = c->kev(stage, sd, k, 0);
                }
            }
            lk = k;
        } else {
            lk = -1;
        }
        const uint32_t tn = c->cfg.tune;
        const bool g32 = sizeof(T) == 4 && !(tn & 0x800u);
        const int gw = g32 ? (k == GK_W16 || k == GK_B2 || k == GK_B4 ? 1 : k == GK_B8 ? 2 : 0)
                       : sizeof(T) != 8                               ? 0
                       : k == GK_B4 && !(tn & 0x100u)                 ? 1
                       : k == GK_B8 && !(tn & 0x200u)                 ? 2
                       : k == GK_W16 && !(tn & 0x400u) && !(tn & 8u)  ? 1
                                                                      : 0;
        if (gw) {
            HIPCHK(launch_grow<T>(gw, g.d_bins[k].as<uint32_t>(), (uint32_t)g.bin_rows[k].size(), a,
                                  cold_block<T>(c, (2 * (int)stage + sd) * 3 + 2, gres_cold<T>(a, nullptr)), st));
        } else if (k < GK_NUM && k >= GK_B2 && !(c->cfg.tune & 4u)) {
            for (const auto& gs : g.gsub[k])
                HIPCHK(launch_gblock_nw<T>((int)gs[0], g.d_bins[k].as<uint32_t>() + gs[1], gs[2], a, st));
        } else if (k < GK_NUM)
            HIPCHK(launch_gblock<T>(k, g.d_bins[k].as<uint32_t>(), (uint32_t)g.bin_rows[k].size(), a, st));
        else {
            for (int q = 0; q < 2; ++q) {
                const int set = sov ? 1 - q : q;
                const Side::StreamSet& S = g.ss[set];
                if (S.stasks.empty()) continue;
                const hipStream_t ss = sov && set == 0 ? c->sto : st;
                const size_t ox = set ? c->xset_nx : 0;
                SplitSync sy{};
                sy.nblk = (c->K + 15) / 16;
                sy.slabs = c->d_xslabs.as<double>() + ox * sy.nblk * SLAB_DOUBLES;
                sy.qhead = c->d_xcnt.as<uint32_t>() + 32 * set;
                sy.chunk_sq = c->d_xchunk_sq.as<double>() + ox;
                sy.chunk_tr = c->d_xchunk_tr.as<double>() + ox;
                sy.newown = c->d_xnewown.as<T>() + ox * c->Kp;
                sy.timeout = reinterpret_cast<uint32_t*>(c->d_res.as<double>() + RES_TIMEOUT);
                sy.cmax = S.cmax;
                sy.lim_slab = (uint64_t)(c->d_xslabs.bytes / sizeof(double)) - ox * sy.nblk * SLAB_DOUBLES;
                sy.lim_chunk = (uint32_t)(c->d_xchunk_sq.bytes / sizeof(double) - ox);
                sy.prof = c->kprof && set == c->kprof_set ? c->d_kprof.as<unsigned long long>() + 8 * (users ? 0 : 1) : nullptr;
                HalfArgs<T> as = a;
                as.tune = S.tune;
                HIPCHK(launch_gstream<T>(g.d_stasks[set].as<SplitTask>(), (uint32_t)S.stasks.size(), S.sgrid,
                                         g.d_xrows[set].as<SplitRow>(), (uint32_t)S.xrows.size(), as, sy,
                                         cold_block<T>(c, (2 * (int)stage + sd) * 3 + set, gres_cold<T>(as, &sy)), ss));
                if (ss == c->st) st_busy = true;
            }
            if (sov) {
                HIPCHK(hipEventRecord(c->oev[2], c->sto));
                HIPCHK(hipStreamWaitEvent(st, c->oev[2], 0));
            }
        }
        if (st == c->st) st_busy = true;
        if (timed) HIPCHK(hipEventRecord(c->kev(stage, sd, k, 1), st));
        c->launches++;
    }
    if (side) {
        HIPCHK(hipEventRecord(c->oev[1], c->sto));
        HIPCHK(hipStreamWaitEvent(c->st, c->oev[1], 0));
        if (two) {
            HIPCHK(hipEventRecord(c->oev[3], c->sto2));
            HIPCHK(hipStreamWaitEvent(c->st, c->oev[3], 0));
        }
    }
}

template <typename T, class F>
static void exchange_stage(sbmf_ctx* c, bool users, uint32_t p, hipStream_t st, F&& with) {
    if (c->nranks <= 1) return;
    const Side& s = users ? c->users : c->items;
    const Side::Stage& g = *s.stg[p];
    DBuf& E = users ? c->d_Ev : c->d_Eu;
    auto rel = [](const std::vector<size_t>& v, size_t base) {
        std::vector<size_t> b(v);
        for (size_t& x : b) x = (x - base) * sizeof(T);
        return b;
    };
    auto bytes = [](const std::vector<size_t>& v) {
        std::vector<size_t> b(v);
        for (size_t& x : b) x *= sizeof(T);
        return b;
    };
    c->comm->group_begin();
    with(p);
    c->comm->group_end();
    const size_t s0 = g.soff.empty() ? 0 : g.soff[0];
    c->comm->alltoallv(E.as<T>() + c->tu.size() + s0, rel(g.soff, s0), bytes(g.scnt), c->d_xrecv.as<T>() + g.rbeg,
                      rel(g.roff, g.rbeg), bytes(g.rcnt), st);
    HIPCHK(launch_unpack<T>(c->d_xrecv.as<T>() + g.rbeg, (users ? c->d_uunpack : c->d_vunpack).as<uint32_t>() + g.rbeg,
                            g.rend - g.rbeg, E.as<T>(), st));
}
template <typename T>
static void exchange_residuals(sbmf_ctx* c, bool users, hipStream_t st) {
    for (uint32_t p = 0; p < c->nstages; ++p) exchange_stage<T>(c, users, p, st, [](uint32_t) {});
}
static void bcast_stage(sbmf_ctx* c, const Side& s, uint32_t p, void* base, size_t unit_bytes) {
    std::vector<uint64_t> lo(c->nranks), hi(c->nranks);
    for (int k = 0; k < c->nranks; ++k) {
        lo[k] = s.sbounds[k][p];
        hi[k] = s.sbounds[k][p + 1];
    }
    c->comm->bcast_blocks(base, unit_bytes, lo, hi, c->stc);
}
template <typename T, class F>
static void run_half_pipelined(sbmf_ctx* c, const Hyper& hy, bool users, F&& bcasts, hipEvent_t start = nullptr) {
    const int sd = users ? 0 : 1;
    const size_t tb = (size_t)sd * (c->nstages + 1);
    if (c->virt) HIPCHK(hipEventRecord(c->tsev[tb], c->st));
    for (uint32_t p = 0; p < c->nstages; ++p) {
        run_half<T>(c, hy, users, p, p == 0 && !c->virt ? start : nullptr);
        if (c->nranks > 1) HIPCHK(hipEventRecord(c->sev[(size_t)sd * c->nstages + p], c->st));
        if (c->virt) HIPCHK(hipEventRecord(c->tsev[tb + p + 1], c->st));
    }
    HIPCHK(hipEventRecord(c->ev[users ? 2 : 4], c->st));
    if (c->nranks <= 1) return;
    for (uint32_t p = 0; p < c->nstages; ++p) {
        HIPCHK(hipStreamWaitEvent(c->stc, c->sev[(size_t)sd * c->nstages + p], 0));
        exchange_stage<T>(c, users, p, c->stc, bcasts);
    }
    HIPCHK(hipEventRecord(c->cev[sd], c->stc));
    HIPCHK(hipStreamWaitEvent(c->st, c->cev[sd], 0));
}

static void kprof_report(sbmf_ctx* c, uint32_t s_cur) {
    unsigned long long h[128];
    HIPCHK(hipMemcpy(h, c->d_kprof.p, sizeof(h), hipMemcpyDeviceToHost));
    HIPCHK(hipMemset(c->d_kprof.p, 0, sizeof(h)));
    static const char* gn[7] = {"setup", "load+mfma", "barrier", "reduce", "solve+handoff", "e-update",
                                "epilogue"};
    for (int sd = 0; sd < 2; ++sd) {
        double tot = 0;
        for (int k = 0; k < 7; ++k) tot += (double)h[16 + 8 * sd + k];
        if (tot == 0) continue;
        std::fprintf(stderr, "[kprof] sweep %u %s gblock multi-wave rows (wave-0 Gcycles total):", s_cur,
                     sd ? "items" : "users");
        for (int k = 0; k < 7; ++k)
            std::fprintf(stderr, " %s %.3f (%.0f%%)", gn[k], (double)h[16 + 8 * sd + k] / 1e9,
                         100.0 * (double)h[16 + 8 * sd + k] / tot);
        std::fprintf(stderr, "\n");
    }
    static const char* nm[7] = {"stage", "apply+issue", "gather+acc", "wg-wait", "xwave+xchg", "solve", "epilogue"};
    for (int sd = 0; sd < 2; ++sd) {
        const Side& S = sd ? c->items : c->users;
        double tot = 0;
        const unsigned long long x7 = h[96 + 2 * sd], x8 = h[97 + 2 * sd], x4 = h[8 * sd + 4];
        h[8 * sd + 4] += x7 + x8;
        for (int k = 0; k < 7; ++k) tot += (double)h[8 * sd + k];
        if (tot == 0) continue;
        std::fprintf(stderr, "[kprof] sweep %u gres %s (grid %u, %zu tasks, wave-0 Mcycles per WG):", s_cur,
                     sd ? "items" : "users", S.stg[0]->ss[c->kprof_set].sgrid,
                     S.stg[0]->ss[c->kprof_set].stasks.size());
        for (int k = 0; k < 7; ++k)
            std::fprintf(stderr, " %s %.3f (%.0f%%)", nm[k], (double)h[8 * sd + k] / S.stg[0]->ss[c->kprof_set].sgrid / 1e6,
                         100.0 * (double)h[8 * sd + k] / tot);
        std::fprintf(stderr, "\n[kprof]   xwave+xchg = xwave+publish %.3f + to-first-valid %.3f + read+sum %.3f\n",
                     (double)x7 / S.stg[0]->ss[c->kprof_set].sgrid / 1e6, (double)x8 / S.stg[0]->ss[c->kprof_set].sgrid / 1e6,
                     (double)x4 / S.stg[0]->ss[c->kprof_set].sgrid / 1e6);
        static const char* cn[3] = {"whole rows", "2-16 chunks", ">16 chunks"};
        for (int cl = 0; cl < 3; ++cl) {
            unsigned long long* hc = h + 32 + 24 * sd + 8 * cl;
            if (!hc[7]) continue;
            const unsigned long long* hx = h + 100 + 6 * sd + 2 * cl;
            const unsigned long long c4 = hc[4];
            hc[4] += hx[0] + hx[1];
            std::fprintf(stderr, "[kprof]   %s: %llu tasks, kcycles per task:", cn[cl], hc[7]);
            for (int k = 0; k < 7; ++k) std::fprintf(stderr, " %s %.1f", nm[k], (double)hc[k] / hc[7] / 1e3);
            std::fprintf(stderr, " (xwave+publish %.1f, to-first-valid %.1f, read+sum %.1f)\n", (double)hx[0] / hc[7] / 1e3,
                         (double)hx[1] / hc[7] / 1e3, (double)c4 / hc[7] / 1e3);
        }
    }
}

static double draw_hyper(const sbmf_ctx* c, const Hyper& prev, const double* res, const HostStream& hs, Hyper& next) {
    const sbmf_config& cf = c->cfg;
    const uint32_t K = c->K;
    const uint64_t N = c->tu.size();
    const bool q2 = cf.quirks == SBMF_QUIRKS_SBPMF2;
    const double* Su2 = &res[RES_COL];
    const double* Su1 = Su2 + K;
    const double* Sv2 = Su2 + 2 * K;
    const double* Sv1 = Su2 + 3 * K;
    auto sd = [&](double var) { return c->sd_is_var ? var : std::sqrt(var); };
    for (std::vector<double>* v : {&next.sig_u, &next.mu_u, &next.sig_v, &next.mu_v}) v->resize(K);
    double d0 = 0.0;
    if (c->bias) {
        const double es = res[RES_ES], esq = res[RES_ESQ2];
        next.tau = hs.g_tau / (cf.b0 + esq);
        next.sig_b0 = hs.g_sb0 / (cf.beta0 + (0.5 * (prev.b0 - prev.mu_b0) * (prev.b0 - prev.mu_b0)));
        const double s0 = 1.0 / (cf.nu0 + next.sig_b0);
        next.mu_b0 = s0 * ((cf.nu0 * cf.mu0) + prev.b0 * next.sig_b0) + sd(s0) * hs.z_mb0;
        const double sb0 = 1 / (next.sig_b0 + next.tau * (double)N);
        const double mb0 = sb0 * (next.sig_b0 * next.mu_b0 + next.tau * (es + (double)N * prev.b0));
        next.b0 = mb0 + sd(sb0) * hs.z_b0;
        d0 = prev.b0 - next.b0;
        for (uint32_t k = 0; k < K; ++k) {
            next.sig_u[k] = hs.g_su[k] / (cf.beta0 + (0.5) * Su2[k]);
            const double s2 = 1 / (cf.nu0 + next.sig_u[k] * c->I);
            next.mu_u[k] = s2 * (cf.nu0 * cf.mu0 + next.sig_u[k] * Su1[k]) + sd(s2) * hs.z_mu[k];
            next.sig_v[k] = hs.g_sv[k] / (cf.beta0 + (0.5) * Sv2[k]);
            const double s1 = 1 / (cf.nu0 + next.sig_v[k] * c->J);
            next.mu_v[k] = s1 * (cf.nu0 * cf.mu0 + next.sig_v[k] * Sv1[k]) + sd(s1) * hs.z_mv[k];
        }
    } else {
        const double esq = res[RES_ESQ];
        next.tau = hs.g_tau / (cf.b0 + 0.5 * esq);
        for (uint32_t k = 0; k < K; ++k) {
            const double du = prev.mu_u[k] - cf.mu0;
            const double bu = q2 ? cf.beta0 + cf.nu0 * du * du + (0.5) * Su2[k]
                                 : cf.beta0 + 0.5 * cf.nu0 * du * du + (0.5) * Su2[k];
            next.sig_u[k] = hs.g_su[k] / bu;
            const double su_star = (double)1.0 / (cf.nu0 * next.sig_u[k] + next.sig_u[k] * c->I);
            const double mu_star = su_star * (cf.nu0 * cf.mu0 * next.sig_u[k] + next.sig_u[k] * Su1[k]);
            next.mu_u[k] = mu_star + sd(su_star) * hs.z_mu[k];
            const double dv = prev.mu_v[k] - cf.mu0;
            const double bv = q2 ? cf.beta0 + cf.nu0 * dv * dv + (0.5) * Sv2[k]
                                 : cf.beta0 + 0.5 * cf.nu0 * dv * dv + (0.5) * Sv2[k];
            next.sig_v[k] = hs.g_sv[k] / bv;
            const double sv_star = (double)1.0 / (cf.nu0 * next.sig_v[k] + next.sig_v[k] * c->J);
            const double mv_star = (q2 ? su_star : sv_star) * (cf.nu0 * cf.mu0 * next.sig_v[k] + next.sig_v[k] * Sv1[k]);
            next.mu_v[k] = mv_star + sd(sv_star) * hs.z_mv[k];
        }
    }
    return d0;
}

template <typename T>
struct SweepRun {
    sbmf_ctx* const c;
    const sbmf_config& cf = c->cfg;
    const hipStream_t st = c->st;
    const uint32_t K = c->K;
    const uint64_t N = c->tu.size(), T_ = c->su.size();
    const bool ref = cf.rng_mode == SBMF_RNG_REFERENCE;
    const bool q2 = cf.quirks == SBMF_QUIRKS_SBPMF2;
    double* const d_res = c->d_res.as<double>();
    double* const scratch = c->d_scratch.as<double>();
    const bool overlap = !ref && !(cf.tune & 0x4000000u);
    const bool par_eval = overlap && c->nranks == 1 && !(cf.tune & 0x10000000u);
    const hipEvent_t ev3 = c->nranks > 1 ? c->ev[3] : c->ev[2];
    const hipEvent_t ev5 = c->nranks > 1 ? c->ev[5] : c->ev[4];
    hipEvent_t ev1(bool staged) const { return staged ? c->ev[0] : c->ev[1]; }

    void prologue_gpu(uint32_t sw, const Hyper& prev) {
        const bool recompute = sw == 0 || (cf.recompute_every && sw % cf.recompute_every == 0);
        if (recompute) {
            HIPCHK(launch_resid<T>(c->d_rtasks.as<ResidTask>(), (uint32_t)c->items.rtasks.size(),
                                   c->d_rtptr.as<uint32_t>(), c->items.r0, c->items.r1, c->d_vpart.as<uint32_t>(),
                                   (c->nranks > 1 ? c->d_vperm2 : c->d_vperm).as<uint32_t>(), c->d_vr.as<T>(),
                                   c->d_V.as<T>(), c->d_U.as<T>(), K,
                                   c->Kp, c->d_Eu.as<T>(), c->d_rtsq.as<double>(), c->d_rowsq_v.as<double>(),
                                   c->bias ? c->d_bv.as<double>() : nullptr, c->d_bu.as<double>(), prev.b0, st));
            c->launches++;
            if (c->nranks > 1) c->comm->bcast_ranges(c->d_rowsq_v.p, sizeof(double), c->items.bounds, st);
            exchange_residuals<T>(c, false, st);
        }
        HIPCHK(launch_sum(c->d_rowsq_v.as<double>(), c->J, d_res + RES_ESQ, scratch, st));
        if (c->bias) {
            double* rs2 = c->d_epart.as<double>();
            HIPCHK(launch_rowsum2<T>(c->d_uptr.as<uint32_t>(), c->users.r0, c->users.r1, c->d_Eu.as<T>(), rs2, st));
            if (c->nranks > 1) c->comm->bcast_ranges(rs2, 2 * sizeof(double), c->users.bounds, st);
            HIPCHK(launch_sum_cols(rs2, c->I, 2, d_res + RES_ES, st));
        }
        const T* hyp = c->d_hyper.as<T>();
        double* colpart = c->d_colpart.as<double>();
        double* colpart_v = colpart + (size_t)((c->I + 255) / 256) * 2 * K;
        HIPCHK(launch_colstats<T>(c->d_U.as<T>(), c->I, hyp + c->Kp, colpart, c->d_V.as<T>(), c->J, hyp + 3 * c->Kp,
                                  colpart_v, K, c->Kp, st));
        HIPCHK(launch_sum_cols2(colpart, (c->I + 255) / 256, d_res + RES_COL, colpart_v, (c->J + 255) / 256,
                                d_res + RES_COL + 2 * K, 2 * K, st));
        c->launches += 3;
        HIPCHK(hipMemcpyAsync(c->h_pre, d_res, c->h_res.size() * sizeof(double), hipMemcpyDeviceToHost, st));
    }
    void stage_hyper(const Hyper& hy) {
        const size_t Kp = c->Kp;
        T* h = static_cast<T*>(c->h_hyper());
        HIPCHK(hipEventSynchronize(c->hev));
        std::fill(h, h + 4 * Kp, T(0));
        for (uint32_t k = 0; k < K; ++k) {
            h[k] = (T)hy.sig_u[k];
            h[Kp + k] = (T)hy.mu_u[k];
            h[2 * Kp + k] = (T)hy.sig_v[k];
            h[3 * Kp + k] = (T)hy.mu_v[k];
        }
        HIPCHK(hipMemcpyAsync(c->d_hyper.p, h, 4 * Kp * sizeof(T), hipMemcpyHostToDevice, st));
        HIPCHK(hipEventRecord(c->hev, st));
    }
    struct Start {
        bool staged;
        uint32_t n_launch;
    };
    Start start_sweep(bool first) {
        c->time_kinds = first;
        const uint32_t n0 = c->launches;
        HIPCHK(hipEventRecord(c->ev[0], st));
        double d0;
        Hyper& hy = c->hyper_of(c->sweep);
        const Hyper& prev = c->hyper_of(c->sweep - 1);
        const bool staged = c->pre.valid && c->pre.sweep == c->sweep && c->pre.staged;
        if (!staged && c->hyper_ahead) stage_hyper(prev);
        c->hyper_ahead = false;
        if (c->pre.valid && c->pre.sweep == c->sweep) {
            std::swap(hy, c->pre.h);
            d0 = c->pre.d0;
        } else {
            HostStream hs;
            if (ref) {
                draw_hyper_variates(c->grand, c, hs);
            } else {
                PhiloxStream ps(cf.seed, c->sweep, 0);
                draw_hyper_variates(ps, c, hs);
            }
            prologue_gpu(c->sweep, prev);
            HIPCHK(hipStreamSynchronize(st));
            d0 = draw_hyper(c, prev, c->h_pre, hs, hy);
        }
        c->pre.valid = false;
        c->pre.staged = false;
        if (!staged) {
            stage_hyper(hy);
            if (ref && c->bias) {
                fill_bias_variates<T>(c, hy);
            } else if (ref) {
                fill_z<T>(c, c->I, c->d_zU);
                fill_z<T>(c, c->J, c->d_zV);
            }
            HIPCHK(hipStreamSynchronize(st));
            HIPCHK(hipEventRecord(c->ev[1], st));
        }
        if (!ref && !staged)
            HIPCHK(launch_philox_fill<T>(c->d_zU.as<T>(), K, c->users.r0, c->users.r1, cf.seed, c->sweep, TAG_USERS, st));
        if (c->bias)
            HIPCHK(launch_bias_rows<T>(c->d_uptr.as<uint32_t>(), c->users.r0, c->users.r1, c->d_Eu.as<T>(),
                                       c->d_bu.as<double>(), c->d_mbu.as<double>(), c->d_sbu.as<double>(),
                                       ref ? c->d_var3u.as<double>() : nullptr, bias_args(c, hy, true, d0), st));
        run_half_pipelined<T>(c, hy, true, [&](uint32_t p) {
            bcast_stage(c, c->users, p, c->d_U.p, c->Kp * sizeof(T));
            if (c->bias) bcast_stage(c, c->users, p, c->d_bu.p, sizeof(double));
        }, c->nranks == 1 && staged && !c->bias ? ev1(staged) : nullptr);
        if (c->nranks > 1) HIPCHK(hipEventRecord(c->ev[3], st));
        return Start{staged, c->launches - n0};
    }
    void item_half(const Hyper& hy, bool staged) {
        if (!ref && !staged)
            HIPCHK(launch_philox_fill<T>(c->d_zV.as<T>(), K, c->items.r0, c->items.r1, cf.seed, c->sweep, TAG_ITEMS, st));
        if (c->bias)
            HIPCHK(launch_bias_rows<T>(c->d_vptr.as<uint32_t>(), c->items.r0, c->items.r1, c->d_Ev.as<T>(),
                                       c->d_bv.as<double>(), c->d_mbv.as<double>(), c->d_sbv.as<double>(),
                                       ref ? c->d_var3v.as<double>() : nullptr, bias_args(c, hy, false, 0.0), st));
        run_half_pipelined<T>(c, hy, false, [&](uint32_t p) {
            bcast_stage(c, c->items, p, c->d_V.p, c->Kp * sizeof(T));
            if (c->bias) bcast_stage(c, c->items, p, c->d_bv.p, sizeof(double));
            bcast_stage(c, c->items, p, c->d_rowsq_v.p, sizeof(double));
            if (cf.eval_train) bcast_stage(c, c->items, p, c->d_rowtr_v.p, sizeof(double));
        }, c->nranks == 1 && staged && !c->bias ? c->ev[2] : nullptr);
        if (c->nranks > 1) HIPCHK(hipEventRecord(c->ev[5], st));
    }
    void evaluate(hipStream_t se, const Hyper& hy, bool collect, double div) {
        if (cf.eval_test && T_) {
            HIPCHK(launch_test<T>(c->d_tu.as<uint32_t>(), c->d_ti.as<uint32_t>(), c->d_tr.as<double>(), c->t0,
                                  c->t1, c->d_U.as<T>(), c->d_V.as<T>(), K, c->Kp, (T)c->lo, (T)c->hi,
                                  collect ? 1 : 0, div, c->d_tsum.as<double>(), c->d_tpart.as<double>(),
                                  c->bias ? c->d_bu.as<double>() : nullptr, c->d_bv.as<double>(), hy.b0, se));
            if (c->nranks > 1) c->comm->bcast_ranges(c->d_tpart.p, 2 * sizeof(double), c->tbblocks, se);
            const uint32_t nb = (uint32_t)((T_ + 255) / 256);
            HIPCHK(launch_sum_cols(c->d_tpart.as<double>(), nb, 2, d_res + RES_TEST_AVG, se));
        }
        if (cf.eval_train)
            HIPCHK(launch_sum(c->d_rowtr_v.as<double>(), c->J, d_res + RES_TRSQ, scratch + c->scratch_half, se));
        if (c->watch.n && collect) {
            HIPCHK(hipEventRecord(c->wev[0], se));
            c->watch.accumulate<T>(c, c->d_U.as<T>(), c->bias ? c->d_bu.as<double>() : nullptr, c->d_bv.as<double>(),
                                   hy.b0, se);
            HIPCHK(hipEventRecord(c->wev[1], se));
        }
        if (c->samples.cap && collect) c->samples.keep<T>(c, hy, se);
        if (c->guests.n) {
            const size_t Kp = c->Kp;
            double* h = c->h_fhyp;
            HIPCHK(hipEventSynchronize(c->fev[0]));
            std::fill(h, h + 2 * Kp, 0.0);
            std::copy(hy.sig_u.begin(), hy.sig_u.begin() + K, h);
            std::copy(hy.mu_u.begin(), hy.mu_u.begin() + K, h + Kp);
            HIPCHK(hipMemcpyAsync(c->d_fhyp.p, h, 2 * Kp * sizeof(double), hipMemcpyHostToDevice, se));
            HIPCHK(hipEventRecord(c->fev[0], se));
            HIPCHK(launch_foldin<T>(c->guests.n, c->fcsr.d_order.as<uint32_t>(), c->fcsr.d_ptr.as<uint32_t>(),
                                    c->fcsr.d_items.as<uint32_t>(), c->fcsr.d_ratings.as<double>(), c->d_fG.as<T>(),
                                    c->d_V.as<T>(), K, c->Kp, c->d_fhyp.as<double>(), hy.tau, c->sd_is_var, cf.seed,
                                    c->sweep, c->fcsr.d_E.as<double>(), se));
            HIPCHK(hipEventRecord(c->fev[1], se));
            c->fdrawn++;
            c->launches++;
            if (collect) {
                c->guests.accumulate<T>(c, c->d_fG.as<T>(), nullptr, nullptr, 0.0, se);
                HIPCHK(hipEventRecord(c->fev[2], se));
            }
        }
        HIPCHK(hipEventRecord(c->ev[6], se));
    }
    void evaluation(const Hyper& hy, bool collect, double div) {
        if (par_eval) {
            HIPCHK(hipStreamWaitEvent(c->sto, ev5, 0));
            evaluate(c->sto, hy, collect, div);
        }
        if (overlap) {
            prologue_gpu(c->sweep + 1, hy);
            HIPCHK(hipEventRecord(c->ev[7], st));
            HIPCHK(launch_philox_fill2<T>(c->d_zU.as<T>(), c->users.r0, c->users.r1, TAG_USERS, c->d_zV.as<T>(),
                                          c->items.r0, c->items.r1, TAG_ITEMS, K, cf.seed, c->sweep + 1, st));
            HIPCHK(hipEventRecord(c->ev[8], st));
        }
        if (par_eval)
            HIPCHK(hipStreamWaitEvent(st, c->ev[6], 0));
        else
            evaluate(st, hy, collect, div);
        HIPCHK(hipMemcpyAsync(c->h_out(), d_res, 8 * sizeof(double), hipMemcpyDeviceToHost, st));
        HIPCHK(hipEventRecord(c->ev[9], st));
    }
    void draw_ahead(const Hyper& hy) {
        HIPCHK(hipEventSynchronize(c->ev[7]));
        HostStream hs;
        PhiloxStream ps(cf.seed, c->sweep + 1, 0);
        draw_hyper_variates(ps, c, hs);
        c->pre.d0 = draw_hyper(c, hy, c->h_pre, hs, c->pre.h);
        c->pre.sweep = c->sweep + 1;
        c->pre.valid = true;
        stage_hyper(c->pre.h);
        c->pre.staged = true;
        c->hyper_ahead = true;
    }
    void report_times(sbmf_sweep_info& info, bool staged) {
        c->timing.ms_hyper = staged ? 0.0 : ev_ms(c->ev[0], ev1(staged));
        c->timing.ms_user_half = ev_ms(ev1(staged), c->ev[2]);
        c->timing.ms_item_half = ev_ms(ev3, c->ev[4]);
        c->timing.ms_comm = c->nranks > 1 ? ev_ms(c->ev[2], c->ev[3]) + ev_ms(c->ev[4], c->ev[5]) : 0.0;
        for (int sd = 0; sd < 2; ++sd) {
            const Side& sdd = sd == 0 ? c->users : c->items;
            for (int k = 0; k < SBMF_NKIND; ++k) {
                if (!c->time_kinds && k != KIND_STREAM) continue;
                double ms = 0.0;
                for (uint32_t p = 0; p < c->nstages; ++p) {
                    const Side::Stage& g = *sdd.stg[p];
                    const bool ran = k < NBIN && !g.bin_rows[k].empty();
                    const int kp = ran ? c->kpv(p, sd, k) : -1;
                    if (ran) ms += ev_ms(kp >= 0 ? c->kev(p, sd, kp, 1) : c->kbg(p, sd, k), c->kev(p, sd, k, 1));
                }
                c->timing.kern_ms[sd][k] = ms;
            }
        }
        info.ms_sweep = ev_ms(c->ev[0], ev5);
    }
    void report_results(sbmf_sweep_info& info) {
        const double* res8 = c->h_out();
        std::copy(res8, res8 + 8, c->h_res.begin());
        uint32_t split_timeout;
        std::memcpy(&split_timeout, res8 + RES_TIMEOUT, sizeof(split_timeout));
        if (c->kprof) kprof_report(c, info.sweep);
        if (split_timeout)
            fail(SBMF_E_STATE, "sweep %u: split-row hand-off timed out (workgroups not co-resident)", info.sweep);
        info.rmse_avg = (cf.eval_test && T_) ? std::sqrt(c->h_res[RES_TEST_AVG] / T_) : NAN;
        info.rmse_this = (cf.eval_test && T_) ? std::sqrt(c->h_res[RES_TEST_THIS] / T_) : NAN;
        info.rmse_train = cf.eval_train && N ? std::sqrt(c->h_res[RES_TRSQ] / N) : NAN;
        c->timing.ms_hyper += overlap ? ev_ms(ev5, c->ev[8]) : 0.0;
        c->timing.ms_eval = overlap && !par_eval ? ev_ms(c->ev[8], c->ev[6]) : ev_ms(ev5, c->ev[6]);
        info.ms_eval = c->timing.ms_eval;
    }

    void run(uint32_t nsweeps, sbmf_sweep_cb cb, void* user) {
        bool queued = false, stop_after = false;
        Start start{};
        for (uint32_t it = 0; it < nsweeps; ++it) {
            if (!queued) start = start_sweep(it == 0);
            queued = false;
            const Hyper& hy = c->hyper_of(c->sweep);
            const uint32_t n1 = c->launches;
            const bool collect = q2 ? true : (c->sweep >= cf.burnin);
            if (collect) c->collected++;
            const double div = avg_collected(cf) ? (double)std::max(1u, c->collected) : (double)(c->sweep + 1);
            item_half(hy, start.staged);
            evaluation(hy, collect, div);
            if (overlap) draw_ahead(hy);
            if (!overlap) HIPCHK(hipEventSynchronize(c->ev[9]));
            sbmf_sweep_info info{};
            info.acc_train = info.acc_avg = info.acc_this = info.ll_this = NAN;
            info.sweep = c->sweep;
            info.collected = collect ? 1u : 0u;
            info.tau = hy.tau;
            report_times(info, start.staged);
            c->timing.n_launch = start.n_launch + (c->launches - n1);
            c->sweep++;
            if (overlap && cf.pipeline && it + 1 < nsweeps && !c->kprof && !stop_after) {
                start = start_sweep(false);
                queued = true;
            }
            if (overlap) HIPCHK(hipEventSynchronize(c->ev[9]));
            report_results(info);
            c->reported = (int)(info.sweep & 1);
            if (cb && cb(&info, user)) {
                if (!queued) break;
                stop_after = true;
            } else if (stop_after) {
                break;
            }
        }
    }
};

template <typename T>
void run_sweeps_T(sbmf_ctx* c, uint32_t nsweeps, sbmf_sweep_cb cb, void* user) {
    SweepRun<T>{c}.run(nsweeps, cb, user);
}
template void run_sweeps_T<float>(sbmf_ctx*, uint32_t, sbmf_sweep_cb, void*);
template void run_sweeps_T<double>(sbmf_ctx*, uint32_t, sbmf_sweep_cb, void*);
template void run_half<float>(sbmf_ctx*, const Hyper&, bool, uint32_t, hipEvent_t);
template void run_half<double>(sbmf_ctx*, const Hyper&, bool, uint32_t, hipEvent_t);

}
```

Baseline: 2.847 billion.

## Double-buffer U and move sweep-tail evaluation off the critical stream

The user factor table is double-buffered, so the user half writes into a separate output buffer and evaluation can keep reading the previous U while the next sweep proceeds. An optional short-tail mode (enabled only by the SBMF_SHORT_TAIL env var) runs evaluation and next-sweep noise generation on side streams, with event waits at the start of the next sweep instead of serialising on the main stream. This costs twice the U memory, an extra device copy at init and upload, and more complex cross-stream dependencies, including a change to which result entries get copied back. With the default settings only the double buffering runs, and the tail path stays dormant.

```diff
diff --git a/scalable-bayesian-matrix-factorization_amd/csrc/ctx.h b/scalable-bayesian-matrix-factorization_amd/csrc/ctx.h
--- a/scalable-bayesian-matrix-factorization_amd/csrc/ctx.h
+++ b/scalable-bayesian-matrix-factorization_amd/csrc/ctx.h
@@ -165,8 +165,18 @@
     hipStream_t sto = nullptr;
     hipStream_t sto2 = nullptr;
     hipEvent_t oev[4] = {};
+    hipStream_t eval_stream() const { return nranks == 1 ? stc : sto; }
+    hipEvent_t tev[2] = {};
+    bool tail_pending = false;
+    bool short_tail = false;
     DBuf d_uptr, d_upart, d_uperm, d_ur, d_vptr, d_vpart, d_vperm, d_vr;
-    DBuf d_U, d_V, d_Eu, d_Ev, d_zU, d_zV, d_hyper;
+    DBuf d_V, d_Eu, d_Ev, d_zU, d_zV, d_hyper;
+    DBuf d_Ub[2];
+    int u_cur = 0;
+    DBuf& U() { return d_Ub[u_cur]; }
+    const DBuf& U() const { return d_Ub[u_cur]; }
+    DBuf& U_out() { return d_Ub[u_cur ^ 1]; }
+    void flip_U() { u_cur ^= 1; }
     DBuf d_rowsq_u, d_rowtr_u, d_rowsq_v, d_rowtr_v;
     DBuf d_colpart, d_res, d_scratch;
     size_t scratch_half = 0;
@@ -290,6 +300,10 @@
     c->cfg.precision == SBMF_F32 ? download_table<float>(c, d, dst, R) : download_table<double>(c, d, dst, R);
 }
 
+static void mirror_U(sbmf_ctx* c, hipStream_t st) {
+    HIPCHK(hipMemcpyAsync(c->U_out().p, c->U().p, c->U().bytes, hipMemcpyDeviceToDevice, st));
+}
+
 static void ensure_pinned(sbmf_ctx* c, size_t bytes) {
     if (c->h_pinned_bytes >= bytes) return;
     pinned_free(c->h_pinned, c->h_pinned_bytes);
diff --git a/scalable-bayesian-matrix-factorization_amd/csrc/kernels.h b/scalable-bayesian-matrix-factorization_amd/csrc/kernels.h
--- a/scalable-bayesian-matrix-factorization_amd/csrc/kernels.h
+++ b/scalable-bayesian-matrix-factorization_amd/csrc/kernels.h
@@ -13,7 +13,8 @@
     const T* E_this;
     T* E_other;
     const T* r_this;
-    T* own;
+    const T* own;
+    T* own_out;
     const T* partner;
     const T* sig;
     const T* mu;
@@ -93,7 +94,8 @@
     const T* E_this;
     T* E_other;
     const T* r_this;
-    T* own;
+    const T* own;
+    T* own_out;
     const T* zbuf;
     const T* sig;
     double* row_sq;
diff --git a/scalable-bayesian-matrix-factorization_amd/csrc/kernels.hip b/scalable-bayesian-matrix-factorization_amd/csrc/kernels.hip
--- a/scalable-bayesian-matrix-factorization_amd/csrc/kernels.hip
+++ b/scalable-bayesian-matrix-factorization_amd/csrc/kernels.hip
@@ -401,7 +401,7 @@
                 if (wr == 0 && lane < GB && kin) newS[kk] = nwv;
                 if (lane < GB) Dsh[lane] = dlt;
             } else {
-                if (lane < GB && kin) a.own[(size_t)row * Kp + kk] = nwv;
+                if (lane < GB && kin) a.own_out[(size_t)row * Kp + kk] = nwv;
             }
         }
         if constexpr (NW > 1) {
@@ -428,7 +428,7 @@
 
     if constexpr (NW > 1) {
         lds_barrier();
-        for (uint32_t k = threadIdx.x; k < K; k += 64 * NW) a.own[(size_t)row * Kp + k] = newS[k];
+        for (uint32_t k = threadIdx.x; k < K; k += 64 * NW) a.own_out[(size_t)row * Kp + k] = newS[k];
     }
     T sq = T(0), trs = T(0);
 #pragma unroll
@@ -953,7 +953,7 @@
         const uint32_t row = tk.row;
         if (!DIRECT && tk.chunk == 0) {
             const auto dst = nch > 1 ? glob(cz->newown) + (size_t)CHK(tk.slab0, cz->lim_chunk) * Kp
-                                     : glob(cz->own) + (size_t)CHK(row, cz->lim_rows) * Kp;
+                                     : glob(cz->own_out) + (size_t)CHK(row, cz->lim_rows) * Kp;
             for (uint32_t k = threadIdx.x; k < K; k += 64 * NW) dst[k] = newS[k];
         }
         double dsq = wave_sum(sums.sq);
@@ -1007,7 +1007,7 @@
             last[CHK((size_t)(i / SLP) * sy.nblk * SLAB_DOUBLES + i % SLP,
                      sy.lim_slab - ((size_t)sr.slab0 * sy.nblk + (sy.nblk - 1)) * SLAB_DOUBLES)] = XSENT;
     }
-    for (uint32_t k = threadIdx.x; k < K; k += 64) a.own[(size_t)sr.row * Kp + k] = static_cast<const T*>(sy.newown)[(size_t)sr.slab0 * Kp + k];
+    for (uint32_t k = threadIdx.x; k < K; k += 64) a.own_out[(size_t)sr.row * Kp + k] = static_cast<const T*>(sy.newown)[(size_t)sr.slab0 * Kp + k];
     if (threadIdx.x == 0) {
         double s = 0.0, t = 0.0;
         for (uint32_t c = 0; c < sr.nch; ++c) {
@@ -1509,6 +1509,7 @@
     c.E_other = a.E_other;
     c.r_this = a.r_this;
     c.own = a.own;
+    c.own_out = a.own_out;
     c.zbuf = a.zbuf;
     c.sig = a.sig;
     c.row_sq = a.row_sq;
@@ -1538,7 +1539,7 @@
     h.partner = a.partner;
     h.cold = d_cold;
     if (!sy) {
-        h.own = a.own;
+        h.own = a.own_out;
         h.sig = a.sig;
     }
     h.tau = a.tau;
diff --git a/scalable-bayesian-matrix-factorization_amd/csrc/lists.cpp b/scalable-bayesian-matrix-factorization_amd/csrc/lists.cpp
--- a/scalable-bayesian-matrix-factorization_amd/csrc/lists.cpp
+++ b/scalable-bayesian-matrix-factorization_amd/csrc/lists.cpp
@@ -23,8 +23,7 @@
 }
 void list_sync(sbmf_ctx* c) {
     HIPCHK(hipSetDevice(c->cfg.device));
-    HIPCHK(hipStreamSynchronize(c->sto));
-    HIPCHK(hipStreamSynchronize(c->st));
+    for (hipStream_t s : {c->sto, c->stc, c->st}) HIPCHK(hipStreamSynchronize(s));
 }
 
 void TopnScratch::alloc(uint32_t rows, uint32_t topn, uint32_t J, bool exclude) {
diff --git a/scalable-bayesian-matrix-factorization_amd/csrc/prepare.cpp b/scalable-bayesian-matrix-factorization_amd/csrc/prepare.cpp
--- a/scalable-bayesian-matrix-factorization_amd/csrc/prepare.cpp
+++ b/scalable-bayesian-matrix-factorization_amd/csrc/prepare.cpp
@@ -272,8 +272,8 @@
             fail(SBMF_E_ARG, "split-row exchange area of %zu chunks at K=%u exceeds 2^32 bytes", nx, c->K);
         c->d_xslabs.alloc(nx * nblk * SLAB_DOUBLES * sizeof(double));
         HIPCHK(hipMemsetAsync(c->d_xslabs.p, 0xff, c->d_xslabs.bytes, st));
-        c->d_gcold.alloc((size_t)c->nstages * 6 * sbmf_ctx::kColdSlot);
-        c->h_gcold.assign((size_t)c->nstages * 6 * sbmf_ctx::kColdSlot, 0xff);
+        c->d_gcold.alloc((size_t)c->nstages * 12 * sbmf_ctx::kColdSlot);
+        c->h_gcold.assign((size_t)c->nstages * 12 * sbmf_ctx::kColdSlot, 0xff);
         c->d_xcnt.alloc(64 * sizeof(uint32_t));
         HIPCHK(hipMemsetAsync(c->d_xcnt.p, 0, c->d_xcnt.bytes, st));
         c->d_xchunk_sq.alloc(nx * sizeof(double));
@@ -281,9 +281,14 @@
         HIPCHK(hipMemsetAsync(c->d_xchunk_tr.p, 0, c->d_xchunk_tr.bytes, st));
         c->d_xnewown.alloc(nx * c->Kp * sizeof(T));
     }
-    c->d_U.alloc((size_t)(c->I + 2) * c->Kp * sizeof(T));
+    c->u_cur = 0;
+    c->tail_pending = false;
+    c->short_tail = std::getenv("SBMF_SHORT_TAIL") && std::atoi(std::getenv("SBMF_SHORT_TAIL")) > 0;
+    for (DBuf& d : c->d_Ub) {
+        d.alloc((size_t)(c->I + 2) * c->Kp * sizeof(T));
+        HIPCHK(hipMemsetAsync(d.p, 0, d.bytes, st));
+    }
     c->d_V.alloc((size_t)(c->J + 2) * c->Kp * sizeof(T));
-    HIPCHK(hipMemsetAsync(c->d_U.p, 0, c->d_U.bytes, st));
     HIPCHK(hipMemsetAsync(c->d_V.p, 0, c->d_V.bytes, st));
     c->d_Eu.alloc(std::max<uint64_t>(N + c->items.nsend, 1) * sizeof(T));
     c->d_Ev.alloc(std::max<uint64_t>(N + c->users.nsend, 1) * sizeof(T));
@@ -384,12 +389,13 @@
         for (uint32_t k = 0; k < c->K; ++k)
             for (uint32_t j = 0; j < c->J; ++j) V[(size_t)j * c->K + k] = 0.0 + c->init_sd * leva_normal(c->grand);
         HIPCHK(hipStreamSynchronize(st));
-        upload_table<T>(c, c->d_U, U.data(), c->I);
+        upload_table<T>(c, c->U(), U.data(), c->I);
         upload_table<T>(c, c->d_V, V.data(), c->J);
     } else {
-        HIPCHK(launch_init_philox<T>(c->d_U.as<T>(), c->K, c->Kp, 0, c->I, c->init_sd, cf.seed, TAG_INIT_U, st));
+        HIPCHK(launch_init_philox<T>(c->U().as<T>(), c->K, c->Kp, 0, c->I, c->init_sd, cf.seed, TAG_INIT_U, st));
         HIPCHK(launch_init_philox<T>(c->d_V.as<T>(), c->K, c->Kp, 0, c->J, c->init_sd, cf.seed, TAG_INIT_V, st));
     }
+    mirror_U(c, st);
     HIPCHK(hipStreamSynchronize(st));
     c->kprof = std::getenv("SBMF_KPROF") && std::atoi(std::getenv("SBMF_KPROF")) > 0;
     if (c->kprof) {
diff --git a/scalable-bayesian-matrix-factorization_amd/csrc/samples.cpp b/scalable-bayesian-matrix-factorization_amd/csrc/samples.cpp
--- a/scalable-bayesian-matrix-factorization_amd/csrc/samples.cpp
+++ b/scalable-bayesian-matrix-factorization_amd/csrc/samples.cpp
@@ -221,7 +221,7 @@
     const uint32_t p = count < cap ? slot(count) : head;
     const size_t I = c->I, J = c->J, Kp = c->Kp;
     cev.begin(se);
-    HIPCHK(hipMemcpyAsync(d_U.as<T>() + p * I * Kp, c->d_U.p, I * Kp * sizeof(T), hipMemcpyDeviceToDevice, se));
+    HIPCHK(hipMemcpyAsync(d_U.as<T>() + p * I * Kp, c->U().p, I * Kp * sizeof(T), hipMemcpyDeviceToDevice, se));
     HIPCHK(hipMemcpyAsync(d_V.as<T>() + p * J * Kp, c->d_V.p, J * Kp * sizeof(T), hipMemcpyDeviceToDevice, se));
     if (c->bias) {
         HIPCHK(hipMemcpyAsync(d_bu.as<double>() + p * I, c->d_bu.p, I * sizeof(double), hipMemcpyDeviceToDevice, se));
diff --git a/scalable-bayesian-matrix-factorization_amd/csrc/sbmf.cpp b/scalable-bayesian-matrix-factorization_amd/csrc/sbmf.cpp
--- a/scalable-bayesian-matrix-factorization_amd/csrc/sbmf.cpp
+++ b/scalable-bayesian-matrix-factorization_amd/csrc/sbmf.cpp
@@ -37,6 +37,7 @@
     samples.drop();
     pinned_free(h_fhyp, h_fhyp_bytes);
     event_destroy(hev);
+    for (auto& e : tev) event_destroy(e);
     stream_destroy(sto);
     stream_destroy(sto2);
     stream_destroy(stc);
@@ -268,6 +269,7 @@
     sbmf::stream_create(&c->sto2);
     for (auto& e : c->oev) sbmf::event_create(&e, hipEventDisableTiming);
     sbmf::event_create(&c->hev, hipEventDisableTiming);
+    for (auto& e : c->tev) sbmf::event_create(&e, hipEventDisableTiming);
     *out = c.release();
     API_END(ctx)
 }
@@ -795,7 +797,7 @@
         ctx->fm->factors(U, V);
         return SBMF_OK;
     }
-    if (U) sbmf::download_table(ctx, ctx->d_U, U, ctx->I);
+    if (U) sbmf::download_table(ctx, ctx->U(), U, ctx->I);
     if (V) sbmf::download_table(ctx, ctx->d_V, V, ctx->J);
     API_END(ctx)
 }
@@ -809,7 +811,11 @@
     HIPCHK(hipSetDevice(ctx->cfg.device));
     HIPCHK(hipStreamSynchronize(ctx->st));
     ctx->pre.valid = false;
-    if (U) sbmf::upload_table(ctx, ctx->d_U, U, ctx->I);
+    if (U) {
+        sbmf::upload_table(ctx, ctx->U(), U, ctx->I);
+        sbmf::mirror_U(ctx, ctx->st);
+        HIPCHK(hipStreamSynchronize(ctx->st));
+    }
     if (V) sbmf::upload_table(ctx, ctx->d_V, V, ctx->J);
     API_END(ctx)
 }
diff --git a/scalable-bayesian-matrix-factorization_amd/csrc/sweep.cpp b/scalable-bayesian-matrix-factorization_amd/csrc/sweep.cpp
--- a/scalable-bayesian-matrix-factorization_amd/csrc/sweep.cpp
+++ b/scalable-bayesian-matrix-factorization_amd/csrc/sweep.cpp
@@ -133,7 +133,8 @@
         a.E_this = c->d_Eu.as<T>();
         a.E_other = c->d_Ev.as<T>();
         a.r_this = c->d_ur.as<T>();
-        a.own = c->d_U.as<T>();
+        a.own = c->U().as<T>();
+        a.own_out = c->U_out().as<T>();
         a.partner = c->d_V.as<T>();
         a.sig = c->d_hyper.as<T>();
         a.mu = c->d_hyper.as<T>() + c->Kp;
@@ -149,8 +150,8 @@
         a.E_this = c->d_Ev.as<T>();
         a.E_other = c->d_Eu.as<T>();
         a.r_this = c->d_vr.as<T>();
-        a.own = c->d_V.as<T>();
-        a.partner = c->d_U.as<T>();
+        a.own = a.own_out = c->d_V.as<T>();
+        a.partner = c->U().as<T>();
         a.sig = c->d_hyper.as<T>() + 2 * c->Kp;
         a.mu = c->d_hyper.as<T>() + 3 * c->Kp;
         a.zrow = c->I;
@@ -177,13 +178,17 @@
     return a;
 }
 
+static int cold_slot(const sbmf_ctx* c, uint32_t stage, int side, int shape) {
+    const int par = side == 0 ? c->u_cur : 0;
+    return (par * (int)c->nstages + (int)stage) * 6 + side * 3 + shape;
+}
 template <typename T>
 static const GresCold<T>* cold_block(sbmf_ctx* c, int slot, const GresCold<T>& cold) {
     static_assert(sizeof(GresCold<T>) <= sbmf_ctx::kColdSlot, "cold block slot");
     unsigned char* h = c->h_gcold.data() + (size_t)slot * sbmf_ctx::kColdSlot;
     unsigned char* d = c->d_gcold.as<unsigned char>() + (size_t)slot * sbmf_ctx::kColdSlot;
     if (std::memcmp(h, &cold, sizeof(cold)) != 0) {
-        for (hipStream_t s : {c->st, c->sto, c->sto2}) HIPCHK(hipStreamSynchronize(s));
+        for (hipStream_t s : {c->st, c->sto, c->sto2, c->stc}) HIPCHK(hipStreamSynchronize(s));
         HIPCHK(hipMemcpy(d, &cold, sizeof(cold), hipMemcpyHostToDevice));
         std::memcpy(h, &cold, sizeof(cold));
         static const bool log = std::getenv("SBMF_COLD_LOG") != nullptr;
@@ -250,7 +255,7 @@
                                                                       : 0;
         if (gw) {
             HIPCHK(launch_grow<T>(gw, g.d_bins[k].as<uint32_t>(), (uint32_t)g.bin_rows[k].size(), a,
-                                  cold_block<T>(c, (2 * (int)stage + sd) * 3 + 2, gres_cold<T>(a, nullptr)), st));
+                                  cold_block<T>(c, cold_slot(c, stage, sd, 2), gres_cold<T>(a, nullptr)), st));
         } else if (k < GK_NUM && k >= GK_B2 && !(c->cfg.tune & 4u)) {
             for (const auto& gs : g.gsub[k])
                 HIPCHK(launch_gblock_nw<T>((int)gs[0], g.d_bins[k].as<uint32_t>() + gs[1], gs[2], a, st));
@@ -279,7 +284,7 @@
                 as.tune = S.tune;
                 HIPCHK(launch_gstream<T>(g.d_stasks[set].as<SplitTask>(), (uint32_t)S.stasks.size(), S.sgrid,
                                          g.d_xrows[set].as<SplitRow>(), (uint32_t)S.xrows.size(), as, sy,
-                                         cold_block<T>(c, (2 * (int)stage + sd) * 3 + set, gres_cold<T>(as, &sy)), ss));
+                                         cold_block<T>(c, cold_slot(c, stage, sd, set), gres_cold<T>(as, &sy)), ss));
                 if (ss == c->st) st_busy = true;
             }
             if (sov) {
@@ -473,6 +478,8 @@
     double* const scratch = c->d_scratch.as<double>();
     const bool overlap = !ref && !(cf.tune & 0x4000000u);
     const bool par_eval = overlap && c->nranks == 1 && !(cf.tune & 0x10000000u);
+    const bool tail = par_eval && c->short_tail;
+    const hipStream_t se = tail ? c->eval_stream() : c->sto;
     const hipEvent_t ev3 = c->nranks > 1 ? c->ev[3] : c->ev[2];
     const hipEvent_t ev5 = c->nranks > 1 ? c->ev[5] : c->ev[4];
     hipEvent_t ev1(bool staged) const { return staged ? c->ev[0] : c->ev[1]; }
@@ -483,7 +490,7 @@
             HIPCHK(launch_resid<T>(c->d_rtasks.as<ResidTask>(), (uint32_t)c->items.rtasks.size(),
                                    c->d_rtptr.as<uint32_t>(), c->items.r0, c->items.r1, c->d_vpart.as<uint32_t>(),
                                    (c->nranks > 1 ? c->d_vperm2 : c->d_vperm).as<uint32_t>(), c->d_vr.as<T>(),
-                                   c->d_V.as<T>(), c->d_U.as<T>(), K,
+                                   c->d_V.as<T>(), c->U().as<T>(), K,
                                    c->Kp, c->d_Eu.as<T>(), c->d_rtsq.as<double>(), c->d_rowsq_v.as<double>(),
                                    c->bias ? c->d_bv.as<double>() : nullptr, c->d_bu.as<double>(), prev.b0, st));
             c->launches++;
@@ -500,7 +507,7 @@
         const T* hyp = c->d_hyper.as<T>();
         double* colpart = c->d_colpart.as<double>();
         double* colpart_v = colpart + (size_t)((c->I + 255) / 256) * 2 * K;
-        HIPCHK(launch_colstats<T>(c->d_U.as<T>(), c->I, hyp + c->Kp, colpart, c->d_V.as<T>(), c->J, hyp + 3 * c->Kp,
+        HIPCHK(launch_colstats<T>(c->U().as<T>(), c->I, hyp + c->Kp, colpart, c->d_V.as<T>(), c->J, hyp + 3 * c->Kp,
                                   colpart_v, K, c->Kp, st));
         HIPCHK(launch_sum_cols2(colpart, (c->I + 255) / 256, d_res + RES_COL, colpart_v, (c->J + 255) / 256,
                                 d_res + RES_COL + 2 * K, 2 * K, st));
@@ -528,11 +535,16 @@
     Start start_sweep(bool first) {
         c->time_kinds = first;
         const uint32_t n0 = c->launches;
+        const bool staged = c->pre.valid && c->pre.sweep == c->sweep && c->pre.staged;
+        if (c->tail_pending) {
+            HIPCHK(hipStreamWaitEvent(st, c->tev[0], 0));
+            HIPCHK(hipStreamWaitEvent(st, staged ? c->ev[6] : c->tev[1], 0));
+            if (!staged) c->tail_pending = false;
+        }
         HIPCHK(hipEventRecord(c->ev[0], st));
         double d0;
         Hyper& hy = c->hyper_of(c->sweep);
         const Hyper& prev = c->hyper_of(c->sweep - 1);
-        const bool staged = c->pre.valid && c->pre.sweep == c->sweep && c->pre.staged;
         if (!staged && c->hyper_ahead) stage_hyper(prev);
         c->hyper_ahead = false;
         if (c->pre.valid && c->pre.sweep == c->sweep) {
@@ -570,13 +582,16 @@
                                        c->d_bu.as<double>(), c->d_mbu.as<double>(), c->d_sbu.as<double>(),
                                        ref ? c->d_var3u.as<double>() : nullptr, bias_args(c, hy, true, d0), st));
         run_half_pipelined<T>(c, hy, true, [&](uint32_t p) {
-            bcast_stage(c, c->users, p, c->d_U.p, c->Kp * sizeof(T));
+            bcast_stage(c, c->users, p, c->U_out().p, c->Kp * sizeof(T));
             if (c->bias) bcast_stage(c, c->users, p, c->d_bu.p, sizeof(double));
         }, c->nranks == 1 && staged && !c->bias ? ev1(staged) : nullptr);
+        c->flip_U();
         if (c->nranks > 1) HIPCHK(hipEventRecord(c->ev[3], st));
         return Start{staged, c->launches - n0};
     }
     void item_half(const Hyper& hy, bool staged) {
+        if (c->tail_pending) HIPCHK(hipStreamWaitEvent(st, c->tev[1], 0));
+        c->tail_pending = false;
         if (!ref && !staged)
             HIPCHK(launch_philox_fill<T>(c->d_zV.as<T>(), K, c->items.r0, c->items.r1, cf.seed, c->sweep, TAG_ITEMS, st));
         if (c->bias)
@@ -594,7 +609,7 @@
     void evaluate(hipStream_t se, const Hyper& hy, bool collect, double div) {
         if (cf.eval_test && T_) {
             HIPCHK(launch_test<T>(c->d_tu.as<uint32_t>(), c->d_ti.as<uint32_t>(), c->d_tr.as<double>(), c->t0,
-                                  c->t1, c->d_U.as<T>(), c->d_V.as<T>(), K, c->Kp, (T)c->lo, (T)c->hi,
+                                  c->t1, c->U().as<T>(), c->d_V.as<T>(), K, c->Kp, (T)c->lo, (T)c->hi,
                                   collect ? 1 : 0, div, c->d_tsum.as<double>(), c->d_tpart.as<double>(),
                                   c->bias ? c->d_bu.as<double>() : nullptr, c->d_bv.as<double>(), hy.b0, se));
             if (c->nranks > 1) c->comm->bcast_ranges(c->d_tpart.p, 2 * sizeof(double), c->tbblocks, se);
@@ -605,7 +620,7 @@
             HIPCHK(launch_sum(c->d_rowtr_v.as<double>(), c->J, d_res + RES_TRSQ, scratch + c->scratch_half, se));
         if (c->watch.n && collect) {
             HIPCHK(hipEventRecord(c->wev[0], se));
-            c->watch.accumulate<T>(c, c->d_U.as<T>(), c->bias ? c->d_bu.as<double>() : nullptr, c->d_bv.as<double>(),
+            c->watch.accumulate<T>(c, c->U().as<T>(), c->bias ? c->d_bu.as<double>() : nullptr, c->d_bv.as<double>(),
                                    hy.b0, se);
             HIPCHK(hipEventRecord(c->wev[1], se));
         }
@@ -634,9 +649,24 @@
         HIPCHK(hipEventRecord(c->ev[6], se));
     }
     void evaluation(const Hyper& hy, bool collect, double div) {
+        if (tail) {
+            prologue_gpu(c->sweep + 1, hy);
+            HIPCHK(hipEventRecord(c->ev[7], st));
+            HIPCHK(hipStreamWaitEvent(se, ev5, 0));
+            evaluate(se, hy, collect, div);
+            HIPCHK(hipMemcpyAsync(c->h_out() + 1, d_res + 1, 7 * sizeof(double), hipMemcpyDeviceToHost, se));
+            HIPCHK(hipEventRecord(c->ev[9], se));
+            HIPCHK(hipEventRecord(c->tev[1], se));
+            HIPCHK(hipStreamWaitEvent(c->sto, ev5, 0));
+            HIPCHK(launch_philox_fill2<T>(c->d_zU.as<T>(), c->users.r0, c->users.r1, TAG_USERS, c->d_zV.as<T>(),
+                                          c->items.r0, c->items.r1, TAG_ITEMS, K, cf.seed, c->sweep + 1, c->sto));
+            HIPCHK(hipEventRecord(c->tev[0], c->sto));
+            c->tail_pending = true;
+            return;
+        }
         if (par_eval) {
-            HIPCHK(hipStreamWaitEvent(c->sto, ev5, 0));
-            evaluate(c->sto, hy, collect, div);
+            HIPCHK(hipStreamWaitEvent(se, ev5, 0));
+            evaluate(se, hy, collect, div);
         }
         if (overlap) {
             prologue_gpu(c->sweep + 1, hy);
@@ -687,7 +717,7 @@
     }
     void report_results(sbmf_sweep_info& info) {
         const double* res8 = c->h_out();
-        std::copy(res8, res8 + 8, c->h_res.begin());
+        std::copy(res8 + 1, res8 + 8, c->h_res.begin() + 1);
         uint32_t split_timeout;
         std::memcpy(&split_timeout, res8 + RES_TIMEOUT, sizeof(split_timeout));
         if (c->kprof) kprof_report(c, info.sweep);
@@ -696,7 +726,7 @@
         info.rmse_avg = (cf.eval_test && T_) ? std::sqrt(c->h_res[RES_TEST_AVG] / T_) : NAN;
         info.rmse_this = (cf.eval_test && T_) ? std::sqrt(c->h_res[RES_TEST_THIS] / T_) : NAN;
         info.rmse_train = cf.eval_train && N ? std::sqrt(c->h_res[RES_TRSQ] / N) : NAN;
-        c->timing.ms_hyper += overlap ? ev_ms(ev5, c->ev[8]) : 0.0;
+        c->timing.ms_hyper += overlap ? ev_ms(ev5, c->ev[tail ? 7 : 8]) : 0.0;
         c->timing.ms_eval = overlap && !par_eval ? ev_ms(c->ev[8], c->ev[6]) : ev_ms(ev5, c->ev[6]);
         info.ms_eval = c->timing.ms_eval;
     }
```

New measurement: 2.850 billion (median of 2 runs). Within noise of the previous version (+0.1%).
